# hpcde/spmv-acc

Measured on AMD Instinct MI355X. Metric: CSR SpMV GFLOP/s (fp64, int32 indices; achieved HBM GB/s in roofline), higher is better.
Workload: dtype f64

## Files before the change

include/spmv_acc.h:

```cpp
#ifndef SPMV_ACC_C_ABI_H
#define SPMV_ACC_C_ABI_H

#ifdef __cplusplus
extern "C" {
#endif

enum spmv_acc_strategy {
  SPMV_ACC_DEFAULT = 0,
  SPMV_ACC_ADAPTIVE = 1,
  SPMV_ACC_THREAD_ROW = 2,
  SPMV_ACC_WF_ROW = 3,
  SPMV_ACC_BLOCK_ROW_ORDINARY = 4,
  SPMV_ACC_LIGHT = 5,
  SPMV_ACC_VECTOR_ROW = 6,
  SPMV_ACC_LINE_ENHANCE = 7,
  SPMV_ACC_LINE = 8,
  SPMV_ACC_FLAT = 9,
  SPMV_ACC_ADAPTIVE_PLUS = 10
};
int spmv_acc_set_strategy(const char *name);
int spmv_acc_set_strategy_id(int strategy);
int spmv_acc_get_strategy(void);
const char *spmv_acc_strategy_name(int strategy);
int spmv_acc_parse_strategy(const char *name);

#ifndef SPMV_ACC_AMD_API_SPMV_H
void sparse_spmv(int htrans, const double halpha, const double hbeta, int hm, int hn, const int *rowptr,
                 const int *colindex, const double *value, const double *x, double *y);
#endif

void spmv_acc_csr_spmv(int trans, double alpha, double beta, int m, int n, int nnz, const int *h_rowptr,
                       const int *d_rowptr, const int *d_colindex, const double *d_value, const double *dx,
                       double *dy);

void spmv_acc_csr_spmv_strategy(int strategy, int trans, double alpha, double beta, int m, int n, int nnz,
                                const int *h_rowptr, const int *d_rowptr, const int *d_colindex,
                                const double *d_value, const double *dx, double *dy);

void spmv_acc_csr_spmv_oop(int strategy, int trans, double alpha, double beta, int m, int n, int nnz, const int *h_rowptr,
                           const int *d_rowptr, const int *d_colindex, const double *d_value, const double *dx,
                           const double *dy_in, double *dy_out);

enum spmv_acc_layout { SPMV_ACC_ROW_MAJOR = 0, SPMV_ACC_COL_MAJOR = 1 };
int spmv_acc_csr_spmm(int layout, int k, double alpha, double beta, int m, int n, int nnz, const int *h_rowptr,
                      const int *d_rowptr, const int *d_colindex, const double *d_value,
                      const double *dX, long long ldx, double *dY, long long ldy);

int spmv_acc_csr_spmv_chunks(int strategy, double alpha, double beta, int n, int nchunks, const int *row_cuts, const int *nnz_ends,
                             const int *d_rowptr, const int *d_colindex, const double *d_value, const double *dx,
                             const double *dy_in, double *dy_out, void *const *streams, void *const *events);

int spmv_acc_break_points(const int *d_rowptr, int m, int nnz, int stride, int *d_break_points, int bp_len);
int spmv_acc_break_points_len(int nnz, int stride);

int spmv_acc_adaptive_plus_analyze(int m, int min_nnz_per_block, int threads_per_block, int vec_size,
                                   const int *h_rowptr, int *h_break_points, int bp_cap,
                                   int *h_first_block_of_row);
int spmv_acc_adaptive_plus_analyze_device(int m, int min_nnz_per_block, int threads_per_block, int vec_size,
                                          const int *d_rowptr, int *d_break_points, int bp_cap,
                                          int *d_first_block_of_row);
int spmv_acc_adaptive_plus_vec(int m, int nnz);

int spmv_acc_adaptive_branch(int m, int rp_quarter, int rp_half, int rp_three_quarter, int rp_last);

int spmv_acc_partition_rows(int m, int parts, int mode, const int *h_rowptr, int *row_begin);

int spmv_acc_sharded_spmv(void *nccl_comm, int strategy, double alpha, double beta, int m_local, int m_pad, int n, int nnz_local,
                          const int *h_rowptr, const int *d_rowptr, const int *d_colindex, const double *d_value, const double *dx,
                          double *dy_local, double *dy_full);

typedef struct spmv_acc_shard *spmv_acc_shard_t;
int spmv_acc_shard_create(spmv_acc_shard_t *out, void *nccl_comm, int strategy, int m_local, int m_pad, int n, int nnz_local,
                          const int *d_rowptr, const int *d_colindex, const double *d_value, int pipeline);
int spmv_acc_shard_step(spmv_acc_shard_t shard, double alpha, double beta, const double *dx, const double *dy_in_local,
                        double *dy_full);
int spmv_acc_shard_prepare(spmv_acc_shard_t shard, double beta, const double *dx);
int spmv_acc_shard_pipeline(spmv_acc_shard_t shard);
int spmv_acc_shard_destroy(spmv_acc_shard_t shard);
int spmv_acc_rccl_comm_init_all(void **comms, int ndev, const int *devices);
int spmv_acc_rccl_comm_destroy(void *comm);

int spmv_acc_stage_csr(int m, int n, int nnz, const int *h_rowptr, const int *h_colindex, const double *h_value,
                       const double *h_x, const double *h_y, int **d_rowptr, int **d_colindex, double **d_value,
                       double **d_x, double **d_y);
int spmv_acc_free_device(void *p);

int spmv_acc_prepare(int strategy, int m, int n, int nnz, const int *h_rowptr, const int *d_rowptr, const int *d_colindex,
                     const double *d_value, const double *dx, float *ms_out);
int spmv_acc_prepare_beta(int strategy, double beta, int m, int n, int nnz, const int *h_rowptr, const int *d_rowptr,
                          const int *d_colindex, const double *d_value, const double *dx, float *ms_out);

void spmv_acc_set_tune_cache(const char *path);

int spmv_acc_refresh_values(const int *d_rowptr);

double spmv_acc_last_prepare_us(void);

void spmv_acc_release_plans(const int *d_rowptr);
int spmv_acc_cached_plans(void);
int spmv_acc_check_plans(void);
int spmv_acc_query_plan(const int *d_rowptr, int m, int *out);
int spmv_acc_query_plan_beta0(const int *d_rowptr, int m);
int spmv_acc_query_plan_slab_passes(const int *d_rowptr, int m);
int spmv_acc_query_plan_settled(const int *d_rowptr, int m);
int spmv_acc_query_plan_col16(const int *d_rowptr, int m);
enum spmv_acc_kernel {
  SPMV_ACC_KERNEL_ROWBLOCK = 0,
  SPMV_ACC_KERNEL_ROWBLOCK_PLUS = 1,
  SPMV_ACC_KERNEL_FLAT_TILE = 2,
  SPMV_ACC_KERNEL_SLAB_PASSES = 3,
  SPMV_ACC_KERNEL_VECTOR_TILE = 4, SPMV_ACC_KERNEL_VECTOR_ROW = 5, SPMV_ACC_KERNEL_WAVE_ROW = 6, SPMV_ACC_KERNEL_LIGHT = 7,
  SPMV_ACC_KERNEL_BLOCK_ROW = 8, SPMV_ACC_KERNEL_COL_SLABS = 9, SPMV_ACC_KERNEL_SCALE_ONLY = 10
};
int spmv_acc_query_plan_last_kernel(const int *d_rowptr, int m);

void spmv_acc_set_stream(void *hip_stream);
void *spmv_acc_get_stream(void);

int spmv_acc_last_error(void);
const char *spmv_acc_last_error_string(void);
void spmv_acc_clear_error(void);
enum spmv_acc_error {
  SPMV_ACC_OK = 0,
  SPMV_ACC_ERR_UNSUPPORTED_TRANS = 1,
  SPMV_ACC_ERR_BAD_ARGUMENT = 2,
  SPMV_ACC_ERR_HIP = 3,
  SPMV_ACC_ERR_TOO_LARGE = 4,
  SPMV_ACC_ERR_UNKNOWN_STRATEGY = 5,
  SPMV_ACC_ERR_NO_DEVICE = 6
};

int spmv_acc_time_spmv(int strategy, int iters, double alpha, double beta, int m, int n, int nnz,
                       const int *h_rowptr, const int *d_rowptr, const int *d_colindex, const double *d_value,
                       const double *dx, double *dy, const double *d_y0, float *ms_out);

int spmv_acc_time_spmv_events(int strategy, int iters, double alpha, double beta, int m, int n, int nnz,
                              const int *h_rowptr, const int *d_rowptr, const int *d_colindex, const double *d_value,
                              const double *dx, double *dy, const double *d_y0, float *ms_out, unsigned event_flags);

int spmv_acc_time_spmv_cold(int strategy, int iters, double alpha, double beta, int m, int n, int nnz,
                            const int *h_rowptr, const int *d_rowptr, const int *d_colindex, const double *d_value,
                            const double *dx, double *dy, const double *d_y0, void *d_flush, long long flush_bytes, float *ms_out);

int spmv_acc_time_spmv_total(int strategy, int iters, double alpha, double beta, int m, int n, int nnz,
                             const int *h_rowptr, const int *d_rowptr, const int *d_colindex, const double *d_value,
                             const double *dx, double *dy, float *total_ms_out);
int spmv_acc_time_spmv_kernels(int strategy, int iters, double alpha, double beta, int m, int n, int nnz,
                               const int *h_rowptr, const int *d_rowptr, const int *d_colindex, const double *d_value,
                               const double *dx, double *dy, const double *d_y0, float *event_ms_out, float *kernel_ms_out, int *launches_out);
int spmv_acc_time_spmv_region(int strategy, int iters, double alpha, double beta, int m, int n, int nnz,
                              const int *h_rowptr, const int *d_rowptr, const int *d_colindex, const double *d_value,
                              const double *dx, double *dy, float *total_ms_out);
double spmv_acc_copy_ceiling_gbs(void *d_dst, const void *d_src, long long bytes, int reps);

int spmv_acc_set_tunable(const char *name, int value);
int spmv_acc_get_tunable(const char *name);
void spmv_acc_reset_tunables(void);

const char *spmv_acc_version(void);

#ifdef __cplusplus
}
#endif

#endif
```

spmv_acc_amd/__init__.py:

```python
from __future__ import annotations

import ctypes
import os
from typing import Optional, Sequence

_HERE = os.path.dirname(os.path.abspath(__file__))
LIB_PATH = os.path.join(_HERE, "lib", "libspmv_acc.so")

STRATEGIES = (
    "default", "adaptive", "thread_row", "wf_row", "block_row_ordinary", "light",
    "vector_row", "line_enhance", "line", "flat", "adaptive_plus",
)
HOT_STRATEGIES = ("default", "adaptive", "flat", "line_enhance", "line", "vector_row", "adaptive_plus")

_c_int_p = ctypes.POINTER(ctypes.c_int)
_c_double_p = ctypes.POINTER(ctypes.c_double)

C_ABI_SYMBOLS = (
    "sparse_spmv", "spmv_acc_csr_spmv", "spmv_acc_csr_spmv_strategy", "spmv_acc_set_strategy",
    "spmv_acc_set_strategy_id", "spmv_acc_get_strategy", "spmv_acc_strategy_name", "spmv_acc_parse_strategy",
    "spmv_acc_break_points", "spmv_acc_break_points_len", "spmv_acc_adaptive_plus_analyze",
    "spmv_acc_adaptive_plus_vec", "spmv_acc_adaptive_branch", "spmv_acc_partition_rows", "spmv_acc_stage_csr",
    "spmv_acc_free_device", "spmv_acc_release_plans", "spmv_acc_cached_plans", "spmv_acc_query_plan",
    "spmv_acc_set_stream", "spmv_acc_get_stream", "spmv_acc_last_error", "spmv_acc_last_error_string",
    "spmv_acc_clear_error", "spmv_acc_time_spmv", "spmv_acc_version", "spmv_acc_set_tunable",
    "spmv_acc_get_tunable", "spmv_acc_reset_tunables", "spmv_acc_time_spmv_total", "spmv_acc_copy_ceiling_gbs", "spmv_acc_adaptive_plus_analyze_device", "spmv_acc_prepare",
    "spmv_acc_last_prepare_us", "spmv_acc_sharded_spmv", "spmv_acc_shard_prepare", "spmv_acc_csr_spmv_chunks", "spmv_acc_query_plan_settled", "spmv_acc_query_plan_col16", "spmv_acc_time_spmv_cold", "spmv_acc_csr_spmv_oop", "spmv_acc_check_plans",
    "spmv_acc_query_plan_beta0", "spmv_acc_query_plan_slab_passes", "spmv_acc_shard_create", "spmv_acc_shard_step", "spmv_acc_shard_pipeline",
    "spmv_acc_shard_destroy", "spmv_acc_rccl_comm_init_all", "spmv_acc_rccl_comm_destroy", "spmv_acc_set_tune_cache",
    "spmv_acc_prepare_beta", "spmv_acc_time_spmv_events", "spmv_acc_refresh_values", "spmv_acc_time_spmv_region", "spmv_acc_query_plan_last_kernel", "spmv_acc_time_spmv_kernels",
    "spmv_acc_csr_spmm",
)

_lib = None


class SpmvAccError(RuntimeError):
    pass


def load_library(path: Optional[str] = None) -> ctypes.CDLL:
    global _lib
    if _lib is not None and path is None:
        return _lib
    p = path or LIB_PATH
    if not os.path.exists(p):
        raise SpmvAccError(
            f"{p} not found: the HIP extension is not built. Run `python -c 'import __graft_entry__ as g; g.build()'` "
            "or `make -C spmv_acc_amd/csrc`. There is no CPU fallback."
        )
    try:
        import torch
    except ImportError:
        pass
    lib = ctypes.CDLL(p)
    vp, ci, cd = ctypes.c_void_p, ctypes.c_int, ctypes.c_double
    lib.sparse_spmv.argtypes = [ci, cd, cd, ci, ci, vp, vp, vp, vp, vp]
    lib.sparse_spmv.restype = None
    lib.spmv_acc_csr_spmv.argtypes = [ci, cd, cd, ci, ci, ci, vp, vp, vp, vp, vp, vp]
    lib.spmv_acc_csr_spmv.restype = None
    lib.spmv_acc_csr_spmv_strategy.argtypes = [ci, ci, cd, cd, ci, ci, ci, vp, vp, vp, vp, vp, vp]
    lib.spmv_acc_csr_spmv_strategy.restype = None
    lib.spmv_acc_set_strategy.argtypes = [ctypes.c_char_p]
    lib.spmv_acc_set_strategy_id.argtypes = [ci]
    lib.spmv_acc_strategy_name.argtypes = [ci]
    lib.spmv_acc_strategy_name.restype = ctypes.c_char_p
    lib.spmv_acc_parse_strategy.argtypes = [ctypes.c_char_p]
    lib.spmv_acc_break_points.argtypes = [vp, ci, ci, ci, vp, ci]
    lib.spmv_acc_break_points_len.argtypes = [ci, ci]
    lib.spmv_acc_adaptive_plus_analyze.argtypes = [ci, ci, ci, ci, vp, vp, ci, vp]
    lib.spmv_acc_adaptive_plus_vec.argtypes = [ci, ci]
    lib.spmv_acc_adaptive_plus_analyze_device.argtypes = [ci, ci, ci, ci, vp, vp, ci, vp]
    lib.spmv_acc_adaptive_branch.argtypes = [ci, ci, ci, ci, ci]
    lib.spmv_acc_partition_rows.argtypes = [ci, ci, ci, vp, vp]
    lib.spmv_acc_stage_csr.argtypes = [ci, ci, ci, vp, vp, vp, vp, vp] + [ctypes.POINTER(vp)] * 5
    lib.spmv_acc_free_device.argtypes = [vp]
    lib.spmv_acc_prepare.argtypes = [ci, ci, ci, ci, vp, vp, vp, vp, vp, ctypes.POINTER(ctypes.c_float)]
    lib.spmv_acc_release_plans.argtypes = [vp]
    lib.spmv_acc_release_plans.restype = None
    lib.spmv_acc_query_plan.argtypes = [vp, ci, vp]
    lib.spmv_acc_set_stream.argtypes = [vp]
    lib.spmv_acc_set_stream.restype = None
    lib.spmv_acc_get_stream.restype = vp
    lib.spmv_acc_last_error_string.restype = ctypes.c_char_p
    lib.spmv_acc_clear_error.restype = None
    lib.spmv_acc_time_spmv.argtypes = [ci, ci, cd, cd, ci, ci, ci, vp, vp, vp, vp, vp, vp, vp, vp]
    lib.spmv_acc_time_spmv_events.argtypes = [ci, ci, cd, cd, ci, ci, ci, vp, vp, vp, vp, vp, vp, vp, vp, ctypes.c_uint]
    lib.spmv_acc_time_spmv_cold.argtypes = [ci, ci, cd, cd, ci, ci, ci, vp, vp, vp, vp, vp, vp, vp, vp, ctypes.c_longlong, vp]
    lib.spmv_acc_version.restype = ctypes.c_char_p
    lib.spmv_acc_set_tunable.argtypes = [ctypes.c_char_p, ci]
    lib.spmv_acc_get_tunable.argtypes = [ctypes.c_char_p]
    lib.spmv_acc_reset_tunables.restype = None
    lib.spmv_acc_time_spmv_total.argtypes = [ci, ci, cd, cd, ci, ci, ci, vp, vp, vp, vp, vp, vp, vp]
    lib.spmv_acc_time_spmv_kernels.argtypes = [ci, ci, cd, cd, ci, ci, ci, vp, vp, vp, vp, vp, vp, vp, vp, vp, vp]
    lib.spmv_acc_time_spmv_region.argtypes = [ci, ci, cd, cd, ci, ci, ci, vp, vp, vp, vp, vp, vp, vp]
    lib.spmv_acc_copy_ceiling_gbs.argtypes = [vp, vp, ctypes.c_longlong, ci]
    lib.spmv_acc_copy_ceiling_gbs.restype = cd
    lib.spmv_acc_last_prepare_us.restype = cd
    lib.spmv_acc_sharded_spmv.argtypes = [vp, ci, cd, cd, ci, ci, ci, ci, vp, vp, vp, vp, vp, vp, vp]
    lib.spmv_acc_csr_spmv_oop.argtypes = [ci, ci, cd, cd, ci, ci, ci, vp, vp, vp, vp, vp, vp, vp]
    lib.spmv_acc_csr_spmv_oop.restype = None
    lib.spmv_acc_query_plan_beta0.argtypes = [vp, ci]
    lib.spmv_acc_query_plan_slab_passes.argtypes = [vp, ci]
    lib.spmv_acc_query_plan_settled.argtypes = [vp, ci]
    lib.spmv_acc_query_plan_col16.argtypes = [vp, ci]
    lib.spmv_acc_query_plan_last_kernel.argtypes = [vp, ci]
    lib.spmv_acc_shard_create.argtypes = [ctypes.POINTER(vp), vp, ci, ci, ci, ci, ci, vp, vp, vp, ci]
    lib.spmv_acc_shard_step.argtypes = [vp, cd, cd, vp, vp, vp]
    lib.spmv_acc_shard_pipeline.argtypes = [vp]
    lib.spmv_acc_shard_destroy.argtypes = [vp]
    lib.spmv_acc_rccl_comm_init_all.argtypes = [ctypes.POINTER(vp), ci, vp]
    lib.spmv_acc_rccl_comm_destroy.argtypes = [vp]
    lib.spmv_acc_set_tune_cache.argtypes = [ctypes.c_char_p]
    lib.spmv_acc_set_tune_cache.restype = None
    lib.spmv_acc_refresh_values.argtypes = [vp]
    lib.spmv_acc_prepare_beta.argtypes = [ci, cd, ci, ci, ci, vp, vp, vp, vp, vp, ctypes.POINTER(ctypes.c_float)]
    lib.spmv_acc_shard_prepare.argtypes = [vp, cd, vp]
    lib.spmv_acc_csr_spmv_chunks.argtypes = [ci, cd, cd, ci, ci, vp, vp, vp, vp, vp, vp, vp, vp, vp, vp]
    ll = ctypes.c_longlong
    lib.spmv_acc_csr_spmm.argtypes = [ci, ci, cd, cd, ci, ci, ci, vp, vp, vp, vp, vp, ll, vp, ll]
    lib.spmv_acc_csr_spmm.restype = ci
    if path is None:
        _lib = lib
    return lib


def strategy_id(name_or_id) -> int:
    if isinstance(name_or_id, int):
        return name_or_id
    s = load_library().spmv_acc_parse_strategy(str(name_or_id).encode())
    if s < 0:
        raise SpmvAccError(f"unknown KERNEL_STRATEGY {name_or_id!r}")
    return s


def _check(lib) -> None:
    code = lib.spmv_acc_last_error()
    if code not in (0, 1):
        msg = lib.spmv_acc_last_error_string().decode()
        lib.spmv_acc_clear_error()
        raise SpmvAccError(f"spmv_acc error {code}: {msg}")


def _ptr(t) -> int:
    if t is None:
        return 0
    if isinstance(t, int):
        return t
    if hasattr(t, "data_ptr"):
        return t.data_ptr()
    return t.ctypes.data


def _require_cuda(*tensors) -> None:
    for t in tensors:
        if t is not None and hasattr(t, "is_cuda") and not t.is_cuda:
            raise SpmvAccError("device pointers required: tensor is not on the GPU (no CPU fallback)")


def _require(lib, **named) -> None:
    device = None
    for name, (t, kind, count) in named.items():
        if t is None or not hasattr(t, "is_cuda"):
            continue
        if not t.is_cuda:
            raise SpmvAccError(f"{name}: device pointers required, tensor is not on the GPU (no CPU fallback)")
        want = "torch.int32" if kind == "i32" else "torch.float64"
        if str(t.dtype) != want:
            raise SpmvAccError(f"{name}: dtype {t.dtype}, the library reads {want} (int32 indices, fp64 values)")
        if not t.is_contiguous():
            raise SpmvAccError(f"{name}: tensor is not contiguous")
        if t.numel() < count:
            raise SpmvAccError(f"{name}: {t.numel()} elements, the shape needs at least {count}")
        if device is None:
            device = t.device
        elif t.device != device:
            raise SpmvAccError(f"{name}: on {t.device}, other arguments on {device}")
    if device is not None:
        import torch

        lib.spmv_acc_set_stream(torch.cuda.current_stream(device).cuda_stream)


def _csr_args(lib, m, n, nnz, rowptr, colindex, value, x, y=None, y0=None) -> None:
    k = max(nnz, 0)
    _require(lib, rowptr=(rowptr, "i32", m + 1), colindex=(colindex, "i32", k), value=(value, "f64", k),
             x=(x, "f64", n), y=(y, "f64", m), y0=(y0, "f64", m))


def sparse_spmv(trans: int, alpha: float, beta: float, m: int, n: int, rowptr, colindex, value, x, y) -> None:
    lib = load_library()
    _csr_args(lib, m, n, -1, rowptr, colindex, value, x, y)
    lib.sparse_spmv(trans, alpha, beta, m, n, _ptr(rowptr), _ptr(colindex), _ptr(value), _ptr(x), _ptr(y))
    _check(lib)


def csr_spmv(alpha: float, beta: float, m: int, n: int, nnz: int, rowptr, colindex, value, x, y,
             strategy=None, h_rowptr=None, trans: int = 0, y_in=None) -> None:
    lib = load_library()
    _csr_args(lib, m, n, nnz, rowptr, colindex, value, x, y, y_in)
    if y_in is not None:
        lib.spmv_acc_csr_spmv_oop(-1 if strategy is None else strategy_id(strategy), trans, alpha, beta, m, n, nnz,
                                  _ptr(h_rowptr), _ptr(rowptr), _ptr(colindex), _ptr(value), _ptr(x), _ptr(y_in), _ptr(y))
        _check(lib)
        return
    args = (trans, alpha, beta, m, n, nnz, _ptr(h_rowptr), _ptr(rowptr), _ptr(colindex), _ptr(value), _ptr(x), _ptr(y))
    if strategy is None:
        lib.spmv_acc_csr_spmv(*args)
    else:
        lib.spmv_acc_csr_spmv_strategy(strategy_id(strategy), *args)
    _check(lib)


SPMM_ROW_MAJOR, SPMM_COL_MAJOR = 0, 1


def _spmm_layouts(name, t, rows: int, k: int):
    s0, s1 = t.stride()
    out = {}
    if (s1 == 1 or k <= 1) and s0 >= max(k, 1):
        out[SPMM_ROW_MAJOR] = s0
    if (s0 == 1 or rows <= 1) and s1 >= max(rows, 1):
        out[SPMM_COL_MAJOR] = s1
    if not out and rows > 0 and k > 0:
        raise SpmvAccError(f"{name}: strides {tuple(t.stride())} of a ({rows}, {k}) view are neither row-major (unit stride on dim 1, "
                           f"leading dimension >= k) nor column-major (unit stride on dim 0, leading dimension >= {rows})")
    return out


def csr_spmm(alpha: float, beta: float, m: int, n: int, nnz: int, rowptr, colindex, value, X, Y, h_rowptr=None) -> None:
    lib = load_library()
    for name, t, rows in (("X", X, n), ("Y", Y, m)):
        if not hasattr(t, "is_cuda") or not hasattr(t, "stride"):
            raise SpmvAccError(f"{name}: a torch tensor on the GPU is required")
        if not t.is_cuda:
            raise SpmvAccError(f"{name}: device pointers required, tensor is not on the GPU (no CPU fallback)")
        if str(t.dtype) != "torch.float64":
            raise SpmvAccError(f"{name}: dtype {t.dtype}, the library reads torch.float64")
        if t.dim() != 2 or t.shape[0] != rows:
            raise SpmvAccError(f"{name}: shape {tuple(t.shape)}, expected ({rows}, k)")
    if X.shape[1] != Y.shape[1]:
        raise SpmvAccError(f"X has {X.shape[1]} columns, Y has {Y.shape[1]}")
    if X.device != Y.device:
        raise SpmvAccError(f"Y: on {Y.device}, X on {X.device}")
    k = int(X.shape[1])
    lx, ly = _spmm_layouts("X", X, n, k), _spmm_layouts("Y", Y, m, k)
    if not lx or not ly:
        layout, ldx, ldy = SPMM_ROW_MAJOR, k, k
    else:
        both = [lay for lay in (SPMM_ROW_MAJOR, SPMM_COL_MAJOR) if lay in lx and lay in ly]
        if not both:
            raise SpmvAccError("X and Y must share one layout (both row-major or both column-major)")
        layout = both[0]
        ldx, ldy = lx[layout], ly[layout]
    _require(lib, rowptr=(rowptr, "i32", m + 1), colindex=(colindex, "i32", max(nnz, 0)), value=(value, "f64", max(nnz, 0)))
    if hasattr(rowptr, "device") and rowptr.device != X.device:
        raise SpmvAccError(f"X: on {X.device}, rowptr on {rowptr.device}")
    lib.spmv_acc_set_stream(__import__("torch").cuda.current_stream(X.device).cuda_stream)
# ... 40 lines not shown
    if blocks < 0:
        raise SpmvAccError(f"adaptive_plus_analyze failed ({blocks})")
    return blocks, bp[: blocks + 1].copy(), fbr


def adaptive_plus_analyze_device(rowptr, m: int, nnz: int, min_nnz_per_block: int = 1024, threads_per_block: int = 256,
                                 vec_size: int = 1):
    import torch

    lib = load_library()
    _require(lib, rowptr=(rowptr, "i32", m + 1))
    cap = m + 2 + nnz // (2 * min_nnz_per_block)
    bp = torch.empty(cap, dtype=torch.int32, device=rowptr.device)
    fbr = torch.empty(m + 1, dtype=torch.int32, device=rowptr.device)
    blocks = lib.spmv_acc_adaptive_plus_analyze_device(m, min_nnz_per_block, threads_per_block, vec_size, _ptr(rowptr),
                                                       _ptr(bp), cap, _ptr(fbr))
    if blocks < 0:
        _check(lib)
        raise SpmvAccError(f"adaptive_plus_analyze_device failed ({blocks})")
    return blocks, bp[: blocks + 1], fbr


def adaptive_branch(m: int, h_rowptr) -> int:
    return load_library().spmv_acc_adaptive_branch(m, int(h_rowptr[m // 4]), int(h_rowptr[m // 2]),
                                                   int(h_rowptr[3 * m // 4]), int(h_rowptr[m]))


def partition_rows(m: int, parts: int, mode: int = 0, h_rowptr=None):
    import numpy as np

    lib = load_library()
    out = np.zeros(parts + 1, dtype=np.int32)
    if h_rowptr is not None:
        h_rowptr = np.ascontiguousarray(h_rowptr, dtype=np.int32)
    rc = lib.spmv_acc_partition_rows(m, parts, mode, _ptr(h_rowptr), _ptr(out))
    if rc != 0:
        _check(lib)
        raise SpmvAccError("partition_rows failed")
    return out


EVENT_DISABLE_SYSTEM_FENCE = 0x20000000


def time_spmv(strategy, iters: int, alpha: float, beta: float, m: int, n: int, nnz: int, rowptr, colindex, value,
              x, y, y0=None, h_rowptr=None, event_flags: int = 0) -> Sequence[float]:
    lib = load_library()
    _csr_args(lib, m, n, nnz, rowptr, colindex, value, x, y, y0)
    out = (ctypes.c_float * iters)()
    rc = lib.spmv_acc_time_spmv_events(strategy_id(strategy), iters, alpha, beta, m, n, nnz, _ptr(h_rowptr), _ptr(rowptr),
                                       _ptr(colindex), _ptr(value), _ptr(x), _ptr(y), _ptr(y0),
                                       ctypes.cast(out, ctypes.c_void_p), event_flags)
    if rc != 0:
        msg = lib.spmv_acc_last_error_string().decode()
        raise SpmvAccError(f"time_spmv failed ({rc}): {msg}")
    return list(out)


def time_spmv_cold(strategy, iters: int, alpha: float, beta: float, m: int, n: int, nnz: int, rowptr, colindex, value, x, y, y0, flush,
                   h_rowptr=None) -> Sequence[float]:
    lib = load_library()
    _csr_args(lib, m, n, nnz, rowptr, colindex, value, x, y, y0)
    out = (ctypes.c_float * iters)()
    rc = lib.spmv_acc_time_spmv_cold(strategy_id(strategy), iters, alpha, beta, m, n, nnz, _ptr(h_rowptr), _ptr(rowptr), _ptr(colindex),
                                     _ptr(value), _ptr(x), _ptr(y), _ptr(y0), _ptr(flush), int(flush.numel() * flush.element_size()),
                                     ctypes.cast(out, ctypes.c_void_p))
    if rc != 0:
        raise SpmvAccError(f"time_spmv_cold failed ({rc}): {lib.spmv_acc_last_error_string().decode()}")
    return list(out)


def time_spmv_total(strategy, iters: int, alpha: float, beta: float, m: int, n: int, nnz: int, rowptr, colindex, value,
                    x, y, h_rowptr=None) -> float:
    lib = load_library()
    _csr_args(lib, m, n, nnz, rowptr, colindex, value, x, y)
    out = ctypes.c_float(0.0)
    rc = lib.spmv_acc_time_spmv_total(strategy_id(strategy), iters, alpha, beta, m, n, nnz, _ptr(h_rowptr), _ptr(rowptr),
                                      _ptr(colindex), _ptr(value), _ptr(x), _ptr(y), ctypes.addressof(out))
    if rc != 0:
        raise SpmvAccError(f"time_spmv_total failed ({rc}): {lib.spmv_acc_last_error_string().decode()}")
    return float(out.value)


def time_spmv_kernels(strategy, iters: int, alpha: float, beta: float, m: int, n: int, nnz: int, rowptr, colindex, value, x, y, y0=None):
    lib = load_library()
    _csr_args(lib, m, n, nnz, rowptr, colindex, value, x, y, y0)
    ev = (ctypes.c_float * iters)()
    kn = (ctypes.c_float * iters)()
    ln = (ctypes.c_int * iters)()
    rc = lib.spmv_acc_time_spmv_kernels(strategy_id(strategy), iters, alpha, beta, m, n, nnz, None, _ptr(rowptr), _ptr(colindex), _ptr(value),
                                        _ptr(x), _ptr(y), _ptr(y0), ctypes.cast(ev, ctypes.c_void_p), ctypes.cast(kn, ctypes.c_void_p),
                                        ctypes.cast(ln, ctypes.c_void_p))
    if rc != 0:
        raise SpmvAccError(f"time_spmv_kernels failed ({rc}): {lib.spmv_acc_last_error_string().decode()}")
    return list(ev), list(kn), list(ln)


def time_spmv_region(strategy, iters: int, alpha: float, beta: float, m: int, n: int, nnz: int, rowptr, colindex, value, x, y):
    lib = load_library()
    _csr_args(lib, m, n, nnz, rowptr, colindex, value, x, y)
    out = ctypes.c_float(0.0)
    args = (strategy_id(strategy), iters, alpha, beta, m, n, nnz, None, _ptr(rowptr), _ptr(colindex), _ptr(value), _ptr(x), _ptr(y),
            ctypes.addressof(out))
    fn = lib.spmv_acc_time_spmv_region

    def run() -> float:
        rc = fn(*args)
        if rc != 0:
            raise SpmvAccError(f"time_spmv_region failed ({rc}): {lib.spmv_acc_last_error_string().decode()}")
        return float(out.value)

    return run


def copy_ceiling_gbs(dst, src, reps: int = 5) -> float:
    lib = load_library()
    _require_cuda(dst, src)
    nbytes = (src.numel() * src.element_size()) // 16 * 16
    return float(lib.spmv_acc_copy_ceiling_gbs(_ptr(dst), _ptr(src), nbytes, reps))


def release_plans(rowptr=None) -> None:
    load_library().spmv_acc_release_plans(_ptr(rowptr))


def set_tune_cache(path: Optional[str]) -> None:
    load_library().spmv_acc_set_tune_cache(path.encode() if path else None)


def refresh_values(rowptr) -> int:
    return int(load_library().spmv_acc_refresh_values(_ptr(rowptr)))


def check_plans() -> int:
    return int(load_library().spmv_acc_check_plans())


KERNEL_NAMES = {0: "rowblock", 1: "rowblock_plus", 2: "flat_tile", 3: "slab_passes", 4: "vector_tile", 5: "vector_row", 6: "wave_row", 7: "light",
                8: "block_row", 9: "col_slabs", 10: "scale_only"}


def query_plan(rowptr, m: int):
    import numpy as np

    out = np.zeros(9, dtype=np.int32)
    found = load_library().spmv_acc_query_plan(_ptr(rowptr), m, _ptr(out))
    if not found:
        return None
    keys = ("nnz", "adaptive_branch", "vec", "flat_tiles", "plus_blocks", "aligned16", "stream_policy", "flat_fixup", "adaptive_family")
    info = dict(zip(keys, (int(v) for v in out)))
    info["slab_passes"] = max(0, int(load_library().spmv_acc_query_plan_slab_passes(_ptr(rowptr), m)))
    info["settled"] = int(load_library().spmv_acc_query_plan_settled(_ptr(rowptr), m)) == 1
    info["col16"] = int(load_library().spmv_acc_query_plan_col16(_ptr(rowptr), m))
    info["last_kernel"] = KERNEL_NAMES.get(int(load_library().spmv_acc_query_plan_last_kernel(_ptr(rowptr), m)), "none")
    return info


def set_strategy(name: str) -> None:
    lib = load_library()
    if lib.spmv_acc_set_strategy(name.encode()) != 0:
        lib.spmv_acc_clear_error()
        raise SpmvAccError(f"unknown KERNEL_STRATEGY {name!r}")


def get_strategy() -> str:
    lib = load_library()
    return lib.spmv_acc_strategy_name(lib.spmv_acc_get_strategy()).decode()
```

spmv_acc_amd/csrc/c_api.cpp:

```cpp
#include <hip/hip_runtime.h>

#include <dlfcn.h>

#include <algorithm>
#include <cstdlib>
#include <cstring>
#include <mutex>
#include <vector>

#include "../../include/spmv_acc.h"
#include "engine.hpp"

#include <string>
#include <cstdint>

using namespace spmv_acc;

namespace {
struct PinTable {
  std::mutex mu;
  struct Range { uintptr_t lo, hi; int refs; };
  std::vector<Range> ranges;
  static constexpr uintptr_t kPage = 4096;
  bool pin(void *p, size_t bytes) {
// ... 202 lines not shown
  if (e != hipSuccess) {
    set_error(kErrHip, hipGetErrorString(e));
    return kErrHip;
  }
  return kOk;
}

int spmv_acc_adaptive_plus_analyze(int m, int min_nnz_per_block, int threads_per_block, int vec_size,
                                   const int *h_rowptr, int *h_break_points, int bp_cap,
                                   int *h_first_block_of_row) {
  if (m < 0 || !h_rowptr || !h_break_points || !h_first_block_of_row || min_nnz_per_block <= 0 || vec_size <= 0 ||
      threads_per_block < vec_size) {
    set_error(kErrBadArgument, "spmv_acc_adaptive_plus_analyze: bad argument");
    return -2;
  }
  std::vector<int> bp, fbr;
  const int blocks = plus_analyze_host(m, min_nnz_per_block, threads_per_block, vec_size, h_rowptr, bp, fbr);
  if (static_cast<int>(bp.size()) > bp_cap) return -1;
  std::copy(bp.begin(), bp.end(), h_break_points);
  std::copy(fbr.begin(), fbr.end(), h_first_block_of_row);
  return blocks;
}

int spmv_acc_adaptive_plus_analyze_device(int m, int min_nnz_per_block, int threads_per_block, int vec_size,
                                          const int *d_rowptr, int *d_break_points, int bp_cap,
                                          int *d_first_block_of_row) {
  if (m < 0 || !d_rowptr || !d_break_points || !d_first_block_of_row || min_nnz_per_block <= 0 || vec_size <= 0 ||
      threads_per_block < vec_size || bp_cap < 1) {
    set_error(kErrBadArgument, "spmv_acc_adaptive_plus_analyze_device: bad argument");
    return -2;
  }
  return plus_analyze_device(m, min_nnz_per_block, threads_per_block, vec_size, d_rowptr, d_break_points, bp_cap,
                             d_first_block_of_row);
}

int spmv_acc_adaptive_plus_vec(int m, int nnz) { return plus_pick_vec(m, nnz); }

int spmv_acc_adaptive_branch(int m, int rp_quarter, int rp_half, int rp_three_quarter, int rp_last) {
  if (m <= 0) return 0;
  RowptrSamples s;
  s.q1 = rp_quarter;
  s.half = rp_half;
  s.q3 = rp_three_quarter;
  s.last = rp_last;
  return adaptive_branch(m, s);
}

int spmv_acc_partition_rows(int m, int parts, int mode, const int *h_rowptr, int *row_begin) {
  if (m < 0 || parts <= 0 || !row_begin || (mode == 1 && !h_rowptr)) {
    set_error(kErrBadArgument, "spmv_acc_partition_rows: bad argument");
    return kErrBadArgument;
  }
  row_begin[0] = 0;
  row_begin[parts] = m;
  if (mode == 0) {
    const long long per = (static_cast<long long>(m) + parts - 1) / parts;
    for (int p = 1; p < parts; ++p) row_begin[p] = static_cast<int>(std::min<long long>(per * p, m));
  } else {
    const long long nnz = h_rowptr[m];
    for (int p = 1; p < parts; ++p) {
      const long long target = nnz * p / parts;
      const int *it = std::lower_bound(h_rowptr, h_rowptr + m + 1, static_cast<int>(target));
      int r = static_cast<int>(it - h_rowptr);
      r = std::max(r, row_begin[p - 1]);
      row_begin[p] = std::min(r, m);
    }
  }
  return kOk;
}

int spmv_acc_sharded_spmv(void *nccl_comm, int strategy, double alpha, double beta, int m_local, int m_pad, int n, int nnz_local,
                          const int *h_rowptr, const int *d_rowptr, const int *d_colindex, const double *d_value, const double *dx,
                          double *dy_local, double *dy_full) {
  if (!nccl_comm || m_local < 0 || m_pad < m_local || m_pad <= 0 || !dy_local || !dy_full) {
    set_error(kErrBadArgument, "spmv_acc_sharded_spmv: bad argument");
    return kErrBadArgument;
  }
  const nccl_all_gather_t all_gather = resolve_all_gather();
  if (!all_gather) {
    set_error(kErrNoDevice, "spmv_acc_sharded_spmv: no RCCL found in the process (librccl.so.1 / librccl.so / SPMV_ACC_RCCL_LIB)");
    return kErrNoDevice;
  }
  clear_error();
  if (m_local > 0) run_spmv(strategy, 0, alpha, beta, m_local, n, nnz_local, h_rowptr, d_rowptr, d_colindex, d_value, dx, dy_local);
  if (last_error() != kOk) return last_error();
  const int rc = all_gather(dy_local, dy_full, static_cast<size_t>(m_pad), kNcclFloat64, nccl_comm, get_stream());
  if (rc != 0) {
    set_error(kErrHip, "spmv_acc_sharded_spmv: ncclAllGather failed (ncclResult " + std::to_string(rc) + ")");
    return kErrHip;
  }
  return kOk;
}

int spmv_acc_stage_csr(int m, int n, int nnz, const int *h_rowptr, const int *h_colindex, const double *h_value,
                       const double *h_x, const double *h_y, int **d_rowptr, int **d_colindex, double **d_value,
                       double **d_x, double **d_y) {
  if (m < 0 || n < 0 || nnz < 0 || !d_rowptr || !d_colindex || !d_value || !d_x || !d_y) {
    set_error(kErrBadArgument, "spmv_acc_stage_csr: bad argument");
    return kErrBadArgument;
  }
  Stager st;
  bool ok = st.ok;
  ok = ok && stage_one(st, h_rowptr, static_cast<size_t>(m) + 1, d_rowptr);
  ok = ok && stage_one(st, h_colindex, static_cast<size_t>(nnz), d_colindex);
  ok = ok && stage_one(st, h_value, static_cast<size_t>(nnz), d_value);
  ok = ok && stage_one(st, h_x, static_cast<size_t>(n), d_x);
  ok = ok && stage_one(st, h_y, static_cast<size_t>(m), d_y);
  ok = ok && hipStreamSynchronize(st.copy) == hipSuccess;
  if (!ok) {
    const hipError_t e = hipGetLastError();
    set_error(kErrHip, std::string("spmv_acc_stage_csr: ") + hipGetErrorString(e));
    return kErrHip;
  }
  return kOk;
}

int spmv_acc_free_device(void *p) {
  if (!p) return kOk;
  return hipFree(p) == hipSuccess ? kOk : kErrHip;
}

void spmv_acc_release_plans(const int *d_rowptr) { release_plans(d_rowptr); }
int spmv_acc_cached_plans(void) { return cached_plan_count(); }
int spmv_acc_check_plans(void) { return check_plans(); }
int spmv_acc_query_plan(const int *d_rowptr, int m, int *out) {
  PlanInfo info;
  if (!out || !query_plan(d_rowptr, m, &info)) return 0;
  out[0] = info.nnz;
  out[1] = info.adaptive_branch;
  out[2] = info.vec;
  out[3] = info.flat_tiles;
  out[4] = info.plus_blocks;
  out[5] = info.aligned16;
  out[6] = info.stream_policy;
  out[7] = info.flat_fixup;
  out[8] = info.adaptive_family;
  return 1;
}
int spmv_acc_query_plan_beta0(const int *d_rowptr, int m) {
  PlanInfo info;
  return query_plan(d_rowptr, m, &info) ? info.adaptive_family_beta0 : -2;
}
int spmv_acc_query_plan_slab_passes(const int *d_rowptr, int m) {
  PlanInfo info;
  return query_plan(d_rowptr, m, &info) ? info.slab_passes : -2;
}
int spmv_acc_query_plan_last_kernel(const int *d_rowptr, int m) {
  PlanInfo info;
  return query_plan(d_rowptr, m, &info) ? info.last_kernel : -2;
}
int spmv_acc_query_plan_col16(const int *d_rowptr, int m) {
  PlanInfo info;
  return query_plan(d_rowptr, m, &info) ? info.col16 : -2;
}
int spmv_acc_query_plan_settled(const int *d_rowptr, int m) {
  PlanInfo info;
  return query_plan(d_rowptr, m, &info) ? info.settled : -2;
}

void spmv_acc_set_stream(void *hip_stream) { set_stream(static_cast<hipStream_t>(hip_stream)); }
void *spmv_acc_get_stream(void) { return static_cast<void *>(get_stream()); }

int spmv_acc_set_tunable(const char *name, int value) { return name ? set_tunable(name, value) : -1; }
int spmv_acc_get_tunable(const char *name) { return name ? get_tunable(name) : -1; }
void spmv_acc_reset_tunables(void) { reset_tunables(); }

double spmv_acc_last_prepare_us(void) { return last_prepare_us(); }

int spmv_acc_last_error(void) { return last_error(); }
const char *spmv_acc_last_error_string(void) { return last_error_string(); }
void spmv_acc_clear_error(void) { clear_error(); }

void spmv_acc_set_tune_cache(const char *path) { set_tune_cache(path); }
int spmv_acc_refresh_values(const int *d_rowptr) { return refresh_values(d_rowptr); }

int spmv_acc_prepare(int strategy, int m, int n, int nnz, const int *h_rowptr, const int *d_rowptr, const int *d_colindex,
                     const double *d_value, const double *dx, float *ms_out) {
  return spmv_acc_prepare_beta(strategy, 1.0, m, n, nnz, h_rowptr, d_rowptr, d_colindex, d_value, dx, ms_out);
}

int spmv_acc_prepare_beta(int strategy, double beta, int m, int n, int nnz, const int *h_rowptr, const int *d_rowptr,
                          const int *d_colindex, const double *d_value, const double *dx, float *ms_out) {
  if (m <= 0) return kOk;
  hipStream_t st = get_stream();
  double *scratch = nullptr;
  if (hipMalloc(reinterpret_cast<void **>(&scratch), sizeof(double) * static_cast<size_t>(m)) != hipSuccess) {
    set_error(kErrHip, "spmv_acc_prepare: hipMalloc failed");
    return kErrHip;
  }
  hipEvent_t e0 = nullptr, e1 = nullptr;
  const bool timed = ms_out && hipEventCreate(&e0) == hipSuccess && hipEventCreate(&e1) == hipSuccess;
  clear_error();
  if (timed) (void)hipEventRecord(e0, st);
  (void)hipMemsetAsync(scratch, 0, sizeof(double) * static_cast<size_t>(m), st);
  {
    UnboundedTuningScope unbounded;
    for (int round = 0; round < 6; ++round) {
      run_spmv(strategy, 0, 1.0, beta != 0.0 ? 1.0 : 0.0, m, n, nnz, h_rowptr, d_rowptr, d_colindex, d_value, dx, scratch);
      if (last_error() != kOk || last_prepare_us() <= 0.0) break;
    }
  }
  if (timed) (void)hipEventRecord(e1, st);
  int rc = hipStreamSynchronize(st) == hipSuccess ? kOk : kErrHip;
  if (timed && rc == kOk && hipEventElapsedTime(ms_out, e0, e1) != hipSuccess) rc = kErrHip;
  if (e0) (void)hipEventDestroy(e0);
  if (e1) (void)hipEventDestroy(e1);
  (void)hipFree(scratch);
  if (rc != kOk) set_error(kErrHip, "spmv_acc_prepare: HIP failure");
  if (rc == kOk && last_error() != kOk) rc = last_error();
  return rc;
}

int spmv_acc_time_spmv(int strategy, int iters, double alpha, double beta, int m, int n, int nnz,
                       const int *h_rowptr, const int *d_rowptr, const int *d_colindex, const double *d_value,
                       const double *dx, double *dy, const double *d_y0, float *ms_out) {
  return spmv_acc_time_spmv_events(strategy, iters, alpha, beta, m, n, nnz, h_rowptr, d_rowptr, d_colindex, d_value, dx, dy, d_y0,
                                   ms_out, 0u);
}

static int time_spmv_per_launch(int strategy, int iters, double alpha, double beta, int m, int n, int nnz,
                                const int *h_rowptr, const int *d_rowptr, const int *d_colindex, const double *d_value,
                                const double *dx, double *dy, const double *d_y0, float *ms_out, unsigned event_flags, void *d_flush,
                                long long flush_bytes);
int spmv_acc_time_spmv_events(int strategy, int iters, double alpha, double beta, int m, int n, int nnz,
                              const int *h_rowptr, const int *d_rowptr, const int *d_colindex, const double *d_value,
                              const double *dx, double *dy, const double *d_y0, float *ms_out, unsigned event_flags) {
  return time_spmv_per_launch(strategy, iters, alpha, beta, m, n, nnz, h_rowptr, d_rowptr, d_colindex, d_value, dx, dy, d_y0, ms_out, event_flags,
                              nullptr, 0);
}
int spmv_acc_time_spmv_cold(int strategy, int iters, double alpha, double beta, int m, int n, int nnz, const int *h_rowptr,
                            const int *d_rowptr, const int *d_colindex, const double *d_value, const double *dx, double *dy,
                            const double *d_y0, void *d_flush, long long flush_bytes, float *ms_out) {
  if (!d_flush || flush_bytes < 32 || reinterpret_cast<uintptr_t>(d_flush) % 16 != 0) {
    set_error(kErrBadArgument, "spmv_acc_time_spmv_cold: needs a 16-byte aligned scratch buffer");
    return kErrBadArgument;
  }
  return time_spmv_per_launch(strategy, iters, alpha, beta, m, n, nnz, h_rowptr, d_rowptr, d_colindex, d_value, dx, dy, d_y0, ms_out, 0u, d_flush,
                              flush_bytes);
}
static int time_spmv_per_launch(int strategy, int iters, double alpha, double beta, int m, int n, int nnz,
                                const int *h_rowptr, const int *d_rowptr, const int *d_colindex, const double *d_value,
                                const double *dx, double *dy, const double *d_y0, float *ms_out, unsigned event_flags, void *d_flush,
                                long long flush_bytes) {
  if (iters <= 0 || !ms_out) {
    set_error(kErrBadArgument, "spmv_acc_time_spmv: bad argument");
    return kErrBadArgument;
  }
  if (spmv_acc_prepare_beta(strategy, beta, m, n, nnz, h_rowptr, d_rowptr, d_colindex, d_value, dx, nullptr) != kOk) return last_error();
  hipStream_t st = get_stream();
  std::vector<hipEvent_t> ev(2 * static_cast<size_t>(iters));
  for (auto &e : ev) {
    if (hipEventCreateWithFlags(&e, event_flags) != hipSuccess) {
      set_error(kErrHip, "hipEventCreate failed");
      return kErrHip;
    }
  }
  clear_error();
  static const bool reset_memcpy = [] {
    const char *e = std::getenv("SPMV_ACC_RESET_MEMCPY");
    return e && *e && *e != '0';
  }();
  static const bool reset_nt = [] {
    const char *e = std::getenv("SPMV_ACC_RESET_NT");
    return !(e && *e == '0');
  }();
  const size_t ybytes = sizeof(double) * static_cast<size_t>(m);
  const bool kernel_copy = !reset_memcpy && reinterpret_cast<uintptr_t>(dy) % 16 == 0 && reinterpret_cast<uintptr_t>(d_y0) % 16 == 0;
  for (int i = 0; i < iters; ++i) {
    if (d_y0) {
      const size_t body = kernel_copy ? ybytes / 16 * 16 : 0;
      if (body) launch_stream_copy(st, dy, d_y0, static_cast<long long>(body), reset_nt);
      if (body < ybytes && kernel_copy)
        hipLaunchKernelGGL(copy_doubles_kernel, dim3(1), dim3(64), 0, st, dy + body / 8, d_y0 + body / 8, static_cast<int>((ybytes - body) / 8));
      else if (body < ybytes)
        (void)hipMemcpyAsync(dy, d_y0, ybytes, hipMemcpyDeviceToDevice, st);
    }
    if (d_flush) {
      const long long half = flush_bytes / 2 / 16 * 16;
      launch_stream_copy(st, static_cast<char *>(d_flush) + half, d_flush, half, false);
    }
    (void)hipEventRecord(ev[2 * i], st);
    run_spmv(strategy, 0, alpha, beta, m, n, nnz, h_rowptr, d_rowptr, d_colindex, d_value, dx, dy);
    (void)hipEventRecord(ev[2 * i + 1], st);
  }
  int rc = kOk;
  if (hipStreamSynchronize(st) != hipSuccess) rc = kErrHip;
  for (int i = 0; i < iters && rc == kOk; ++i) {
    if (hipEventElapsedTime(&ms_out[i], ev[2 * i], ev[2 * i + 1]) != hipSuccess) rc = kErrHip;
  }
  for (auto &e : ev) (void)hipEventDestroy(e);
  if (rc != kOk) set_error(kErrHip, "spmv_acc_time_spmv: HIP failure while timing");
  if (rc == kOk && last_error() != kOk) rc = last_error();
  return rc;
}

int spmv_acc_time_spmv_total(int strategy, int iters, double alpha, double beta, int m, int n, int nnz,
                             const int *h_rowptr, const int *d_rowptr, const int *d_colindex, const double *d_value,
                             const double *dx, double *dy, float *total_ms_out) {
  if (iters <= 0 || !total_ms_out) {
    set_error(kErrBadArgument, "spmv_acc_time_spmv_total: bad argument");
    return kErrBadArgument;
  }
  if (spmv_acc_prepare_beta(strategy, beta, m, n, nnz, h_rowptr, d_rowptr, d_colindex, d_value, dx, nullptr) != kOk) return last_error();
  hipStream_t st = get_stream();
  hipEvent_t e0, e1;
  if (hipEventCreate(&e0) != hipSuccess || hipEventCreate(&e1) != hipSuccess) {
// ... 156 lines not shown
```

spmv_acc_amd/csrc/dispatch.cpp:

```cpp
#include "engine_internal.hpp"

namespace spmv_acc {
using namespace detail;

namespace detail {

constexpr int kFlatMaxTileRows = 16384;

thread_local int t_strict_name = -1;

bool run_flat(hipStream_t st, Plan &p, double alpha, double beta, const double *x, double *y) {
  if (!ensure_flat(p, st)) return false;
  const bool strict = t_strict_name == kFlat;
  if (p.flat.max_tile_rows > kFlatMaxTileRows && tun(kT_rowblock_guard) && !strict) {
    return run_rowblock(st, p, nullptr, alpha, beta, x, y, false, 0);
  }
  p.A.cold = nullptr;
  p.flat.col16 = nullptr;
  if (!autotune_policy(p, kFamFlat, st, [&](int pol, double *ys) { launch_flat_with(st, p, pol, 1.0, trial_beta(), x, ys); })) return false;
  if (!autotune_flat_mode(p, st, x)) return false;
  if (!autotune_flat_geometry(p, st, x)) return false;
  if (!autotune_hint(p, kFamFlat, st, [&](double *ys) { launch_flat_with(st, p, policy_for(p, kFamFlat), 1.0, trial_beta(), x, ys); })) return false;
  const Col16 *c16 = nullptr;
  if (p.flat.stride == kThreads * kNnzPerThread && !flat_segment_sum() &&
      !autotune_col16(p, kFamFlat, st, [&](const Col16 *c, double *ys) {
        p.flat.col16 = c;
        launch_flat_with(st, p, policy_for(p, kFamFlat), 1.0, trial_beta(), x, ys);
      }, &c16))
    return false;
  p.flat.col16 = c16;
  const int rb_mode = tun(kT_flat_rowblock);
  const bool tile_pinned = tun(kT_flat_finish) >= 0 || tun(kT_flat_npt) >= 0 || tun(kT_flat_early) >= 0;
  if (rb_mode != 0 && (rb_mode > 0 || !tile_pinned) && !flat_segment_sum() && tun(kT_col16) <= 0 &&
      !t_coarse_tuning && !strict) {
    if (rb_mode > 0) {
      int vec = 1, rpb = kThreads;
      pick_rowblock_shape(p.A.m, p.A.count(), rowblock_target_for(p), &vec, &rpb);
      if (t_capturing ? (p.rowblock_ok == 1 && p.rowblock_rpb == rpb) : (probe_rowblock(p, rpb, st) && p.rowblock_ok == 1))
        return run_rowblock(st, p, nullptr, alpha, beta, x, y, false, 0);
    } else if (p.flat_rowblock_choice < 0 && !t_capturing && !by_rule()) {
      int vec = 1, rpb = kThreads;
      pick_rowblock_shape(p.A.m, p.A.count(), rowblock_target_for(p), &vec, &rpb);
      if (!probe_rowblock(p, rpb, st)) return false;
      p.flat_rowblock_choice = 0;
      if (p.rowblock_ok == 1) {
        TimingPhase ph(st, p.A.m);
        float ms2[2] = {0.f, 0.f};
        bool ok = ph.ok && run_rowblock(st, p, nullptr, 1.0, trial_beta(), x, ph.y, false);
        ok = ok && ph.in_turns(2, [&](int c) {
          if (c == 0) launch_flat_with(st, p, policy_for(p, kFamFlat), 1.0, trial_beta(), x, ph.y);
          else (void)run_rowblock(st, p, nullptr, 1.0, trial_beta(), x, ph.y, false);
        }, ranking_rounds(), ms2);
        if (!ok) return false;
        const float ms_flat = ms2[0], ms_rb = ms2[1];
        p.flat_rowblock_choice = ms_rb < 0.985f * ms_flat ? 1 : 0;
        tune_log("m %d nnz %d flat on balanced rows: tile kernel %.2f us, row blocks %.2f us -> %s", p.A.m, p.A.nnz, ms_flat * 1e3f, ms_rb * 1e3f,
                 p.flat_rowblock_choice ? "row blocks" : "tile kernel");
      }
    }
    if (rb_mode < 0 && p.flat_rowblock_choice == 1) return run_rowblock(st, p, nullptr, alpha, beta, x, y, false, 0);
  }
  launch_flat_with(st, p, policy_for(p, kFamFlat), alpha, beta, x, y);
  p.last_kernel = kKernelFlatTile;
  p.last_c16 = c16 && p.flat.stride == kThreads * kNnzPerThread && p.A.cold == nullptr ? c16->rec_ints : 0;
  return true;
}

bool validate_plan(Plan &p, hipStream_t st) {
  if (p.invalid < 0) {
    if (!plan_work_allowed("validating the matrix")) return false;
    ++t_plan_work;
    int *d_flags = nullptr;
    int h = -1;
    if (!hip_ok(hipMalloc(reinterpret_cast<void **>(&d_flags), sizeof(int)), "hipMalloc validate")) return false;
    if (hip_ok(hipMemsetAsync(d_flags, 0, sizeof(int), st), "memset validate")) {
      launch_validate_csr(st, p.A, d_flags);
      if (!hip_ok(hipMemcpyAsync(&h, d_flags, sizeof(int), hipMemcpyDeviceToHost, st), "read validate") ||
          !hip_ok(hipStreamSynchronize(st), "sync validate"))
        h = -1;
    }
    (void)hipFree(d_flags);
    if (h < 0) return false;
    p.invalid = h;
  }
  if (p.invalid != 0) {
    std::string what = "matrix failed validation:";
    if (p.invalid & 1) what += " rowptr decreases or is negative;";
    if (p.invalid & 2) what += " rowptr[m] != nnz;";
    if (p.invalid & 4) what += " column index outside [0, n);";
    set_error(kErrBadArgument, what);
    return false;
  }
  return true;
}

bool launch_full_guard(Plan &p, hipStream_t st) {
  if (!p.A.guard || !p.A.stale) return true;
  if (!p.have_rp_digest) {
    if (!plan_work_allowed("the full row-pointer digest (guard_full)")) return false;
    ++t_plan_work;
    const size_t words = static_cast<size_t>(Plan::kDigestSlots) * kDigestMaxParts + 1;
    if (!p.d_digest_acc && !hip_ok(hipMalloc(reinterpret_cast<void **>(&p.d_digest_acc), sizeof(unsigned long long) * words), "hipMalloc digest"))
      return false;
    unsigned long long *out = p.d_digest_acc + words - 1;
    launch_rowptr_digest(st, p.A.rp, p.A.m, p.d_digest_acc);
    launch_rowptr_verdict(st, p.d_digest_acc, p.A.m, 0, nullptr, out);
    unsigned long long h = 0;
    if (!hip_ok(hipMemcpyAsync(&h, out, sizeof(h), hipMemcpyDeviceToHost, st), "read digest") || !hip_ok(hipStreamSynchronize(st), "sync digest"))
      return false;
    p.rp_digest = h;
    p.have_rp_digest = true;
  }
  unsigned long long *part = p.d_digest_acc + static_cast<size_t>(p.digest_turn++ % Plan::kDigestSlots) * kDigestMaxParts;
  launch_rowptr_digest(st, p.A.rp, p.A.m, part);
  launch_rowptr_verdict(st, part, p.A.m, p.rp_digest, p.A.stale, nullptr);
  return true;
}

bool probe_rowblock(Plan &p, int rpb, hipStream_t st) {
  if (p.rowblock_ok >= 0 && p.rowblock_rpb == rpb) return true;
  if (!plan_work_allowed("the row-block balance probe")) return false;
  ++t_plan_work;
  p.rowblock_rpb = rpb;
  int *d_max = nullptr;
  if (!hip_ok(hipMalloc(reinterpret_cast<void **>(&d_max), 2 * sizeof(int)), "hipMalloc probe")) return false;
  bool ok = hip_ok(hipMemsetAsync(d_max, 0, 2 * sizeof(int), st), "memset probe");
  if (ok) {
    const long long nblocks = (static_cast<long long>(p.A.m) + rpb - 1) / rpb;
    const long long avg_block = nblocks > 0 ? p.A.count() / nblocks : 0;
    launch_max_block_nnz(st, p.A.rp, p.A.m, rpb, static_cast<int>(avg_block), d_max);
    int h[2] = {0, 0};
    ok = hip_ok(hipMemcpyAsync(h, d_max, 2 * sizeof(int), hipMemcpyDeviceToHost, st), "read probe") &&
         hip_ok(hipStreamSynchronize(st), "sync probe");
    if (ok) {
      p.max_block_nnz = h[0];
      const bool few_rounds = h[0] <= kRowblockMaxRounds * kTile;
      const bool near_avg = h[0] <= kTile || h[0] <= 4 * avg_block;
      p.rowblock_ok = (few_rounds && near_avg) ? 1 : 0;
      p.rowblock_uneven = nblocks >= 16 && 5LL * h[1] >= nblocks;
    }
  }
  (void)hipFree(d_max);
  return ok;
}

bool ensure_digest(Plan &p, int rpb, hipStream_t st) {
  if (p.digest.lens && p.digest.rpb == rpb) return true;
  if (!plan_work_allowed("the row digest")) return false;
  ++t_plan_work;
  p.free_digest();
  const size_t nblocks = (static_cast<size_t>(p.A.m) + rpb - 1) / rpb;
  if (!hip_ok(hipMalloc(reinterpret_cast<void **>(&p.digest.lens), static_cast<size_t>(p.A.m)), "hipMalloc row lengths") ||
      !hip_ok(hipMalloc(reinterpret_cast<void **>(&p.digest.base), sizeof(int) * (nblocks + 1)), "hipMalloc row-block bases")) {
    p.free_digest();
    return false;
  }
  launch_row_digest(st, p.A.rp, p.A.m, rpb, p.digest.lens, p.digest.base);
  if (!hip_ok(hipStreamSynchronize(st), "build the row digest")) {
    p.free_digest();
    return false;
  }
  p.digest.rpb = rpb;
  return true;
}

bool run_plus(hipStream_t st, Plan &p, const int *h_rowptr, double alpha, double beta, const double *x, double *y);

bool run_rowblock(hipStream_t st, Plan &p, const int *h_rowptr, double alpha, double beta, const double *x, double *y,
                  bool allow_uneven_switch, int lanes_per_row) {
  int vec = 1, rpb = kThreads;
  const int forced = tun(kT_rowblock_vec);
  auto shape_for = [&](int target, int *v_out, int *r_out) {
    pick_rowblock_shape(p.A.m, p.A.count(), target, v_out, r_out);
    if (lanes_per_row > 0) *v_out = lanes_per_row;
    if (forced > 0) {
      *v_out = forced;
      *r_out = kThreads / forced;
    }
  };
  shape_for(rowblock_target_for(p), &vec, &rpb);
  if (tun(kT_rowblock_guard)) {
    if (!probe_rowblock(p, rpb, st)) return false;
    if (p.rowblock_ok == 0)
      return run_plus(st, p, h_rowptr, alpha, beta, x, y);
    if (p.rowblock_uneven && allow_uneven_switch) return run_plus(st, p, h_rowptr, alpha, beta, x, y);
  }
  const RowDigest *dg = nullptr;
  int cache_ends = 0;
  const int want_lens = tun(kT_rowlen);
  auto setup = [&]() {
    dg = nullptr;
    if (want_lens > 0 || (want_lens < 0 && static_cast<long long>(p.A.count()) <= 8LL * p.A.m)) {
      const bool have = p.digest.lens && p.digest.rpb == rpb;
      if (have || !t_capturing) {
        if (!ensure_digest(p, rpb, st)) return false;
        dg = &p.digest;
      }
    }
    cache_ends = 0;
    if (tun(kT_cache_ends_mb) > 0 && tun(kT_zigzag) && p.A.count() > 0) {
      const long long nblocks = (static_cast<long long>(p.A.m) + rpb - 1) / rpb;
      const double bytes_per_block = 12.0 * p.A.count() / static_cast<double>(nblocks);
      cache_ends = static_cast<int>(tun(kT_cache_ends_mb) * 1048576.0 / bytes_per_block);
    }
    return true;
  };
  if (!setup()) return false;
  const int chunk = tun(kT_xcd_chunk);
  const int base_flags = chunk > 0 ? (4 | (chunk << 8)) : 0;
  p.A.cold = nullptr;
  if (!autotune_policy(p, kFamRowblock, st, [&](int pol, double *ys) {
        const int zz = next_reverse(p) ? 64 : 0;
        launch_rowblock_stream(st, p.A, vec, rpb, base_flags | (pol << 4) | zz, 1.0, trial_beta(), x, ys, dg, cache_ends);
      }))
    return false;
  if (tun(kT_rowblock_target) <= 0 && p.rb_target == 0 && p.stream_policy[kFamRowblock][t_beta_class] >= 0 && !t_capturing && !t_coarse_tuning &&
      !t_no_policy_timing && !by_rule()) {
    int v2[2], r2[2];
    const int cand[2] = {kRowblockTargetRule, kRowblockTargetAlt};
    for (int c = 0; c < 2; ++c) shape_for(cand[c], &v2[c], &r2[c]);
    if (v2[0] == v2[1] && r2[0] == r2[1]) {
      p.rb_target = cand[0];
    } else {
      TimingPhase ph(st, p.A.m);
      bool ok = ph.ok;
      bool skip[2] = {false, false};
      float ms[2] = {1e30f, 1e30f};
      const int pol = policy_for(p, kFamRowblock);
      for (int c = 0; ok && c < 2; ++c) {
        vec = v2[c];
        rpb = r2[c];
        if (tun(kT_rowblock_guard)) {
          ok = probe_rowblock(p, rpb, st);
          skip[c] = ok && p.rowblock_ok == 0;
        }
      }
      for (int round = 0; ok && round < ranking_rounds(); ++round) {
        for (int c = 0; ok && c < 2; ++c) {
          if (skip[c]) continue;
          vec = v2[c];
          rpb = r2[c];
          ok = setup();
          float t = 0.f;
          ok = ok && ph.time([&] {
            const int zz = next_reverse(p) ? 64 : 0;
            launch_rowblock_stream(st, p.A, vec, rpb, base_flags | (pol << 4) | zz, 1.0, trial_beta(), x, ph.y, dg, cache_ends);
          }, &t);
          if (ok && t < ms[c]) ms[c] = t;
        }
      }
      if (!ok) return false;
      p.rb_target = (!skip[1] && (skip[0] || ms[1] < 0.985f * ms[0])) ? cand[1] : cand[0];
      tune_log("m %d nnz %d row blocks: %d products per block %.2f us, %d products %.2f us -> %d", p.A.m, p.A.nnz, cand[0], ms[0] * 1e3f, cand[1], ms[1] * 1e3f,
               p.rb_target);
    }
    shape_for(rowblock_target_for(p), &vec, &rpb);
    if (tun(kT_rowblock_guard) && !probe_rowblock(p, rpb, st)) return false;
    if (!setup()) return false;
  }
  if (!autotune_hint(p, kFamRowblock, st, [&](double *ys) {
        const int zz = next_reverse(p) ? 64 : 0;
        launch_rowblock_stream(st, p.A, vec, rpb, base_flags | (policy_for(p, kFamRowblock) << 4) | zz, 1.0, trial_beta(), x, ys, dg, cache_ends);
      }))
    return false;
  const Col16 *c16 = nullptr;
  if (!autotune_col16(p, kFamRowblock, st, [&](const Col16 *c, double *ys) {
        const int zz = next_reverse(p) ? 64 : 0;
        launch_rowblock_stream(st, p.A, vec, rpb, base_flags | (policy_for(p, kFamRowblock) << 4) | zz, 1.0, trial_beta(), x, ys, dg, cache_ends, c);
      }, &c16))
    return false;
  const int zz = next_reverse(p) ? 64 : 0;
  launch_rowblock_stream(st, p.A, vec, rpb, base_flags | (policy_for(p, kFamRowblock) << 4) | zz, alpha, beta, x, y, dg, cache_ends, c16);
  p.last_kernel = kKernelRowblock;
  p.last_c16 = c16 && p.A.cold == nullptr ? c16->rec_ints : 0;
  return true;
}

bool run_plus_prepare(Plan &p, const int *h_rowptr, hipStream_t st, const double *x) {
  auto launch = [&](int pol, double *ys) {
    launch_plus(st, p.A, p.d_pbp, p.d_pfbr, p.d_pblk, p.plus_blocks, p.plus_has_long, tun(kT_xcd_chunk), pol,
                p.d_ppartial, 1.0, trial_beta(), x, ys, next_reverse(p));
  };
  const int forced = tun(kT_plus_min_nnz);
  if (forced > 0) {
    return ensure_plus(p, h_rowptr, st, forced > 0 ? forced : kPlusMinNnz) && autotune_policy(p, kFamPlus, st, launch);
  }
  if (tun(kT_deterministic)) {
    int vec = 1, rpb = kThreads;
    pick_rowblock_shape(p.A.m, p.A.count(), rowblock_target_for(p), &vec, &rpb);
    return probe_rowblock(p, rpb, st) && ensure_plus(p, h_rowptr, st, p.rowblock_ok == 0 ? kPlusMinNnz : 1536);
  }
  if (p.plus_tuned_min > 0) return ensure_plus(p, h_rowptr, st, p.plus_tuned_min) && autotune_policy(p, kFamPlus, st, launch);
  if (t_capturing) return (p.plus_blocks >= 0 || ensure_plus(p, h_rowptr, st, 1536)) && autotune_policy(p, kFamPlus, st, launch);
  if (t_coarse_tuning || defer_tuning())
    return ensure_plus(p, h_rowptr, st, p.rowblock_ok == 0 ? kPlusMinNnz : 1536) && autotune_policy(p, kFamPlus, st, launch);
  if (!ensure_plus(p, h_rowptr, st, 1536) || !autotune_policy(p, kFamPlus, st, launch)) return false;
  TimingPhase ph(st, p.A.m);
  bool ok = ph.ok;
  const int candidates[3] = {1536, 1920, kPlusMinNnz};
  float best = 1e30f;
  int best_min = kPlusMinNnz;
  for (int c = 0; ok && c < 3; ++c) {
    ok = ensure_plus(p, h_rowptr, st, candidates[c]);
    if (!ok) break;
    float ms = 0.f;
    ok = ph.time([&] { launch(policy_for(p, kFamPlus), ph.y); }, &ms);
    if (ok) tune_log("m %d nnz %d beta class %d row-block-plus: MIN_NNZ_PER_BLOCK %d -> %.2f us (kept for both classes)", p.A.m, p.A.nnz, t_beta_class, candidates[c], ms * 1e3f);
    if (ok && ms < best) {
      best = ms;
      best_min = candidates[c];
    }
  }
  if (!ok) return false;
  p.plus_tuned_min = best_min;
  return ensure_plus(p, h_rowptr, st, best_min);
}

thread_local bool t_in_slab = false;
bool ensure_segments(Plan &p, int S, hipStream_t st);
thread_local bool t_in_segment_timing = false;
static bool decide_whole_pass_hint(hipStream_t st, Plan &p, const double *x) {
  const int s = p.seg_slabs - 1;
  if (p.seg_rest_below <= 0 || p.seg_entries[s] == 0 || tun(kT_gather_hint) == 0 || static_cast<long long>(p.A.n) * 8 >= (1LL << 32)) return true;
  if (p.hint_state < 0 && !t_capturing && !ensure_hint(p, st)) return false;
  if (p.hint_state != 1 || !p.d_cold) return true;
  if (p.seg_whole_hint >= 0 || t_capturing || by_rule()) return true;
  TimingPhase ph(st, p.A.m, false);
  float ms[2] = {0.f, 0.f};
  bool ok = ph.ok;
  for (int h = 0; ok && h < 2; ++h)
    ok = ph.time([&] {
      launch_segment_tiles(st, p.seg_blocks[s], 1.0, p.seg_blk[s], p.seg_row[s], p.seg_begin[s], p.seg_vptr[s], p.A.ci, p.A.v, x, p.d_seg_ys, ph.y,
                           h ? p.d_cold : nullptr);
    }, &ms[h]);
  if (!ok) return false;
  p.seg_whole_hint = ms[1] < 0.985f * ms[0] ? 1 : 0;
  tune_log("m %d nnz %d: slab passes, whole-row pass: plain gathers %.1f us, hinted %.1f us -> %s", p.A.m, p.A.nnz, ms[0] * 1e3f, ms[1] * 1e3f,
           p.seg_whole_hint ? "hinted" : "plain");
  return true;
}

void run_segments(hipStream_t st, Plan &p, double alpha, double beta, const double *x, double *y) {
  p.last_kernel = kKernelSlabPasses;
  const int whole = p.seg_rest_below > 0 ? p.seg_slabs - 1 : -1;
  if (!t_in_segment_timing && !decide_whole_pass_hint(st, p, x)) return;
  const bool whole_hinted = whole >= 0 && p.hint_state == 1 && p.d_cold && p.seg_whole_hint != 0 && tun(kT_gather_hint) != 0 &&
                            static_cast<long long>(p.A.n) * 8 < (1LL << 32);
  const unsigned char *whole_cold = whole_hinted ? p.d_cold : nullptr;
  launch_guard_check(st, p.A);
  if (beta != 1.0 || p.A.yin) launch_scale_y(st, p.A.m, beta, y, p.A.yin);
  for (int s = 0; s < p.seg_slabs; ++s) {
    if (p.seg_entries[s] == 0) continue;
    launch_segment_tiles(st, p.seg_blocks[s], alpha, p.seg_blk[s], p.seg_row[s], p.seg_begin[s], p.seg_vptr[s], p.A.ci, p.A.v, x, p.d_seg_ys, y,
                         s == whole ? whole_cold : nullptr);
    if (p.seg_pieces[s]) launch_segment_merge(st, p.seg_pieces[s], p.seg_cut[s], p.seg_entries[s], p.seg_row[s], p.d_seg_ys, y);
  }
}
int seg_auto_slabs(int n) {
  const long long per = static_cast<long long>(tun(kT_slab_kb) > 0 ? tun(kT_slab_kb) : 32768) << 10;
  const long long s = (static_cast<long long>(n) * 8 + per / 2) / per;
  return s < 2 ? 2 : (s > 16 ? 16 : static_cast<int>(s));
}

bool run_plus(hipStream_t st, Plan &p, const int *h_rowptr, double alpha, double beta, const double *x, double *y) {
  p.A.cold = nullptr;
  auto launch_here = [&](double a, double b, double *yy) {
    launch_plus(st, p.A, p.d_pbp, p.d_pfbr, p.d_pblk, p.plus_blocks, p.plus_has_long, tun(kT_xcd_chunk), policy_for(p, kFamPlus),
                p.d_ppartial, a, b, x, yy, next_reverse(p));
  };
  auto time_against_segments = [&](float ms[2], bool *timed) {
    *timed = false;
    const int S_auto = seg_auto_slabs(p.A.n);
    if (p.seg_state < 0) {
      size_t free_b = 0, total_b = 0;
      const size_t build_bytes = (2 * static_cast<size_t>(S_auto) + 4) * (static_cast<size_t>(p.A.m) + 1) * sizeof(int) + (static_cast<size_t>(p.A.count()) / 4) * 12;
      const bool room = hipMemGetInfo(&free_b, &total_b) == hipSuccess && free_b > 2 * build_bytes;
      (void)hipGetLastError();
      if (room && last_error_code_only() == kOk && !ensure_segments(p, S_auto, st)) {
        (void)hipGetLastError();
        tune_log("m %d nnz %d: slab_segments: the run lists could not be built (%s), row-block-plus stays", p.A.m, p.A.nnz, last_error_string());
        clear_error();
        p.free_segments();
      }
    }
    if (p.seg_state != 1) return true;
    TimingPhase ph(st, p.A.m);
    ScopedSet<const double *> no_yin(p.A.yin, nullptr);
    bool ok = ph.ok && decide_whole_pass_hint(st, p, x);
    ScopedSet in_timing(t_in_segment_timing, true);
    ok = ok && ph.time([&] { launch_here(1.0, trial_beta(), ph.y); }, &ms[0]) && ph.time([&] { run_segments(st, p, 1.0, trial_beta(), x, ph.y); }, &ms[1]);
    if (ok && ms[0] < 1.33f * ms[1] && ms[1] < 1.33f * ms[0]) {
      float again[2] = {0.f, 0.f};
      ok = ph.time([&] { launch_here(1.0, trial_beta(), ph.y); }, &again[0]) && ph.time([&] { run_segments(st, p, 1.0, trial_beta(), x, ph.y); }, &again[1]);
      if (ok) ms[0] = std::min(ms[0], again[0]), ms[1] = std::min(ms[1], again[1]);
    }
    *timed = ok;
    return ok;
  };
  const bool slabs_auto = tun(kT_slab_segments) < 0 && !t_in_slab && t_strict_name != kLineEnhance && t_strict_name != kLine;
  if (slabs_auto && p.seg_choice < 0 && !p.seg_early_tried && !t_capturing && !by_rule() && tun(kT_gather_hint) != 0) {
    if (!ensure_hint(p, st)) return false;
    p.seg_early_tried = true;
    if (p.hint_state == 1) {
      {
        ScopedSet coarse(t_coarse_tuning, true), no_policy(t_no_policy_timing, true);
        if (!run_plus_prepare(p, h_rowptr, st, x)) return false;
      }
      float ms[2] = {0.f, 0.f};
      bool timed = false;
      if (!time_against_segments(ms, &timed)) return false;
      if (timed && ms[1] < 0.85f * ms[0]) p.seg_choice = 1;
      if (timed)
        tune_log("m %d nnz %d beta class %d: row-block-plus (coarse) %.2f us, %d column-slab passes over run lists %.2f us -> %s", p.A.m, p.A.nnz, t_beta_class,
                 ms[0] * 1e3f, seg_auto_slabs(p.A.n), ms[1] * 1e3f, p.seg_choice == 1 ? "slab passes" : "not decided: the kernel is tuned first");
      if (!timed) p.seg_choice = 0;
    }
  }
  if (slabs_auto && p.seg_choice == 1) {
    if (p.seg_state != 1 && !t_capturing && last_error_code_only() == kOk && !ensure_segments(p, seg_auto_slabs(p.A.n), st)) {
      (void)hipGetLastError();
      clear_error();
      p.free_segments();
      p.seg_choice = 0;
    }
    if (p.seg_state == 1) {
      run_segments(st, p, alpha, beta, x, y);
      return true;
// ... 92 lines not shown
    p.adaptive_family[cls] = best_family;
    p.adaptive_provisional[cls] = !looked_twice;
    if (!looked_twice) t_tuning_deferred = true;
  }
  return run_family(p.adaptive_family[cls], alpha, beta, y);
}

}


int refresh_values(const int *d_rowptr) {
  std::vector<std::shared_ptr<Plan>> todo;
  {
    std::lock_guard<std::mutex> lk(g_mu);
    for (auto &kv : g_plans)
      if (std::get<1>(kv.first) == d_rowptr && kv.second->d_slab_rp) todo.push_back(kv.second);
  }
  hipStream_t st = t_stream;
  for (auto &p : todo) {
    std::lock_guard<std::mutex> plan_lock(p->mu);
    if (!p->d_slab_rp) continue;
    launch_slab_scatter(st, p->A, p->slab_width, p->slab_count, p->d_slab_rp, p->d_slab_off, p->d_slab_ci, p->d_slab_v, true);
  }
  return static_cast<int>(todo.size());
}

UnboundedTuningScope::UnboundedTuningScope() { ++t_unbounded_tuning; }
UnboundedTuningScope::~UnboundedTuningScope() { --t_unbounded_tuning; }
FlatSegmentSumScope::FlatSegmentSumScope() : prev(t_flat_segment_sum) { t_flat_segment_sum = true; }
FlatSegmentSumScope::~FlatSegmentSumScope() { t_flat_segment_sum = prev; }

static bool run_col_slabs(Plan &p, int S, int strategy, hipStream_t st, double alpha, double beta, int m, int n, const double *dx, double *dy) {
  if (!ensure_slabs(p, S, st)) return false;
  launch_guard_check(st, p.A);
  if (beta != 1.0 || p.A.yin) launch_scale_y(st, m, beta, dy, p.A.yin);
  ScopedSet in_slab(t_in_slab, true);
  for (int s = 0; s < S && last_error_code_only() == kOk; ++s) {
    const long long o = p.slab_off[s];
    const int ms = p.slab_rows[s];
    if (ms == 0) continue;
    run_spmv(strategy, 0, alpha, 0.0, ms, n, static_cast<int>(p.slab_off[s + 1] - o), nullptr, p.slab_crp[s], p.d_slab_ci + o, p.d_slab_v + o, dx,
             p.d_slab_ys, nullptr);
    if (last_error_code_only() == kOk) launch_slab_merge(st, ms, p.slab_rowid[s], p.d_slab_ys, dy);
  }
  p.last_kernel = kKernelColSlabs;
  return last_error_code_only() == kOk;
}

static int slab_copy_auto(Plan &p, int strategy, hipStream_t st, int n, const double *dx) {
  const bool hook = tun(kT_col_slabs) == -2;
  if (p.slab_copy_choice == 0 || p.seg_state != 1 || !(hook || (p.seg_choice == 1 && tun(kT_slab_segments) < 0)) || tun(kT_deterministic) || t_strict_name >= 0 ||
      t_capturing || !dx)
    return 0;
  const int S = p.seg_slabs - (p.seg_rest_below > 0 ? 1 : 0);
  if (S < 2 || S > 16) return 0;
  const bool adopted = p.slab_copy_choice == 1 && !p.d_slab_rp;
  if (p.slab_copy_choice < 0 || adopted) {
    if (!(t_unbounded_tuning > 0 || (p.calls > static_cast<unsigned long long>(kSlabCopyAfterCalls) && !defer_tuning()))) return 0;
    size_t free_b = 0, total_b = 0;
    if (hipMemGetInfo(&free_b, &total_b) != hipSuccess || free_b < 36ull * static_cast<size_t>(p.A.count())) {
      (void)hipGetLastError();
      p.slab_copy_choice = 0;
      tune_log("m %d nnz %d: slab-major copy not built: %.1f GB free, 3 x 12 B per non-zero = %.1f GB wanted", p.A.m, p.A.nnz, free_b / 1e9, 36e-9 * p.A.count());
      return 0;
    }
    const int count = p.A.count() < kValueSamples ? p.A.count() : kValueSamples;
    TimingPhase ph(st, p.A.m);
    bool ok = ph.ok && ensure_slabs(p, S, st) &&
              hip_ok(hipMalloc(reinterpret_cast<void **>(&p.d_value_samples), 12 * static_cast<size_t>(count) + 8), "hipMalloc value samples") &&
              hip_ok(hipHostMalloc(reinterpret_cast<void **>(&p.h_values_changed), sizeof(int)), "hipHostMalloc value flag");
    if (ok) {
      *p.h_values_changed = 0;
      p.value_samples = count;
      launch_value_samples(st, p.A.v, p.A.ci, p.A.nnz0, p.A.count() - 1, count, p.d_value_samples, nullptr);
      UnboundedTuningScope unbounded;
      ScopedSet no_budget(t_budget_spmvs, 0.0);
      for (int round = 0; ok && round < 4 && !adopted; ++round) {
        const unsigned w0 = t_plan_work;
        ok = run_col_slabs(p, S, strategy, st, 1.0, trial_beta(), p.A.m, n, dx, ph.y) && hip_ok(hipStreamSynchronize(st), "settle the slabs' plans");
        if (t_plan_work == w0) break;
      }
      float ms[2] = {0.f, 0.f};
      ScopedSet in_timing(t_in_segment_timing, true);
      ok = ok && (adopted || ph.in_turns(2, [&](int c) {
        if (c == 0) run_segments(st, p, 1.0, trial_beta(), dx, ph.y);
        else (void)run_col_slabs(p, S, strategy, st, 1.0, trial_beta(), p.A.m, n, dx, ph.y);
      }, 2, ms));
      if (ok && !adopted) {
        p.slab_copy_choice = (ms[1] < 0.97f * ms[0] || tun(kT_col_slabs) == -2) ? 1 : 0;
        tune_log("m %d nnz %d: slab passes over run lists %.1f us, slab-major copy (%d slabs, %.2f GB held) %.1f us -> %s", p.A.m, p.A.nnz, ms[0] * 1e3f, S,
                 12e-9 * p.A.count(), ms[1] * 1e3f, p.slab_copy_choice ? "the copy (values guarded by samples)" : "the passes");
      }
    }
    if (!ok || p.slab_copy_choice != 1) {
      if (!ok) {
        (void)hipGetLastError();
        clear_error();
      }
      p.free_slabs();
      p.slab_copy_choice = 0;
      return 0;
    }
  }
  *p.h_values_changed = 0;
  launch_value_samples(st, p.A.v, p.A.ci, p.A.nnz0, p.A.count() - 1, p.value_samples, p.d_value_samples, p.h_values_changed);
  if (!hip_ok(hipStreamSynchronize(st), "compare the value samples")) return 0;
  if (*p.h_values_changed & 2) {
    tune_log("m %d nnz %d: the caller's column indices changed under the slab-major copy: the copy is dropped, the run-list passes serve", p.A.m, p.A.nnz);
    p.free_slabs();
    p.slab_copy_choice = 0;
    return 0;
  }
  if (*p.h_values_changed) {
    launch_slab_scatter(st, p.A, p.slab_width, p.slab_count, p.d_slab_rp, p.d_slab_off, p.d_slab_ci, p.d_slab_v, true);
    launch_value_samples(st, p.A.v, p.A.ci, p.A.nnz0, p.A.count() - 1, p.value_samples, p.d_value_samples, nullptr);
    ++p.values_refreshed;
    tune_log("m %d nnz %d: the caller's values changed under the slab-major copy: refreshed (%u so far)", p.A.m, p.A.nnz, p.values_refreshed);
  }
  return S;
}

namespace {
thread_local bool t_early_clock = false;
thread_local std::chrono::steady_clock::time_point t_early_began;

void run_spmv_call(int strategy, int trans, double alpha, double beta, int m, int n, int nnz, const int *h_rowptr,
                   const int *d_rowptr, const int *d_colindex, const double *d_value, const double *dx, double *dy,
                   const double *dy_in);
}

void run_spmv(int strategy, int trans, double alpha, double beta, int m, int n, int nnz, const int *h_rowptr,
              const int *d_rowptr, const int *d_colindex, const double *d_value, const double *dx, double *dy,
              const double *dy_in) {
  apply_env_tunables();
  bool early = rule_until_settled() && !t_in_slab && !t_rule_twin && t_unbounded_tuning == 0 && m > 0 && d_rowptr && dy && strategy >= 0 &&
               strategy < kStrategyCount && strategy < 32 && tun(kT_col_slabs) < 2;
  const bool capturing = early && stream_capturing(t_stream);
  if (early) early = !plan_settled_for(d_rowptr, d_colindex, d_value, m, n, strategy, beta != 0.0 ? 1 : 0);
  if (!early) {
    run_spmv_call(strategy, trans, alpha, beta, m, n, nnz, h_rowptr, d_rowptr, d_colindex, d_value, dx, dy, dy_in);
    return;
  }
  if (capturing && !rule_twin_exists(d_rowptr, d_colindex, d_value, m, n)) {
    run_spmv_call(strategy, trans, alpha, beta, m, n, nnz, h_rowptr, d_rowptr, d_colindex, d_value, dx, dy, dy_in);
    return;
  }
  if (capturing) {
    ScopedSet twin(t_rule_twin, true);
    run_spmv_call(strategy, trans, alpha, beta, m, n, nnz, h_rowptr, d_rowptr, d_colindex, d_value, dx, dy, dy_in);
    return;
  }
  const auto began = std::chrono::steady_clock::now();
  const int err_before = last_error_code_only();
  int served_kernel = -1, served_c16 = 0;
  {
    ScopedSet twin(t_rule_twin, true);
    run_spmv_call(strategy, trans, alpha, beta, m, n, nnz, h_rowptr, d_rowptr, d_colindex, d_value, dx, dy, dy_in);
    if (const std::shared_ptr<Plan> tp = t_last_plan.lock()) {
      served_kernel = tp->last_kernel;
      served_c16 = tp->last_c16;
    }
  }
  if (last_error_code_only() != err_before && last_error_code_only() != kOk && last_error_code_only() != kErrUnsupportedTrans) return;
  const double twin_prepare_us = t_last_prepare_us;
  double *scratch = tune_scratch(static_cast<size_t>(m));
  if (!scratch) {
    clear_error();
    return;
  }
  (void)hipMemsetAsync(scratch, 0, sizeof(double) * static_cast<size_t>(m), t_stream);
  t_early_began = began;
  {
    ScopedSet early_clock(t_early_clock, true);
    run_spmv_call(strategy, 0, alpha, beta, m, n, nnz, h_rowptr, d_rowptr, d_colindex, d_value, dx, scratch, nullptr);
  }
  t_last_prepare_us += twin_prepare_us;
  if (const std::shared_ptr<Plan> p = t_last_plan.lock()) {
    std::lock_guard<std::mutex> plan_lock(p->mu);
    const int cls = beta != 0.0 ? 1 : 0;
    if (!((p->settled_for[cls] >> strategy) & 1u)) {
      p->last_kernel = served_kernel;
      p->last_c16 = served_c16;
    }
  }
  if (plan_settled_for(d_rowptr, d_colindex, d_value, m, n, strategy, beta != 0.0 ? 1 : 0)) drop_rule_twin(d_rowptr, d_colindex, d_value, m, n);
}

namespace {
void run_spmv_call(int strategy, int trans, double alpha, double beta, int m, int n, int nnz, const int *h_rowptr,
                   const int *d_rowptr, const int *d_colindex, const double *d_value, const double *dx, double *dy,
                   const double *dy_in) {
  const int strategy_named = strategy;
  if (trans != 0) {
    set_error(kErrUnsupportedTrans, "only operation_none is supported; computed y = alpha*A*x + beta*y");
  }
  apply_env_tunables();
  if (m <= 0) return;
  if (m > INT_MAX - (1 << 16)) {
    set_error(kErrTooLarge, "row count does not leave room for block arithmetic in int32; shard the matrix");
    return;
  }
  if (!d_rowptr || !dy || (n > 0 && !dx)) {
    set_error(kErrBadArgument, "null rowptr / x / y");
    return;
  }
  if (dy_in == dy) dy_in = nullptr;
  if (dy_in && beta != 0.0) {
    const uintptr_t a = reinterpret_cast<uintptr_t>(dy_in), b = reinterpret_cast<uintptr_t>(dy), bytes = sizeof(double) * static_cast<uintptr_t>(m);
    if (a < b + bytes && b < a + bytes) {
      set_error(kErrBadArgument, "y_in and y_out overlap without being the same vector");
      return;
    }
  }
  hipStream_t st = t_stream;
  note_stream_use();
  t_capturing = stream_capturing(st);
  if (strategy < 0 || strategy >= kStrategyCount) {
    set_error(kErrUnknownStrategy, "unknown strategy id");
    return;
  }
  const std::shared_ptr<Plan> p = get_plan(m, n, nnz, h_rowptr, d_rowptr, d_colindex, d_value);
  if (!p) return;
  t_last_plan = p;
  struct ScratchScope {
    bool outer;
    ~ScratchScope() {
      if (outer) release_tune_scratch();
    }
  } scratch_scope{!t_in_slab};
  std::lock_guard<std::mutex> plan_lock(p->mu);
  t_beta_class = beta != 0.0 ? 1 : 0;
  struct BudgetScope {
    Plan &p;
    bool outer;
    int strategy, cls;
    ~BudgetScope() {
      if (!outer) return;
      if (t_first_trial_ms > 0.f) p.trial_ms = t_first_trial_ms;
      p.tuning_open = t_tuning_deferred;
      if (!t_tuning_deferred && strategy >= 0 && strategy < 32) p.settled_for[cls] |= 1u << strategy;
      t_budget_spmvs = 0.0;
      t_budget_ms = -1.0;
    }
  } budget_scope{*p, !t_in_slab, strategy_named, beta != 0.0 ? 1 : 0};
  if (!t_in_slab) {
    t_call_began = (t_early_clock && p->calls == 0) ? t_early_began : std::chrono::steady_clock::now();
    t_tuning_deferred = false;
    t_first_trial_ms = 0.f;
    const int allowance = p->calls == 0 ? tun(kT_first_call_budget) : tun(kT_later_call_budget);
    t_budget_spmvs = (t_unbounded_tuning > 0 || t_capturing || allowance <= 0) ? 0.0 : static_cast<double>(allowance);
    t_budget_ms = (t_budget_spmvs > 0.0 && p->trial_ms > 0.0) ? t_budget_spmvs * p->trial_ms : -1.0;
  }
  struct PrepareClock {
    unsigned work0;
    std::chrono::steady_clock::time_point t0;
    ~PrepareClock() {
      t_last_prepare_us =
          t_plan_work != work0 ? std::chrono::duration<double, std::micro>(std::chrono::steady_clock::now() - t0).count() : 0.0;
    }
  } prepare_clock{t_plan_work, std::chrono::steady_clock::now()};
  if (p->calls++ == 0) ++t_plan_work;
  (void)hipGetLastError();
  if (p->launched && p->last_stream != st && !t_capturing && !t_in_slab) {
    if (!p->order_event && hipEventCreateWithFlags(&p->order_event, hipEventDisableTiming) != hipSuccess) p->order_event = nullptr;
    if (p->order_event && hipEventRecord(p->order_event, p->last_stream) == hipSuccess) (void)hipStreamWaitEvent(st, p->order_event, 0);
    (void)hipGetLastError();
  }
  p->last_stream = st;
  p->launched = true;
  if (t_capturing) p->captured = true;
  struct YinScope {
    CsrDev &A;
    ~YinScope() { A.yin = nullptr; }
  } yin_scope{p->A};
  p->A.yin = beta != 0.0 ? dy_in : nullptr;
  p->last_c16 = 0;

  if (p->A.count() == 0) {
    launch_scale_y(st, m, beta, dy, p->A.yin);
    p->last_kernel = kKernelScaleOnly;
    return;
  }
  ScopedSet strict_scope(t_strict_name, t_in_slab ? t_strict_name : (tun(kT_strict_strategy) ? strategy : -1));
  if (!d_colindex || !d_value) {
    set_error(kErrBadArgument, "null colindex / value with nnz > 0");
    return;
  }
  if (tun(kT_validate) && !validate_plan(*p, st)) return;
  if (tun(kT_guard_full) && !t_in_slab && !launch_full_guard(*p, st)) return;

  int copy_slabs = (tun(kT_col_slabs) >= 2 && !t_in_slab) ? (tun(kT_col_slabs) > 64 ? 64 : tun(kT_col_slabs)) : 0;
  if (!copy_slabs && tun(kT_col_slabs) < 0 && !t_in_slab) copy_slabs = slab_copy_auto(*p, strategy, st, n, dx);
  if (copy_slabs) {
    if (!run_col_slabs(*p, copy_slabs, strategy, st, alpha, beta, m, n, dx, dy)) return;
    t_last_plan = p;
    t_beta_class = beta != 0.0 ? 1 : 0;
    if (t_plan_work != prepare_clock.work0 && p->tune_key) tune_store(*p);
    return;
  }

  if (tun(kT_slab_segments) >= 1 && !t_in_slab && !(t_strict_name == kLineEnhance || t_strict_name == kLine || t_strict_name == kFlat)) {
    const int S = tun(kT_slab_segments) == 1 ? seg_auto_slabs(n) : tun(kT_slab_segments) > 16 ? 16 : tun(kT_slab_segments);
    if (last_error_code_only() == kOk && !t_capturing && !ensure_segments(*p, S, st)) {
      (void)hipGetLastError();
      tune_log("m %d nnz %d: slab_segments: the run lists could not be built (%s), ordinary path", m, p->A.nnz, last_error_string());
      clear_error();
      p->free_segments();
      p->seg_state = 0;
    }
    if (p->seg_state == 1) {
      run_segments(st, *p, alpha, beta, dx, dy);
      if (t_plan_work != prepare_clock.work0 && p->tune_key) tune_store(*p);
      return;
    }
  }


  const long long avg = static_cast<long long>(p->A.count()) / m;
  auto resident_blocks = [&]() {
    int cus = 0;
    if (hipDeviceGetAttribute(&cus, hipDeviceAttributeMultiprocessorCount, p->device) != hipSuccess || cus <= 0) cus = 256;
    (void)hipGetLastError();
    return cus * 8;
  };
  if (strategy == kLight) {
    if (!p->d_light_counter) {
      if (!plan_work_allowed("LIGHT's row counter")) return;
      ++t_plan_work;
      if (!hip_ok(hipMalloc(reinterpret_cast<void **>(&p->d_light_counter), 2 * sizeof(unsigned)), "hipMalloc light counter") ||
          !hip_ok(hipMemsetAsync(p->d_light_counter, 0, 2 * sizeof(unsigned), st), "memset light counter") ||
          !hip_ok(hipStreamSynchronize(st), "sync light counter"))
        return;
    }
    launch_light(st, p->A, classic_vec(avg), resident_blocks(), p->d_light_counter, alpha, beta, dx, dy);
    p->last_kernel = kKernelLight;
    strategy = -1;
  } else if (strategy == kBlockRowOrdinary) {
    launch_block_row(st, p->A, resident_blocks(), alpha, beta, dx, dy);
    p->last_kernel = kKernelBlockRow;
    strategy = -1;
  }
  switch (strategy) {
  case -1:
    break;
  case kVectorRow:
  {
    const int forced_w = tun(kT_vector_width);
    const bool tile_form = tun(kT_vector_tile) != 0;
    const int w = (forced_w >= 1 && forced_w <= 64 && (forced_w & (forced_w - 1)) == 0) ? forced_w
                  : tile_form ? tile_vec(avg) : classic_vec(avg);
    if (tun(kT_rowblock_guard) && !probe_rowblock(*p, kThreads / w, st)) return;
    if (tile_form && p->rowblock_ok == 0) {
      run_plus(st, *p, h_rowptr, alpha, beta, dx, dy);
    } else if (tile_form && p->rowblock_ok != 0) {
      const double a = static_cast<double>(p->A.count()) / m;
      auto launch = [&](int pol, double al, double be, double *yy) {
        launch_vector_tile(st, p->A, m, w, w, a, a, kVectorTarget, tun(kT_xcd_chunk), pol, al, be, dx, yy,
                           next_reverse(*p));
      };
      if (!autotune_policy(*p, kFamVector, st, [&](int pol, double *ys) { launch(pol, 1.0, trial_beta(), ys); })) return;
      launch(policy_for(*p, kFamVector), alpha, beta, dy);
      p->last_kernel = kKernelVectorTile;
    } else {
      launch_vector_row(st, p->A, m, w, 1, alpha, beta, dx, dy, p->rowblock_ok == 0);
      p->last_kernel = kKernelVectorRow;
    }
    break;
  }
  case kWfRow:
    launch_wave_row(st, p->A, alpha, beta, dx, dy);
    p->last_kernel = kKernelWaveRow;
    break;
  case kDefault:
    run_rowblock(st, *p, h_rowptr, alpha, beta, dx, dy, true);
    break;
  case kThreadRow:
    run_rowblock(st, *p, h_rowptr, alpha, beta, dx, dy, false, 1);
    break;
  case kLineEnhance:
  case kLine:
    run_rowblock(st, *p, h_rowptr, alpha, beta, dx, dy);
    break;
  case kFlat:
    run_flat(st, *p, alpha, beta, dx, dy);
    break;
  case kAdaptive: {
    if (!fetch_samples(*p, h_rowptr)) return;
    if (tun(kT_adaptive_timed) && !tun(kT_adaptive_split) && !tun(kT_deterministic)) {
      run_adaptive_timed(st, *p, h_rowptr, alpha, beta, dx, dy);
      break;
    }
    switch (adaptive_branch(m, p->samples)) {
    case 1:
      if (tun(kT_adaptive_split)) {
        const int half_rows = m / 2;
        const long long a0 = half_rows > 0 ? p->samples.half / half_rows : 0;
        const long long a1 = (static_cast<long long>(p->samples.last) - p->samples.half) / (m - half_rows);
        if (tun(kT_vector_tile)) {
          const double f0 = half_rows > 0 ? static_cast<double>(p->samples.half) / half_rows : 0.0;
          const double f1 = (static_cast<double>(p->samples.last) - p->samples.half) / (m - half_rows);
          launch_vector_tile(st, p->A, half_rows, tile_vec(a0), tile_vec(a1), f0, f1, kVectorTarget,
                             tun(kT_xcd_chunk), policy_for(*p, kFamVector), alpha, beta, dx, dy);
        } else {
          launch_vector_row(st, p->A, half_rows, classic_vec(a0), classic_vec(a1), alpha, beta, dx, dy);
        }
      } else {
        run_plus(st, *p, h_rowptr, alpha, beta, dx, dy);
      }
      break;
    default:
      if (quarters_uneven(p->samples) && !tun(kT_adaptive_split)) run_plus(st, *p, h_rowptr, alpha, beta, dx, dy);
      else run_rowblock(st, *p, h_rowptr, alpha, beta, dx, dy, true);
      break;
    }
    break;
  }
  case kAdaptivePlus:
    run_plus(st, *p, h_rowptr, alpha, beta, dx, dy);
    break;
  default:
    set_error(kErrUnknownStrategy, "unknown strategy id");
    break;
  }
  if (t_plan_work != prepare_clock.work0 && p->tune_key) tune_store(*p);
  const hipError_t launch_err = hipGetLastError();
  if (launch_err != hipSuccess && last_error_code_only() == kOk)
    set_error(kErrHip, std::string("kernel launch failed: ") + hipGetErrorString(launch_err));
}
}
// ... 3 lines not shown
```

spmv_acc_amd/csrc/engine.hpp:

```cpp
#pragma once

#include <hip/hip_runtime_api.h>

#include <string>
#include <vector>

#include "kernels.hpp"

namespace spmv_acc {

enum Strategy {
  kDefault = 0,
  kAdaptive = 1,
  kThreadRow = 2,
  kWfRow = 3,
  kBlockRowOrdinary = 4,
  kLight = 5,
  kVectorRow = 6,
  kLineEnhance = 7,
  kLine = 8,
  kFlat = 9,
  kAdaptivePlus = 10,
  kStrategyCount = 11
};

enum Error {
  kOk = 0,
  kErrUnsupportedTrans = 1,
  kErrBadArgument = 2,
  kErrHip = 3,
  kErrTooLarge = 4,
  kErrUnknownStrategy = 5,
  kErrNoDevice = 6
};

const char *strategy_name(int s);
int parse_strategy(const char *name);

void set_error(int code, const std::string &what);
int last_error();
const char *last_error_string();
void clear_error();

int set_tunable(const char *name, int value);
int get_tunable(const char *name);
void reset_tunables();

struct UnboundedTuningScope {
  UnboundedTuningScope();
  ~UnboundedTuningScope();
};

double last_prepare_us();

void set_stream(hipStream_t s);
hipStream_t get_stream();

int active_strategy();
int set_active_strategy(int s);

struct FlatSegmentSumScope {
  FlatSegmentSumScope();
  ~FlatSegmentSumScope();
  bool prev;
};

struct RowptrSamples {
  int q1 = 0;
  int half = 0;
  int q3 = 0;
  int last = 0;
};

int adaptive_branch(int m, const RowptrSamples &s);

int plus_analyze_host(int m, int min_nnz_per_block, int threads_per_block, int vec_size, const int *host_row_ptr,
                      std::vector<int> &break_points, std::vector<int> &first_block_of_row);
int plus_analyze_device(int m, int min_nnz_per_block, int threads_per_block, int vec_size, const int *d_rowptr,
                        int *d_break_points, int bp_cap, int *d_first_block_of_row);
int plus_pick_vec(int m, int nnz);
int plus_pick_vec_tuned(int m, int nnz, int min_nnz);

void run_spmv(int strategy, int trans, double alpha, double beta, int m, int n, int nnz, const int *h_rowptr,
              const int *d_rowptr, const int *d_colindex, const double *d_value, const double *dx, double *dy,
              const double *dy_in = nullptr);

int run_spmm(int layout, int k, double alpha, double beta, int m, int n, int nnz, const int *h_rowptr, const int *d_rowptr, const int *d_colindex,
             const double *d_value, const double *dX, long long ldx, double *dY, long long ldy);
void release_plans(const int *d_rowptr, int m_only = -1);
void kernel_clock_begin();
void kernel_clock_set(bool on);
void kernel_clock_release();
size_t kernel_clock_used();
bool kernel_clock_failed();
hipEvent_t kernel_clock_event(size_t i);

struct PlanInfo {
  int nnz = 0;
  int adaptive_branch = 0;
  int vec = 0;
  int flat_tiles = 0;
  int plus_blocks = 0;
  int aligned16 = 0;
  int stream_policy = -1;
  int flat_fixup = -1;
  int adaptive_family = -1;
  int adaptive_family_beta0 = -1;
  int slab_passes = 0;
  int last_kernel = -1;
  int col16 = -1;
  int settled = 0;
};
bool query_plan(const int *d_rowptr, int m, PlanInfo *out);
unsigned plan_work_count();
int cached_plan_count();
void set_tune_cache(const char *path);
int refresh_values(const int *d_rowptr);
int check_plans();

}
```

spmv_acc_amd/csrc/engine_internal.hpp:

```cpp
#pragma once

#include "engine.hpp"

#include <hip/hip_runtime.h>

#include <algorithm>
#include <atomic>
#include <chrono>
#include <climits>
#include <cstdarg>
#include <cstdio>
#include <cstdint>
#include <cstdlib>
#include <cstring>
#include <deque>
#include <map>
#include <memory>
#include <mutex>
#include <string>
#include <tuple>

#include <vector>

#include "kernels.hpp"

namespace spmv_acc {
namespace detail {

extern thread_local hipStream_t t_stream;
void note_stream_use();
extern std::mutex g_mu;
bool hip_ok(hipError_t e, const char *what);
int last_error_code_only();
extern thread_local double t_last_prepare_us;
extern thread_local unsigned t_plan_work;
extern const char *const kStaleText;
inline bool stream_capturing(hipStream_t st) {
  hipStreamCaptureStatus cap = hipStreamCaptureStatusNone;
  const bool capturing = hipStreamIsCapturing(st, &cap) == hipSuccess && cap != hipStreamCaptureStatusNone;
  (void)hipGetLastError();
  return capturing;
}
template <typename T> struct ScopedSet {
  T &ref;
  const T old;
  ScopedSet(T &r, T value) : ref(r), old(r) { ref = value; }
  ~ScopedSet() { ref = old; }
  ScopedSet(const ScopedSet &) = delete;
  ScopedSet &operator=(const ScopedSet &) = delete;
};
struct Tunable {
  const char *name;
  int def;
  int val;
};
enum TunableId {
  kT_xcd_chunk, kT_rowblock_vec, kT_rowblock_target, kT_stream_plain, 
  kT_rowblock_guard, kT_adaptive_timed, kT_adaptive_split, 
  kT_plus_min_nnz, kT_plus_host_analysis, kT_flat_finish, kT_flat_npt, kT_validate, kT_rowlen, kT_flat_early, kT_vector_tile, kT_col16, kT_vector_width, kT_zigzag, kT_cache_ends_mb, kT_flat_reduce, kT_gather_hint, kT_hint_budget_kb, kT_deterministic, kT_col_slabs, kT_flat_rowblock, kT_guard_full, kT_slab_segments, kT_first_call_budget, kT_later_call_budget, kT_slab_whole_below, kT_strict_strategy, kT_slab_kb, kT_hint_min_x_mb, kT_max_grid_blocks, kT_flat_small_nnz_k, kTunableCount
};
extern Tunable g_tunables[];
void apply_env_tunables();
extern thread_local bool t_rule_twin;
inline int tun(TunableId id) {
  if (id == kT_deterministic) return (t_rule_twin || g_tunables[id].val > 0) ? 1 : 0;
  return g_tunables[id].val;
}
inline bool rule_until_settled() { return g_tunables[kT_deterministic].val == 0; }
bool quarters_uneven(const RowptrSamples &s);
int classic_vec(long long avg);
int tile_vec(long long avg);

int guard_acquire(int device, const int **d_guard, int **h_flag);
void guard_release(int device, int slot, bool launched, hipStream_t last_stream);
enum Family { kFamRowblock = 0, kFamPlus = 1, kFamFlat = 2, kFamVector = 3, kFamilyCount = 4 };
enum LastKernel { kKernelRowblock = 0, kKernelPlus = 1, kKernelFlatTile = 2, kKernelSlabPasses = 3, kKernelVectorTile = 4, kKernelVectorRow = 5,
                  kKernelWaveRow = 6, kKernelLight = 7, kKernelBlockRow = 8, kKernelColSlabs = 9, kKernelScaleOnly = 10 };
extern thread_local int t_strict_name;

typedef std::tuple<int, const void *, const void *, const void *, int, int, int> PlanKey;

struct Plan {
  int device = 0;
  PlanKey key;
  hipStream_t last_stream = nullptr;
  hipEvent_t order_event = nullptr;
  bool launched = false;
  unsigned long long last_use = 0;
  std::mutex mu;
  unsigned long long calls = 0;
  unsigned launches = 0;
  double trial_ms = 0.0;
  int last_c16 = -1;
  int last_kernel = -1;
  bool tuning_open = true;
  bool captured = false;
  unsigned settled_for[2] = {0, 0};
  CsrDev A;
  int guard_slot = -1;
  bool have_samples = false;
  RowptrSamples samples;
  int stream_policy[kFamilyCount][2] = {{-1, -1}, {-1, -1}, {-1, -1}, {-1, -1}};
  int invalid = -1;
  int rowblock_ok = -1;
  int rowblock_rpb = 0;
  int rb_target = 0;
  int max_block_nnz = 0;
  bool rowblock_uneven = false;
  int adaptive_family[2] = {-1, -1};
  float adaptive_ms[2][3] = {{1e30f, 1e30f, 1e30f}, {1e30f, 1e30f, 1e30f}};
  bool adaptive_provisional[2] = {false, false};
  bool adaptive_skipped[2][3] = {{false, false, false}, {false, false, false}};
  RowDigest digest;
  int flat_tiles = -1;
  FlatPlan flat;
  Col16 col16;
  int c16_use[kFamilyCount] = {-1, -1, -1, -1};
  int flat_npt_choice = 0;
  bool flat_geometry_tuned = false;
  int flat_rowblock_choice = -1;
  bool flat_early_choice = false;
  int flat_mode_choice[2] = {-1, -1};
  unsigned long long tune_key = 0;
  unsigned *d_light_counter = nullptr;
  static constexpr int kDigestSlots = 8;
  bool have_rp_digest = false;
  unsigned long long rp_digest = 0;
  unsigned long long *d_digest_acc = nullptr;
  unsigned digest_turn = 0;
  int slab_count = 0;
  int slab_width = 0;
  int slab_copy_choice = -1;
  unsigned long long *d_value_samples = nullptr;
  int *h_values_changed = nullptr;
  int value_samples = 0;
  unsigned values_refreshed = 0;
  long long *d_slab_off = nullptr;
  std::vector<int *> slab_rowid, slab_crp;
  std::vector<int> slab_rows;
  double *d_slab_ys = nullptr;
  int *d_slab_rp = nullptr;
  int *d_slab_ci = nullptr;
  double *d_slab_v = nullptr;
  std::vector<long long> slab_off;
  int plus_blocks = -1;
  int plus_vec = 0;
  int plus_min = 0;
  int plus_tuned_min = 0;
  bool plus_has_long = false;
  int hint_state = -1;
  unsigned char *d_cold = nullptr;
  double hint_hot_share = 0.0;
  int hint_use[kFamilyCount] = {-1, -1, -1, -1};
  int *d_pbp = nullptr;
  int *d_pfbr = nullptr;
  double *d_ppartial = nullptr;
  void *d_pblk = nullptr;
  int spmm_state = -1;
  SpmmLong spmm;
  void free_spmm() {
    for (void *q : {static_cast<void *>(spmm.rows), static_cast<void *>(spmm.first), static_cast<void *>(spmm.piece), static_cast<void *>(spmm.partial)})
      if (q) (void)hipFree(q);
    spmm = SpmmLong();
    spmm_state = -1;
  }

  ~Plan() {
    free_device();
    guard_release(device, guard_slot, launched, last_stream);
  }
  bool is_stale() const { return A.stale && __atomic_load_n(A.stale, __ATOMIC_RELAXED) != 0; }
  void free_col16() {
    if (col16.d16) (void)hipFree(col16.d16);
    if (col16.rec) (void)hipFree(col16.rec);
    if (col16.ovf) (void)hipFree(col16.ovf);
    if (col16.ci_guard) (void)hipFree(col16.ci_guard);
    col16 = Col16();
  }
  void free_digest() {
    if (digest.lens) (void)hipFree(digest.lens);
    if (digest.base) (void)hipFree(digest.base);
    digest = RowDigest();
  }
  void free_slabs();
  int seg_state = -1, seg_slabs = 0;
  int seg_choice = -1;
  bool seg_early_tried = false;
  std::vector<int *> seg_row, seg_begin, seg_vptr, seg_blk, seg_cut;
  std::vector<int> seg_entries, seg_blocks, seg_pieces;
  double *d_seg_ys = nullptr;
  int seg_rest_below = 0;
  int seg_whole_hint = -1;
  void free_segments() {
    seg_rest_below = 0;
    seg_whole_hint = -1;
    for (auto *list : {&seg_row, &seg_begin, &seg_vptr, &seg_blk, &seg_cut}) {
      for (int *q : *list)
        if (q) (void)hipFree(q);
      list->clear();
    }
    seg_entries.clear();
    seg_blocks.clear();
    seg_pieces.clear();
    if (d_seg_ys) (void)hipFree(d_seg_ys);
    d_seg_ys = nullptr;
    seg_state = -1;
    seg_slabs = 0;
  }
  void free_device() {
    if (order_event) (void)hipEventDestroy(order_event);
    order_event = nullptr;
    free_slabs();
    free_segments();
    if (d_light_counter) (void)hipFree(d_light_counter);
    d_light_counter = nullptr;
    if (d_digest_acc) (void)hipFree(d_digest_acc);
    d_digest_acc = nullptr;
    if (d_cold) (void)hipFree(d_cold);
    d_cold = nullptr;
    hint_state = -1;
    free_flat();
    free_digest();
    free_col16();
    free_spmm();
    if (d_pbp) (void)hipFree(d_pbp);
    if (d_pfbr) (void)hipFree(d_pfbr);
    if (d_ppartial) (void)hipFree(d_ppartial);
    if (d_pblk) (void)hipFree(d_pblk);
    d_pblk = nullptr;
    d_ppartial = nullptr;
    d_pbp = d_pfbr = nullptr;
  }
  static void free_flat_plan(FlatPlan &F) {
    if (F.bp) (void)hipFree(F.bp);
    if (F.head) (void)hipFree(F.head);
    if (F.tail) (void)hipFree(F.tail);
    if (F.tail_row) (void)hipFree(F.tail_row);
    if (F.tail_end) (void)hipFree(F.tail_end);
    if (F.digest) (void)hipFree(F.digest);
    F = FlatPlan();
  }
  void free_flat() {
    free_flat_plan(flat);
    flat_tiles = -1;
  }
};

struct TuneRecord {
  int v[26];
  bool operator==(const TuneRecord &o) const { return std::memcmp(v, o.v, sizeof(v)) == 0; }
};
constexpr int kTuneFields = 26;
bool tune_cache_enabled();
void tune_adopt(Plan &p);
void tune_store(const Plan &p);
extern std::map<PlanKey, std::shared_ptr<Plan>> g_plans;
extern thread_local std::weak_ptr<Plan> t_last_plan;
extern thread_local bool t_capturing;
bool plan_work_allowed(const char *what);
bool plan_settled_for(const int *rp, const int *ci, const double *v, int m, int n, int strategy, int cls);
void drop_rule_twin(const int *rp, const int *ci, const double *v, int m, int n);
bool rule_twin_exists(const int *rp, const int *ci, const double *v, int m, int n);
const int *host_view(const int *h);
bool fetch_samples(Plan &p, const int *h_rowptr);
std::shared_ptr<Plan> get_plan(int m, int n, int nnz, const int *h_rowptr, const int *rp, const int *ci, const double *v);
bool report_stale_last_plan();
void drain_deferred_locked();

extern thread_local bool t_flat_segment_sum;
inline bool flat_segment_sum() { return (t_flat_segment_sum || tun(kT_flat_reduce) == 1) && tun(kT_col16) <= 0; }
extern thread_local int t_beta_class;
inline double trial_beta() { return t_beta_class ? 1.0 : 0.0; }
extern thread_local bool t_coarse_tuning;
extern thread_local bool t_no_policy_timing;
extern thread_local bool t_in_slab;
inline bool next_reverse(Plan &p) { return tun(kT_zigzag) && (p.launches++ & 1u); }
constexpr int kRowblockTargetRule = 1800, kRowblockTargetAlt = 1500;
inline int rowblock_target_for(const Plan &p) { return tun(kT_rowblock_target) > 0 ? tun(kT_rowblock_target) : (p.rb_target > 0 ? p.rb_target : kRowblockTargetRule); }
constexpr int kFlatSmallNnz = 24 << 20;
inline long long flat_small_nnz() { return static_cast<long long>(tun(kT_flat_small_nnz_k)) << 10; }
int policy_for(const Plan &p, int fam);
bool tune_log_enabled();
void tune_log(const char *fmt, ...);
double *tune_scratch(size_t len);
void release_tune_scratch();
bool build_flat_plan(const CsrDev &A, int stride, hipStream_t stream, FlatPlan &F);
int flat_stride_for(const Plan &p);
bool ensure_flat(Plan &p, hipStream_t stream);
int analyze_on_device(hipStream_t st, const int *d_rowptr, int m, int min_nnz, int threads, int vec, int **d_bp, int **d_fbr);
bool ensure_plus(Plan &p, const int *h_rowptr, hipStream_t stream, int min_nnz);
bool ensure_col16(Plan &p, hipStream_t st);
bool ensure_hint(Plan &p, hipStream_t st);
bool ensure_slabs(Plan &p, int S, hipStream_t st);
bool ensure_segments(Plan &p, int S_cols, hipStream_t st);
void launch_flat_plan(hipStream_t st, const CsrDev &A, FlatPlan &F, int policy, double alpha, double beta, const double *x, double *y, bool reverse);
void launch_flat_with(hipStream_t st, Plan &p, int policy, double alpha, double beta, const double *x, double *y);
bool autotune_flat_mode(Plan &p, hipStream_t st, const double *x);
bool autotune_flat_geometry(Plan &p, hipStream_t st, const double *x);

extern thread_local std::chrono::steady_clock::time_point t_call_began;
extern thread_local double t_budget_spmvs;
extern thread_local double t_budget_ms;
extern thread_local bool t_tuning_deferred;
extern thread_local float t_first_trial_ms;
extern thread_local int t_unbounded_tuning;
inline bool defer_tuning() {
  if (t_budget_spmvs <= 0.0 || t_budget_ms < 0.0) return false;
  const double spent = std::chrono::duration<double, std::milli>(std::chrono::steady_clock::now() - t_call_began).count();
  if (spent < 0.5 * t_budget_ms) return false;
  t_tuning_deferred = true;
  return true;
}
inline bool by_rule() { return tun(kT_deterministic) != 0 || defer_tuning(); }
inline double budget_spent_fraction() {
  if (t_budget_spmvs <= 0.0 || t_budget_ms <= 0.0) return 0.0;
  return std::chrono::duration<double, std::milli>(std::chrono::steady_clock::now() - t_call_began).count() / t_budget_ms;
}

struct TuneTimer {
  static constexpr int kMaxTimed = 5;
  hipEvent_t e0 = nullptr, e1 = nullptr;
  hipEvent_t per[2 * kMaxTimed] = {};
  void *reset_ptr = nullptr;
  size_t reset_bytes = 0;
  bool ok = false;
  TuneTimer() {
// ... 195 lines not shown
```

spmv_acc_amd/csrc/k_col16.hip:

```cpp
#include <climits>

#include <rocprim/device/device_scan.hpp>

#include "device_utils.hpp"
#include "kernels.hpp"

namespace spmv_acc {
namespace {

using namespace dev;

constexpr int kChunk = kCol16Chunk;

__global__ __launch_bounds__(kThreads) void col16_base_kernel(const int *__restrict__ ci, int nnz, int chunk0, int nchunks,
                                                              int *__restrict__ base, int *__restrict__ esc_count,
                                                              unsigned long long *__restrict__ stats) {
  const int lane = threadIdx.x & (kWave - 1);
  const long long c_ll = static_cast<long long>(blockIdx.x) * (kThreads / kWave) + threadIdx.x / kWave;
  if (c_ll >= nchunks) return;
  const int c = static_cast<int>(c_ll);
  const long long j0 = (static_cast<long long>(chunk0) + c) * kChunk + 4 * lane;
  int col[4];
#pragma unroll
  for (int e = 0; e < 4; ++e) col[e] = (j0 + e < nnz) ? ci[j0 + e] : INT_MAX;
  int lo0 = col[0] < col[1] ? col[0] : col[1], hi0 = col[0] < col[1] ? col[1] : col[0];
  int lo1 = col[2] < col[3] ? col[2] : col[3], hi1 = col[2] < col[3] ? col[3] : col[2];
  const int smallest = lo0 < lo1 ? lo0 : lo1;
  int second = lo0 < lo1 ? (hi0 < lo1 ? hi0 : lo1) : (hi1 < lo0 ? hi1 : lo0);
  const int mine = second != INT_MAX ? second : smallest;
  int rank = 0;
  for (int l = 0; l < kWave; ++l) {
    const int other = __shfl(mine, l, kWave);
    rank += (other < mine || (other == mine && l < lane)) ? 1 : 0;
  }
  const int valid = __popcll(__ballot(mine != INT_MAX));
  const int want = valid > 0 ? (valid - 1) / 2 : 0;
  const unsigned long long holder = __ballot(rank == want);
  const int src = holder ? __ffsll(static_cast<long long>(holder)) - 1 : 0;
  const int median = __shfl(mine, src, kWave);
  long long b = static_cast<long long>(median) - 32767;
  if (valid == 0 || b < 0) b = 0;
  const int bs = static_cast<int>(b);
  int esc = 0;
#pragma unroll
  for (int e = 0; e < 4; ++e) {
    if (col[e] != INT_MAX) {
      const long long d = static_cast<long long>(col[e]) - bs;
      esc += (d < 0 || d > 65534) ? 1 : 0;
    }
  }
#pragma unroll
  for (int o = 32; o > 0; o >>= 1) esc += __shfl_xor(esc, o, kWave);
  if (lane == 0) {
    base[c] = bs;
    esc_count[c] = esc;
    if (esc > 0) atomicAdd(stats, static_cast<unsigned long long>(esc));
    if (esc > 12) atomicAdd(stats + 1, 1ull);
    if (esc > 28) atomicAdd(stats + 2, 1ull);
    if (esc > 60) atomicAdd(stats + 3, 1ull);
  }
}

__global__ __launch_bounds__(kThreads) void col16_overflow_kernel(int *__restrict__ cnt, int nchunks, int E) {
  const long long c = static_cast<long long>(blockIdx.x) * kThreads + threadIdx.x;
  if (c < nchunks) {
    const int over = cnt[c] - E;
    cnt[c] = over > 0 ? over : 0;
  }
}

__global__ __launch_bounds__(kThreads) void col16_encode_kernel(const int *__restrict__ ci, int nnz, int chunk0, int nchunks,
                                                                const int *__restrict__ base, const int *__restrict__ ovf_start,
                                                                int R, unsigned short *__restrict__ d16, int *__restrict__ rec,
                                                                int *__restrict__ ovf) {
  const int lane = threadIdx.x & (kWave - 1);
  const long long c_ll = static_cast<long long>(blockIdx.x) * (kThreads / kWave) + threadIdx.x / kWave;
  if (c_ll >= nchunks) return;
  const int c = static_cast<int>(c_ll);
  const long long j0 = (static_cast<long long>(chunk0) + c) * kChunk + 4 * lane;
  const int bs = base[c];
  const int E = R - 4;
  int col[4];
  bool is_esc[4];
  int mine = 0;
#pragma unroll
  for (int e = 0; e < 4; ++e) {
    col[e] = (j0 + e < nnz) ? ci[j0 + e] : bs;
    const long long d = static_cast<long long>(col[e]) - bs;
    is_esc[e] = d < 0 || d > 65534;
    mine += is_esc[e] ? 1 : 0;
  }
  int incl = mine;
#pragma unroll
  for (int o = 1; o < kWave; o <<= 1) {
    const int up = __shfl_up(incl, o, kWave);
    if (lane >= o) incl += up;
  }
  const int total = __shfl(incl, kWave - 1, kWave);
  int pos = incl - mine;
  int *r = rec + static_cast<size_t>(c) * R;
  const int o0 = ovf_start[c];
  unsigned short out[4];
#pragma unroll
  for (int e = 0; e < 4; ++e) {
    out[e] = 0xFFFF;
    if (is_esc[e]) {
      if (pos < E) r[4 + pos] = col[e];
      else ovf[o0 + pos - E] = col[e];
      ++pos;
    } else {
      out[e] = static_cast<unsigned short>(col[e] - bs);
    }
  }
  unsigned short *dst = d16 + static_cast<size_t>(c) * kChunk + 4 * lane;
#pragma unroll
  for (int e = 0; e < 4; ++e) dst[e] = out[e];
  if (lane == 0) {
    r[0] = bs;
    r[1] = total;
    r[2] = o0;
  }
}

__global__ __launch_bounds__(kWave) void col16_guard_kernel(const int *__restrict__ ci, int lo, int span, int *__restrict__ out) {
  out[threadIdx.x] = ci[lo + static_cast<int>(static_cast<long long>(threadIdx.x) * span / (kWave - 1))];
}

}

size_t col16_scan_bytes(int nchunks) {
  size_t bytes = 0;
  (void)rocprim::exclusive_scan(nullptr, bytes, static_cast<int *>(nullptr), static_cast<int *>(nullptr), 0,
                                static_cast<size_t>(nchunks) + 1, rocprim::plus<int>());
  return bytes;
}

void launch_col16_base(hipStream_t stream, const int *ci, int nnz, int chunk0, int nchunks, int *base, int *esc_count,
                       unsigned long long *stats) {
  if (nchunks <= 0) return;
  const int waves_per_block = kThreads / kWave;
  SPMV_ACC_LAUNCH(col16_base_kernel, dim3((nchunks + waves_per_block - 1) / waves_per_block), dim3(kThreads), 0, stream, ci, nnz,
                     chunk0, nchunks, base, esc_count, stats);
}

void launch_col16_overflow(hipStream_t stream, int *cnt, int nchunks, int E) {
  if (nchunks <= 0) return;
  SPMV_ACC_LAUNCH(col16_overflow_kernel, dim3((nchunks + kThreads - 1) / kThreads), dim3(kThreads), 0, stream, cnt, nchunks, E);
}

bool launch_col16_scan(hipStream_t stream, int nchunks, const int *esc_count, int *esc_start, void *tmp, size_t tmp_bytes) {
  return rocprim::exclusive_scan(tmp, tmp_bytes, esc_count, esc_start, 0, static_cast<size_t>(nchunks) + 1, rocprim::plus<int>(),
                                 stream) == hipSuccess;
}

void launch_col16_encode(hipStream_t stream, const int *ci, int nnz, int chunk0, int nchunks, const int *base, const int *ovf_start,
                         int R, unsigned short *d16, int *rec, int *ovf) {
  if (nchunks <= 0) return;
  const int waves_per_block = kThreads / kWave;
  SPMV_ACC_LAUNCH(col16_encode_kernel, dim3((nchunks + waves_per_block - 1) / waves_per_block), dim3(kThreads), 0, stream, ci, nnz,
                     chunk0, nchunks, base, ovf_start, R, d16, rec, ovf);
}

void launch_col16_guard(hipStream_t stream, const int *ci, int lo, int span, int *out) {
  SPMV_ACC_LAUNCH(col16_guard_kernel, dim3(1), dim3(kWave), 0, stream, ci, lo, span, out);
}

}
```

spmv_acc_amd/csrc/kernels.hpp:

```cpp
#pragma once

#include <hip/hip_runtime_api.h>
#include <hip/hip_ext.h>

namespace spmv_acc {

bool kernel_clock_next(hipEvent_t *start, hipEvent_t *stop);
#define SPMV_ACC_LAUNCH(kernel, grid, block, shmem, stream, ...)                                                                  \
  do {                                                                                                                           \
    hipEvent_t kc_e0_ = nullptr, kc_e1_ = nullptr;                                                                               \
    if (::spmv_acc::kernel_clock_next(&kc_e0_, &kc_e1_))                                                                         \
      hipExtLaunchKernelGGL(kernel, grid, block, shmem, stream, kc_e0_, kc_e1_, 0, __VA_ARGS__);                                 \
    else                                                                                                                         \
      hipLaunchKernelGGL(kernel, grid, block, shmem, stream, __VA_ARGS__);                                                       \
  } while (0)

struct CsrDev {
  int m = 0;
  int n = 0;
  int nnz = 0;
  int nnz0 = 0;
  int count() const { return nnz - nnz0; }
  const int *rp = nullptr;
  const int *ci = nullptr;
  const double *v = nullptr;
  bool aligned16 = false;
  const int *guard = nullptr;
  int *stale = nullptr;
  const unsigned char *cold = nullptr;
  const double *yin = nullptr;
};
inline bool x32_ok(const CsrDev &A) { return A.n > 0 && A.n <= (1 << 29); }
constexpr int kGuardSamples = 64;
void launch_guard_fill(hipStream_t stream, const int *rp, int m, int *d_guard);
void launch_guard_check(hipStream_t stream, const CsrDev &A);
struct SlabBounds {
  int first[15];
};
constexpr int kSegMaxPlanes = 16;
bool launch_segment_count(hipStream_t stream, const CsrDev &A, const SlabBounds &B, int S, int *cnt, int *beg, int *not_monotone, int rest_below = 0);
void launch_segment_pieces(hipStream_t stream, const int *cnt_s, int m, int piece_max, int *pieces);
void launch_segment_compact(hipStream_t stream, const int *cnt_s, const int *beg_s, const int *pos, int m, int piece_max, int *seg_row,
                            int *seg_begin, int *seg_len, int *has_pieces);
void launch_segment_cut_list(hipStream_t stream, const int *cnt_s, const int *pos, int m, int piece_max, int *counter, int *cut);
constexpr int kSegPiece = 512;
void launch_segment_cost(hipStream_t stream, int entries, int *seg_len, int *cost);
int segment_block_count(long long total_cost);
void launch_segment_blocks(hipStream_t stream, int entries, int nblocks, const int *cptr, int *blk_first);
void launch_segment_tiles(hipStream_t stream, int nblocks, double alpha, const int *blk_first, const int *seg_row, const int *seg_begin,
                          const int *vptr, const int *ci, const double *v, const double *x, double *ys, double *y, const unsigned char *cold = nullptr);
void launch_segment_merge(hipStream_t stream, int ncut, const int *cut, int entries, const int *seg_row, const double *ys, double *y);
constexpr int kDigestMaxParts = 1024;
int rowptr_digest_parts(int m);
void launch_rowptr_digest(hipStream_t stream, const int *rp, int m, unsigned long long *part);
void launch_rowptr_verdict(hipStream_t stream, const unsigned long long *part, int m, unsigned long long expected, int *stale,
                           unsigned long long *digest_out);

constexpr int kStreamPolicyNt = 0;
constexpr int kStreamPolicyDefault = 1;
constexpr int kStreamPolicyIndexDefault = 2;
constexpr int kStreamPolicyValueDefault = 3;

constexpr int kThreads = 256;
constexpr int kMaxGridBlocks = 8388593;
int max_grid_blocks();
constexpr int kNnzPerThread = 8;
constexpr int kTile = kThreads * kNnzPerThread;
constexpr int kVectorTarget = 1900;
constexpr int kPlusThreads = 256;
constexpr int kPlusR = 2;
constexpr int kPlusMinNnz = 2 * kPlusR * kPlusThreads;
constexpr int kPlusLongChunk = 2 * kPlusMinNnz;

void launch_vector_row(hipStream_t stream, const CsrDev &A, int row_split, int w0, int w1, double alpha, double beta,
                       const double *x, double *y, bool single_row_groups = false);

void launch_vector_tile(hipStream_t stream, const CsrDev &A, int row_split, int w0, int w1, double avg0, double avg1,
                        int target_products, int xcd_chunk, int stream_policy, double alpha, double beta, const double *x,
                        double *y, bool reverse = false);

void launch_light(hipStream_t stream, const CsrDev &A, int w, int grid_blocks, unsigned *counter, double alpha, double beta, const double *x,
                  double *y);
void launch_block_row(hipStream_t stream, const CsrDev &A, int grid_blocks, double alpha, double beta, const double *x, double *y);

void launch_wave_row(hipStream_t stream, const CsrDev &A, double alpha, double beta, const double *x, double *y);

struct RowDigest {
  int rpb = 0;
  unsigned char *lens = nullptr;
  int *base = nullptr;
};
struct Col16;
void launch_rowblock_stream(hipStream_t stream, const CsrDev &A, int vec, int rows_per_block, int flags,
                            double alpha, double beta, const double *x, double *y, const RowDigest *digest = nullptr,
                            int cache_ends = 0, const Col16 *col16 = nullptr);
void launch_row_digest(hipStream_t stream, const int *rp, int m, int rows_per_block, unsigned char *lens, int *base);
void pick_rowblock_shape(int m, int nnz, int target_products, int *vec, int *rows_per_block);

void launch_max_block_nnz(hipStream_t stream, const int *rp, int m, int rows_per_block, int avg_block, int *d_out);
constexpr int kRowblockMaxRounds = 8;

void launch_break_points(hipStream_t stream, const int *rp, int m, int nnz, int stride, int *bp, int bp_len);

constexpr int kCol16Chunk = 256;
struct Col16 {
  int state = -1;
  int chunk0 = 0;
  int nchunks = 0;
  int rec_ints = 0;
  unsigned short *d16 = nullptr;
  int *rec = nullptr;
  int *ovf = nullptr;
  int *ci_guard = nullptr;
  long long escapes = 0;
  long long overflow = 0;
  size_t bytes = 0;
};
struct Col16Dev {
  const unsigned short *d16;
  const int *rec;
  const int *ovf;
  const int *ci_guard;
  int rec_ints;
  int guard_lo, guard_span;
};
inline Col16Dev col16_dev(const Col16 &C, const CsrDev &A) {
  Col16Dev d;
  d.d16 = C.d16 - static_cast<long long>(C.chunk0) * kCol16Chunk;
  d.rec = C.rec - static_cast<long long>(C.chunk0) * C.rec_ints;
  d.ovf = C.ovf;
  d.ci_guard = C.ci_guard;
  d.rec_ints = C.rec_ints;
  d.guard_lo = A.nnz0;
  d.guard_span = A.count() > 0 ? A.count() - 1 : 0;
  return d;
}
constexpr int kHintLineShift = 4;
constexpr int kHintBins = 4096;
constexpr int kHintSamples = 8 << 20;
void launch_hint_census(hipStream_t stream, const int *ci, int nnz, int ncols, int stride, int samples, unsigned *counts);
void launch_hint_hist(hipStream_t stream, const unsigned *counts, int nlines, unsigned *hist_lines, unsigned long long *hist_hits);
void launch_hint_bits(hipStream_t stream, const int *ci, int nnz, int ncols, const unsigned *counts, unsigned threshold, unsigned char *bits);

size_t col16_scan_bytes(int nchunks);
void launch_col16_base(hipStream_t stream, const int *ci, int nnz, int chunk0, int nchunks, int *base, int *esc_count, unsigned long long *stats);
void launch_col16_overflow(hipStream_t stream, int *cnt, int nchunks, int E);
bool launch_col16_scan(hipStream_t stream, int nchunks, const int *esc_count, int *esc_start, void *tmp, size_t tmp_bytes);
void launch_col16_encode(hipStream_t stream, const int *ci, int nnz, int chunk0, int nchunks, const int *base, const int *ovf_start, int R,
                         unsigned short *d16, int *rec, int *ovf);
void launch_col16_guard(hipStream_t stream, const int *ci, int lo, int span, int *out);

struct FlatPlan {
  int stride = 0;
  int ntiles = 0;
  int tile0 = 0;
  int *bp = nullptr;
  double *head = nullptr;
  double *tail = nullptr;
  int *tail_row = nullptr;
  int *tail_end = nullptr;
  void *digest = nullptr;
  int xcd_chunk = 0;
  int stream_policy = 0;
  bool can_finish = false;
  bool needs_fixup = true;
  int max_tile_rows = 0;
  bool early_stream = false;
  bool reverse = false;
  int cache_ends = 0;
  bool segment_sum = false;
  const Col16 *col16 = nullptr;
  bool mode_tuned[2] = {false, false};
  bool tuned_fixup[2] = {true, true};
};
constexpr int kFlatFinish = 128;
void launch_break_points_from(hipStream_t stream, const int *rp, int m, int nnz, int stride, int tile0, int *bp, int bp_len);
void launch_flat_digest(hipStream_t stream, const CsrDev &A, const FlatPlan &P);
void launch_flat_needs_fixup(hipStream_t stream, const CsrDev &A, const FlatPlan &P, int *d_flag);
void launch_flat(hipStream_t stream, const CsrDev &A, const FlatPlan &P, double alpha, double beta, const double *x,
                 double *y);

void launch_plus_digest(hipStream_t stream, const CsrDev &A, const int *bp, const int *fbr, int nblocks, int long_chunk, void *blk,
                        int *d_has_long);
void launch_plus(hipStream_t stream, const CsrDev &A, const int *bp, const int *fbr, const void *blk, int nblocks,
                 bool has_long_rows, int xcd_chunk, int stream_policy, double *partial, double alpha, double beta,
                 const double *x, double *y, bool reverse = false);

size_t plus_analyze_device_workspace_bytes(int m);
bool plus_analyze_device_count(hipStream_t stream, const int *rp, int m, int min_nnz, int threads_per_block,
                               int vec_size, void *workspace, int *d_total);
void plus_analyze_device_emit(hipStream_t stream, const int *rp, int m, int min_nnz, const void *workspace, int *d_bp,
                              int *d_fbr);

void launch_slab_count(hipStream_t stream, const CsrDev &A, int width, int S, int *cnt);
void launch_slab_scatter(hipStream_t stream, const CsrDev &A, int width, int S, const int *rps, const long long *off, int *ci_out,
                         double *v_out, bool values_only = false);
void launch_slab_flags(hipStream_t stream, const int *rps, int m, int *flags);
void launch_slab_compact(hipStream_t stream, const int *rps, const int *pos, int m, int *rowid, int *crp);
void launch_slab_merge(hipStream_t stream, int ms, const int *rowid, const double *ys, double *y);
void launch_value_samples(hipStream_t stream, const double *v, const int *ci, long long lo, long long span, int count, unsigned long long *saved, int *changed);
constexpr int kValueSamples = 65536;
constexpr int kSlabCopyAfterCalls = 32;

void launch_stream_copy(hipStream_t stream, void *dst, const void *src, long long bytes, bool non_temporal);

struct SpmmLong {
  int nlong = 0;
  int npieces = 0;
  int *rows = nullptr;
  int *first = nullptr;
  int *piece = nullptr;
  double *partial = nullptr;
};
int spmm_team_lanes(int kp);
void launch_spmm_rows(hipStream_t stream, const CsrDev &A, bool row_major, int kp, long long ldx, long long ldy, double alpha, double beta,
                      const double *x, double *y);
void launch_spmm_long(hipStream_t stream, const CsrDev &A, const SpmmLong &L, bool row_major, int kp, long long ldx, long long ldy, double alpha,
                      double beta, const double *x, double *y);
void launch_spmm_scale(hipStream_t stream, int m, int k, bool row_major, long long ldy, double beta, double *y);

void launch_scale_y(hipStream_t stream, int m, double beta, double *y, const double *yin = nullptr);
void launch_validate_csr(hipStream_t stream, const CsrDev &A, int *d_flags);

}
```

spmv_acc_amd/csrc/plan.cpp:

```cpp
#include "engine_internal.hpp"

namespace spmv_acc {
using namespace detail;

namespace detail {

constexpr int kGuardSlots = 4096;
struct GuardPool {
  int *d_guard = nullptr;
  int *h_flags = nullptr;
  std::deque<std::pair<int, hipEvent_t>> free_slots;
  bool failed = false;
};
std::mutex g_guard_mu;
std::map<int, GuardPool> g_guard_pools;

int guard_acquire(int device, const int **d_guard, int **h_flag) {
  std::lock_guard<std::mutex> lk(g_guard_mu);
  GuardPool &P = g_guard_pools[device];
  if (P.failed) return -1;
  if (!P.d_guard) {
    if (hipMalloc(reinterpret_cast<void **>(&P.d_guard), sizeof(int) * kGuardSlots * kGuardSamples) != hipSuccess ||
        hipHostMalloc(reinterpret_cast<void **>(&P.h_flags), sizeof(int) * kGuardSlots,
                      hipHostMallocCoherent | hipHostMallocMapped | hipHostMallocPortable) != hipSuccess) {
// ... 327 lines not shown
              "spmv_acc_release_plans: the results of the EARLIER calls made on it since the change are invalid; the plan has "
              "been rebuilt, so the call that reports this ran on the matrix as it is now and its y is valid");
    erase_with_sibling_locked(key);
    it = g_plans.end();
  }
  if (it != g_plans.end()) {
    if (nnz < 0 || nnz == it->second->A.nnz) {
      it->second->last_use = ++g_use_clock;
      return it->second;
    }
    if (!plan_work_allowed("rebuilding the plan of a matrix whose nnz changed")) return nullptr;
    erase_with_sibling_locked(key);
  }
  if (!plan_work_allowed("building the plan of a matrix seen for the first time")) return nullptr;
  if (!t_rule_twin && g_plans.size() >= kMaxPlans) {
    size_t primaries = 0;
    auto oldest = g_plans.end();
    for (auto jt = g_plans.begin(); jt != g_plans.end(); ++jt) {
      if (std::get<6>(jt->first) != 0) continue;
      ++primaries;
      if (oldest == g_plans.end() || jt->second->last_use < oldest->second->last_use) oldest = jt;
    }
    if (primaries >= kMaxPlans && oldest != g_plans.end()) {
      const PlanKey gone = oldest->first;
      erase_with_sibling_locked(gone);
    }
  }
  if (nnz < 0) {
    if ((h_rowptr = host_view(h_rowptr)) != nullptr) {
      nnz = h_rowptr[m];
    } else if (!hip_ok(hipMemcpyAsync(&nnz, rp + m, sizeof(int), hipMemcpyDeviceToHost, t_stream), "read rowptr[m]") ||
               !hip_ok(hipStreamSynchronize(t_stream), "read rowptr[m]")) {
      return nullptr;
    }
  }
  if (nnz < 0 || nnz > INT_MAX - (1 << 16)) {
    set_error(kErrTooLarge, "nnz does not leave room for tile arithmetic in int32; shard the matrix");
    return nullptr;
  }
  std::shared_ptr<Plan> p = std::make_shared<Plan>();
  p->device = dev;
  p->key = key;
  p->A.m = m;
  p->A.n = n;
  p->A.nnz = nnz;
  {
    const int *hv = host_view(h_rowptr);
    int first = 0;
    if (hv) first = hv[0];
    else if (!hip_ok(hipMemcpyAsync(&first, rp, sizeof(int), hipMemcpyDeviceToHost, t_stream), "read rowptr[0]") ||
             !hip_ok(hipStreamSynchronize(t_stream), "read rowptr[0]"))
      return nullptr;
    p->A.nnz0 = (first > 0 && first <= nnz) ? first : 0;
  }
  p->A.rp = rp;
  p->A.ci = ci;
  p->A.v = v;
  p->A.aligned16 = (reinterpret_cast<uintptr_t>(ci) % 16 == 0) && (reinterpret_cast<uintptr_t>(v) % 16 == 0) &&
                   nnz >= 8;
  p->last_use = ++g_use_clock;
  p->guard_slot = guard_acquire(dev, &p->A.guard, &p->A.stale);
  if (p->guard_slot >= 0) {
    launch_guard_fill(t_stream, rp, m, const_cast<int *>(p->A.guard));
    if (!hip_ok(hipStreamSynchronize(t_stream), "record the plan guard")) return nullptr;
    if (tune_cache_enabled() && !tun(kT_deterministic)) {
      int samples[kGuardSamples], col_samples[kGuardSamples] = {};
      bool ok = hipMemcpy(samples, p->A.guard, sizeof(samples), hipMemcpyDeviceToHost) == hipSuccess;
      const long long first = samples[0], extent = static_cast<long long>(samples[kGuardSamples - 1]) - first;
      for (int k = 0; ok && ci && extent > 0 && k < kGuardSamples; ++k)
        ok = hipMemcpy(&col_samples[k], ci + first + k * (extent - 1) / (kGuardSamples - 1), sizeof(int), hipMemcpyDeviceToHost) == hipSuccess;
      if (ok) {
        p->tune_key = tune_key_of(dev, m, n, nnz, samples, col_samples);
        tune_adopt(*p);
      }
      (void)hipGetLastError();
    }
  }
  g_plans[key] = p;
  return p;
}

const char *const kStaleText =
    "the matrix behind a cached plan changed (same pointers and shape, different rowptr) without spmv_acc_release_plans: the "
    "results of the calls made on it since the change -- including the calling thread's most recent SpMV on these pointers -- "
    "are invalid; the plan has been dropped and the next call on the matrix rebuilds it";

bool report_stale_last_plan() {
  const std::shared_ptr<Plan> p = t_last_plan.lock();
  if (!p || !p->is_stale()) return false;
  set_error(kErrBadArgument, kStaleText);
  t_last_plan.reset();
  std::lock_guard<std::mutex> lk(g_mu);
  auto it = g_plans.find(p->key);
  if (it != g_plans.end() && it->second == p) erase_with_sibling_locked(p->key);
  return true;
}
}

int check_plans() {
  std::lock_guard<std::mutex> lk(g_mu);
  int dropped = 0;
  std::vector<PlanKey> gone;
  for (auto &kv : g_plans) {
    if (!kv.second->is_stale()) continue;
    PlanKey k = kv.first;
    std::get<6>(k) = 0;
    if (std::find(gone.begin(), gone.end(), k) == gone.end()) gone.push_back(k);
  }
  for (const PlanKey &k : gone) {
    erase_with_sibling_locked(k);
    ++dropped;
  }
  if (dropped) set_error(kErrBadArgument, kStaleText);
  return dropped;
}


void release_plans(const int *d_rowptr, int m_only) {
  std::lock_guard<std::mutex> lk(g_mu);
  for (auto it = g_plans.begin(); it != g_plans.end();) {
    if (!d_rowptr || (std::get<1>(it->first) == d_rowptr && (m_only < 0 || std::get<4>(it->first) == m_only))) {
      it = g_plans.erase(it);
    } else {
      ++it;
    }
  }
  drain_deferred_locked();
}

bool query_plan(const int *d_rowptr, int m, PlanInfo *out) {
  std::lock_guard<std::mutex> lk(g_mu);
  for (auto &kv : g_plans) {
    if (std::get<1>(kv.first) == d_rowptr && std::get<4>(kv.first) == m && std::get<6>(kv.first) == 0) {
      const Plan &p = *kv.second;
      out->nnz = p.A.nnz;
      out->adaptive_branch = p.have_samples ? adaptive_branch(m, p.samples) : 0;
      int rb_vec = 1, rb_rows = kThreads;
      pick_rowblock_shape(m, p.A.count(), rowblock_target_for(p), &rb_vec, &rb_rows);
      out->vec = rb_vec;
      out->flat_tiles = p.flat_tiles;
      out->plus_blocks = p.plus_blocks;
      out->aligned16 = p.A.aligned16 ? 1 : 0;
      const int afam = p.adaptive_family[1] >= 0 ? p.adaptive_family[1] : p.adaptive_family[0];
      int fam = afam;
      for (int f = 0; fam < 0 && f < kFamilyCount; ++f)
        if (p.stream_policy[f][1] >= 0 || p.stream_policy[f][0] >= 0) fam = f;
      out->stream_policy = fam < 0 ? -1 : (p.stream_policy[fam][1] >= 0 ? p.stream_policy[fam][1] : p.stream_policy[fam][0]);
      out->flat_fixup = p.flat_tiles > 0 ? (p.flat.needs_fixup ? 1 : 0) : -1;
      out->adaptive_family = afam;
      out->adaptive_family_beta0 = p.adaptive_family[0];
      out->settled = p.calls > 0 && !p.tuning_open ? 1 : 0;
      out->last_kernel = p.last_kernel;
      out->col16 = p.last_c16;
      out->slab_passes = p.seg_state == 1 && (tun(kT_slab_segments) >= 1 || (tun(kT_slab_segments) < 0 && p.seg_choice == 1)) ? p.seg_slabs - (p.seg_rest_below > 0 ? 1 : 0) : 0;
      return true;
    }
  }
  return false;
}

int cached_plan_count() {
  std::lock_guard<std::mutex> lk(g_mu);
  int n = 0;
  for (auto &kv : g_plans) n += std::get<6>(kv.first) == 0 ? 1 : 0;
  return n;
}

namespace detail {
bool plan_settled_for(const int *rp, const int *ci, const double *v, int m, int n, int strategy, int cls) {
  int dev = 0;
  if (hipGetDevice(&dev) != hipSuccess) return true;
  std::lock_guard<std::mutex> lk(g_mu);
  auto it = g_plans.find(PlanKey(dev, rp, ci, v, m, n, 0));
  if (it == g_plans.end()) return false;
  const Plan &p = *it->second;
  return strategy >= 0 && strategy < 32 && ((p.settled_for[cls & 1] >> strategy) & 1u);
}

bool rule_twin_exists(const int *rp, const int *ci, const double *v, int m, int n) {
  int dev = 0;
  if (hipGetDevice(&dev) != hipSuccess) return false;
  std::lock_guard<std::mutex> lk(g_mu);
  return g_plans.find(PlanKey(dev, rp, ci, v, m, n, 1)) != g_plans.end();
}

void drop_rule_twin(const int *rp, const int *ci, const double *v, int m, int n) {
  int dev = 0;
  if (hipGetDevice(&dev) != hipSuccess) return;
  std::lock_guard<std::mutex> lk(g_mu);
  auto it = g_plans.find(PlanKey(dev, rp, ci, v, m, n, 1));
  if (it != g_plans.end() && !it->second->captured) g_plans.erase(it);
}
}

}
```

spmv_acc_amd/csrc/tile_stage.hpp:

```cpp
#pragma once

#include "device_utils.hpp"
#include "kernels.hpp"

namespace spmv_acc {
namespace dev {

template <int THREADS, int NPT, bool NTC, bool NTV, bool HINT>
__device__ __forceinline__ void stage_products_all(double *__restrict__ lds, int a0, int hi, const int *__restrict__ ci,
                                                   const double *__restrict__ v, const double *__restrict__ x,
                                                   const unsigned char *__restrict__ cold) {
  constexpr int K = NPT / 4;
  int4v c[K];
  double2v va[K], vb[K];
  unsigned nib[K];
#pragma unroll
  for (int k = 0; k < K; ++k) {
    const int j = a0 + 4 * (threadIdx.x + k * THREADS);
    const int jc = (j < hi) ? j : a0;
    c[k] = load_stream_i4<NTC>(ci + jc);
    va[k] = load_stream_d2<NTV>(v + jc);
    vb[k] = load_stream_d2<NTV>(v + jc + 2);
    if (HINT) nib[k] = static_cast<unsigned>(cold[jc >> 3]) >> (jc & 4);
  }
// ... 9 lines not shown
    } else {
      xg[k][0] = gather_u32(x, c[k].x);
      xg[k][1] = gather_u32(x, c[k].y);
      xg[k][2] = gather_u32(x, c[k].z);
      xg[k][3] = gather_u32(x, c[k].w);
    }
  }
#pragma unroll
  for (int k = 0; k < K; ++k) {
    const int g = threadIdx.x + k * THREADS;
    double2v p0, p1;
    p0.x = va[k].x * xg[k][0];
    p0.y = va[k].y * xg[k][1];
    p1.x = vb[k].x * xg[k][2];
    p1.y = vb[k].y * xg[k][3];
    double2v *dst = reinterpret_cast<double2v *>(lds + 4 * g);
    dst[0] = p0;
    dst[1] = p1;
  }
}

template <int THREADS, int NPT, bool NTC, bool NTV, bool HINT>
__device__ __forceinline__ void stage_products_tail(double *__restrict__ lds, int a0, int hi, const int *__restrict__ ci,
                                                    const double *__restrict__ v, const double *__restrict__ x,
                                                    const unsigned char *__restrict__ cold) {
  const XGather xr = make_xgather(x, HINT);
#pragma nounroll
  for (int k = 0; k < NPT / 4 - 1; ++k) {
    const int wave_j = __builtin_amdgcn_readfirstlane(a0 + 4 * ((threadIdx.x & ~(kWave - 1)) + k * THREADS));
    if (wave_j >= hi) break;
    const int g = threadIdx.x + k * THREADS;
    const int j = a0 + 4 * g;
    const int jc = (j < hi) ? j : a0;
    const int4v c = load_stream_i4<NTC>(ci + jc);
    const double2v va = load_stream_d2<NTV>(v + jc), vb = load_stream_d2<NTV>(v + jc + 2);
    double xg[4];
    if (HINT) {
      const unsigned nib = static_cast<unsigned>(cold[jc >> 3]) >> (jc & 4);
      xg[0] = gather_hinted(xr, c.x, nib & 1u);
      xg[1] = gather_hinted(xr, c.y, nib & 2u);
      xg[2] = gather_hinted(xr, c.z, nib & 4u);
      xg[3] = gather_hinted(xr, c.w, nib & 8u);
    } else {
      xg[0] = gather_u32(x, c.x);
      xg[1] = gather_u32(x, c.y);
      xg[2] = gather_u32(x, c.z);
      xg[3] = gather_u32(x, c.w);
    }
    double2v p0, p1;
    p0.x = va.x * xg[0];
    p0.y = va.y * xg[1];
    p1.x = vb.x * xg[2];
    p1.y = vb.y * xg[3];
    double2v *dst = reinterpret_cast<double2v *>(lds + 4 * g);
    dst[0] = p0;
    dst[1] = p1;
  }
}

template <int THREADS, int NPT, bool NTC = true, bool NTV = true, bool HINT = false>
__device__ __forceinline__ void stage_products(double *__restrict__ lds, int a0, int hi, int nnz,
                                               const int *__restrict__ ci, const double *__restrict__ v,
                                               const double *__restrict__ x, bool allow_fast = true,
                                               const unsigned char *__restrict__ cold = nullptr, bool x32 = false) {
  static_assert(NPT % 4 == 0, "NPT must be a multiple of 4");
  constexpr int K = NPT / 4;
  if (allow_fast && x32 && ((hi + 3) & ~3) <= nnz) {
    const int last_j = __builtin_amdgcn_readfirstlane(a0 + 4 * ((threadIdx.x & ~(kWave - 1)) + (K - 1) * THREADS));
    if (last_j < hi) stage_products_all<THREADS, NPT, NTC, NTV, HINT>(lds, a0, hi, ci, v, x, cold);
    else stage_products_tail<THREADS, NPT, NTC, NTV, HINT>(lds, a0, hi, ci, v, x, cold);
    return;
  }
#pragma nounroll
  for (int k = 0; k < K; ++k) {
    const int g = threadIdx.x + k * THREADS;
    const int j = a0 + 4 * g;
    if (j < hi && j + 4 <= nnz) {
      const int4v c = load_stream_i4<NTC>(ci + j);
      const double2v va = load_stream_d2<NTV>(v + j), vb = load_stream_d2<NTV>(v + j + 2);
      double2v p0, p1;
      p0.x = va.x * x[c.x];
      p0.y = va.y * x[c.y];
      p1.x = vb.x * x[c.z];
      p1.y = vb.y * x[c.w];
      double2v *dst = reinterpret_cast<double2v *>(lds + 4 * g);
      dst[0] = p0;
      dst[1] = p1;
    } else if (j < hi) {
#pragma unroll
      for (int e = 0; e < 4; ++e) {
        if (j + e < nnz) lds[4 * g + e] = v[j + e] * x[ci[j + e]];
      }
    }
  }
}

__device__ __forceinline__ bool stage_fast_ok(int hi, int nnz) { return ((hi + 3) & ~3) <= nnz; }

template <int NPT> struct StreamRegs {
  int4v c[NPT / 4];
  double2v va[NPT / 4], vb[NPT / 4];
  bool has[NPT / 4];
};

template <int THREADS, int NPT, bool NTC, bool NTV>
__device__ __forceinline__ void stage_issue(StreamRegs<NPT> &R, int a0, int hi, const int *__restrict__ ci,
                                            const double *__restrict__ v) {
#pragma unroll
  for (int k = 0; k < NPT / 4; ++k) {
    const int wave_j = __builtin_amdgcn_readfirstlane(a0 + 4 * ((threadIdx.x & ~(kWave - 1)) + k * THREADS));
    R.has[k] = wave_j < hi;
    if (R.has[k]) {
      const int j = a0 + 4 * (threadIdx.x + k * THREADS);
      const int jc = (j < hi) ? j : a0;
      R.c[k] = load_stream_i4<NTC>(ci + jc);
      R.va[k] = load_stream_d2<NTV>(v + jc);
      R.vb[k] = load_stream_d2<NTV>(v + jc + 2);
    }
  }
}

template <int THREADS, int NPT>
__device__ __forceinline__ void stage_finish(double *__restrict__ lds, const StreamRegs<NPT> &R, const double *__restrict__ x) {
  constexpr int K = NPT / 4;
  double xg[K][4];
#pragma unroll
  for (int k = 0; k < K; ++k) {
    if (R.has[k]) {
      xg[k][0] = x[R.c[k].x];
      xg[k][1] = x[R.c[k].y];
      xg[k][2] = x[R.c[k].z];
      xg[k][3] = x[R.c[k].w];
    }
  }
#pragma unroll
  for (int k = 0; k < K; ++k) {
    if (R.has[k]) {
      const int g = threadIdx.x + k * THREADS;
      double2v p0, p1;
      p0.x = R.va[k].x * xg[k][0];
      p0.y = R.va[k].y * xg[k][1];
      p1.x = R.vb[k].x * xg[k][2];
      p1.y = R.vb[k].y * xg[k][3];
      double2v *dst = reinterpret_cast<double2v *>(lds + 4 * g);
      dst[0] = p0;
      dst[1] = p1;
    }
  }
}

typedef unsigned int uint2v __attribute__((ext_vector_type(2)));
typedef uint2v uint2v_a2 __attribute__((aligned(2)));

__device__ __forceinline__ void c16_decode(int (&c)[4], const uint2v d, int rv, int R, int lane, const int *__restrict__ ovf) {
  const int bs = __builtin_amdgcn_readlane(rv, 0);
  const int nesc = __builtin_amdgcn_readlane(rv, 1);
  const int dq[4] = {static_cast<int>(d.x & 0xFFFFu), static_cast<int>(d.x >> 16), static_cast<int>(d.y & 0xFFFFu), static_cast<int>(d.y >> 16)};
#pragma unroll
  for (int q = 0; q < 4; ++q) c[q] = bs + dq[q];
  if (nesc > 0) {
    const int E = R - 4;
    const unsigned long long lt = (1ull << lane) - 1ull;
    const bool e[4] = {dq[0] == 0xFFFF, dq[1] == 0xFFFF, dq[2] == 0xFFFF, dq[3] == 0xFFFF};
    const unsigned long long slot[4] = {__ballot(e[0]), __ballot(e[1]), __ballot(e[2]), __ballot(e[3])};
    int r = __popcll(slot[0] & lt) + __popcll(slot[1] & lt) + __popcll(slot[2] & lt) + __popcll(slot[3] & lt);
#pragma unroll
    for (int q = 0; q < 4; ++q) {
      if (slot[q]) {
        const int got = __shfl(rv, (4 + r) & (kWave - 1), kWave);
        if (e[q]) c[q] = r < E ? got : ovf[__builtin_amdgcn_readlane(rv, 2) + r - E];
      }
      r += e[q] ? 1 : 0;
    }
  }
}

template <int THREADS, int NPT, bool NTC, bool NTV>
__device__ __forceinline__ void stage_products_c16_all(double *__restrict__ lds, int a0, int lo4, int hi, const Col16Dev &C,
                                                       const double *__restrict__ v, const double *__restrict__ x) {
  constexpr int K = NPT / 4;
  uint2v d[K];
  double2v va[K], vb[K];
  int rv[K];
  const int lane = threadIdx.x & (kWave - 1);
  const int R = C.rec_ints;
  const int rl = lane < R ? lane : 0;
#pragma unroll
  for (int k = 0; k < K; ++k) {
    const int wave_j = __builtin_amdgcn_readfirstlane(a0 + 4 * ((threadIdx.x & ~(kWave - 1)) + k * THREADS));
    rv[k] = C.rec[static_cast<long long>(wave_j >> 8) * R + rl];
  }
#pragma unroll
  for (int k = 0; k < K; ++k) {
    const int j = a0 + 4 * (threadIdx.x + k * THREADS);
    const uint2v_a2 *p = reinterpret_cast<const uint2v_a2 *>(C.d16 + j);
    d[k] = NTC ? __builtin_nontemporal_load(p) : *p;
  }
#pragma unroll
  for (int k = 0; k < K; ++k) {
    const int j = a0 + 4 * (threadIdx.x + k * THREADS);
    const int jv = (j >= lo4 && j < hi) ? j : lo4;
    va[k] = load_stream_d2<NTV>(v + jv);
    vb[k] = load_stream_d2<NTV>(v + jv + 2);
  }
  double xg[K][4];
#pragma unroll
  for (int k = 0; k < K; ++k) {
    const int j = a0 + 4 * (threadIdx.x + k * THREADS);
    int c[4];
    c16_decode(c, d[k], rv[k], R, lane, C.ovf);
    const bool mine = j >= lo4 && j < hi;
    const int bs = __builtin_amdgcn_readlane(rv[k], 0);
#pragma unroll
    for (int q = 0; q < 4; ++q) xg[k][q] = gather_u32(x, mine ? c[q] : bs);
  }
#pragma unroll
  for (int k = 0; k < K; ++k) {
    const int g = threadIdx.x + k * THREADS;
    double2v p0, p1;
    p0.x = va[k].x * xg[k][0];
    p0.y = va[k].y * xg[k][1];
    p1.x = vb[k].x * xg[k][2];
    p1.y = vb[k].y * xg[k][3];
    double2v *dst = reinterpret_cast<double2v *>(lds + 4 * g);
    dst[0] = p0;
    dst[1] = p1;
  }
}

template <int THREADS, int NPT, bool NTC, bool NTV>
__device__ __forceinline__ void stage_products_c16_tail(double *__restrict__ lds, int a0, int lo4, int hi, const Col16Dev &C,
                                                        const double *__restrict__ v, const double *__restrict__ x) {
  const int lane = threadIdx.x & (kWave - 1);
  const int R = C.rec_ints;
  const int rl = lane < R ? lane : 0;
#pragma nounroll
  for (int k = 0; k < NPT / 4 - 1; ++k) {
    const int wave_j = __builtin_amdgcn_readfirstlane(a0 + 4 * ((threadIdx.x & ~(kWave - 1)) + k * THREADS));
    if (wave_j >= hi) break;
    const int g = threadIdx.x + k * THREADS;
    const int j = a0 + 4 * g;
    const int rv = C.rec[static_cast<long long>(wave_j >> 8) * R + rl];
    const uint2v_a2 *p = reinterpret_cast<const uint2v_a2 *>(C.d16 + j);
    const uint2v d = NTC ? __builtin_nontemporal_load(p) : *p;
    const int jv = (j >= lo4 && j < hi) ? j : lo4;
    const double2v va = load_stream_d2<NTV>(v + jv), vb = load_stream_d2<NTV>(v + jv + 2);
    int c[4];
    c16_decode(c, d, rv, R, lane, C.ovf);
    const bool mine = j >= lo4 && j < hi;
    const int bs = __builtin_amdgcn_readlane(rv, 0);
    double xg[4];
#pragma unroll
    for (int q = 0; q < 4; ++q) xg[q] = gather_u32(x, mine ? c[q] : bs);
    double2v p0, p1;
    p0.x = va.x * xg[0];
    p0.y = va.y * xg[1];
    p1.x = vb.x * xg[2];
    p1.y = vb.y * xg[3];
    double2v *dst = reinterpret_cast<double2v *>(lds + 4 * g);
    dst[0] = p0;
    dst[1] = p1;
  }
}

template <int THREADS, int NPT, bool NTC, bool NTV>
__device__ __forceinline__ void stage_products_c16(double *__restrict__ lds, int a0, int lo4, int hi, const Col16Dev &C,
                                                   const double *__restrict__ v, const double *__restrict__ x) {
  const int last_j = __builtin_amdgcn_readfirstlane(a0 + 4 * ((threadIdx.x & ~(kWave - 1)) + (NPT / 4 - 1) * THREADS));
  if (last_j < hi) stage_products_c16_all<THREADS, NPT, NTC, NTV>(lds, a0, lo4, hi, C, v, x);
  else stage_products_c16_tail<THREADS, NPT, NTC, NTV>(lds, a0, lo4, hi, C, v, x);
}

__device__ __forceinline__ void check_ci_guard(const int *__restrict__ ci, const Col16Dev &C, int *__restrict__ stale) {
  if (C.ci_guard != nullptr && stale != nullptr && blockIdx.x == 0 && threadIdx.x < kWave) {
    const int idx = C.guard_lo + static_cast<int>(static_cast<long long>(threadIdx.x) * C.guard_span / (kWave - 1));
    if (ci[idx] != C.ci_guard[threadIdx.x]) __hip_atomic_store(stale, 1, __ATOMIC_RELAXED, __HIP_MEMORY_SCOPE_SYSTEM);
  }
}

constexpr int kTileSpans = 64;
template <int N> struct TileSpansN {
  int n;
  int lo[N], hi[N];
  double sum[N];
};
typedef TileSpansN<kTileSpans> TileSpans;
typedef TileSpansN<32> TileSpans2K;

template <int THREADS, class Spans>
__device__ __forceinline__ double tile_row_sum(const double *__restrict__ lds, Spans &sh, int lo, int hi, int lane, int w) {
  const int span = hi - lo;
  const bool posted = w < kWave && span >= 64 && span > 16 * w;
  int slot = -1;
  double s = 0.0;
  if (posted) {
    if (lane == 0) {
      slot = atomicAdd(&sh.n, 1);
      sh.lo[slot] = lo;
      sh.hi[slot] = hi;
    }
  } else {
    int j = lo + lane;
    for (; j + 3 * w < hi; j += 4 * w) {
      const double a = lds[j], b = lds[j + w], c = lds[j + 2 * w], d = lds[j + 3 * w];
      s += a;
      s += b;
      s += c;
      s += d;
    }
    for (; j < hi; j += w) s += lds[j];
  }
  const int n = __syncthreads_count(posted && lane == 0);
  if (n > 0) {
    const int wave = threadIdx.x / kWave, l = threadIdx.x & (kWave - 1);
    for (int e = wave; e < n; e += THREADS / kWave) {
      double t = 0.0;
      const int b = sh.hi[e];
      for (int j = sh.lo[e] + l; j < b; j += kWave) t += lds[j];
      t = group_sum<64>(t);
      if (l == 0) sh.sum[e] = t;
    }
    __syncthreads();
    if (slot >= 0) s = sh.sum[slot];
    __syncthreads();
    if (threadIdx.x == 0) sh.n = 0;
    __syncthreads();
  }
  return s;
}

template <int THREADS, int R, class Spans>
__device__ __forceinline__ void tile_rows_sum(const double *__restrict__ lds, Spans &sh, const int (&lo)[R], const int (&hi)[R],
                                              int lane, int w, double (&acc)[R]) {
  int slot[R];
  bool posted_any = false;
#pragma unroll
  for (int k = 0; k < R; ++k) {
    const int span = hi[k] - lo[k];
    const bool posted = w < kWave && span >= 64 && span > 16 * w;
    slot[k] = -1;
    if (posted) {
      if (lane == 0) {
        slot[k] = atomicAdd(&sh.n, 1);
        sh.lo[slot[k]] = lo[k];
        sh.hi[slot[k]] = hi[k];
        posted_any = true;
      }
    } else {
      for (int j = lo[k] + lane; j < hi[k]; j += w) acc[k] += lds[j];
    }
  }
  if (__syncthreads_count(posted_any) > 0) {
    const int n = sh.n;
    const int wave = threadIdx.x / kWave, l = threadIdx.x & (kWave - 1);
    for (int e = wave; e < n; e += THREADS / kWave) {
      double t = 0.0;
      const int b = sh.hi[e];
      for (int j = sh.lo[e] + l; j < b; j += kWave) t += lds[j];
      t = group_sum<64>(t);
      if (l == 0) sh.sum[e] = t;
    }
    __syncthreads();
#pragma unroll
    for (int k = 0; k < R; ++k)
      if (slot[k] >= 0) acc[k] += sh.sum[slot[k]];
    __syncthreads();
    if (threadIdx.x == 0) sh.n = 0;
    __syncthreads();
  }
}

}
}
```

spmv_acc_amd/csrc/tuner.cpp:

```cpp
#include "engine_internal.hpp"

namespace spmv_acc {
using namespace detail;

namespace detail {

bool build_flat_plan(const CsrDev &A, int stride, hipStream_t stream, FlatPlan &F) {
  if (!plan_work_allowed("flat: break points and tile digests")) return false;
  ++t_plan_work;
  Plan::free_flat_plan(F);
  const int nnz = A.nnz;
  const int tile0 = A.nnz0 / stride;
  const int tiles = nnz / stride + (nnz % stride ? 1 : 0) - tile0;
  const size_t n1 = static_cast<size_t>(tiles) + 1;
  if (!hip_ok(hipMalloc(reinterpret_cast<void **>(&F.bp), sizeof(int) * n1), "hipMalloc break points") ||
      !hip_ok(hipMalloc(reinterpret_cast<void **>(&F.head), sizeof(double) * n1), "hipMalloc head carries") ||
      !hip_ok(hipMalloc(reinterpret_cast<void **>(&F.tail), sizeof(double) * n1), "hipMalloc tail carries") ||
      !hip_ok(hipMalloc(reinterpret_cast<void **>(&F.tail_row), sizeof(int) * n1), "hipMalloc tail rows") ||
      !hip_ok(hipMalloc(reinterpret_cast<void **>(&F.tail_end), sizeof(int) * n1), "hipMalloc tail ends") ||
      !hip_ok(hipMalloc(&F.digest, 16 * n1), "hipMalloc tile digest")) {
    Plan::free_flat_plan(F);
    return false;
  }
  F.stride = stride;
// ... 105 lines not shown
  (void)hipFree(tbp);
  (void)hipFree(tfbr);
  return rc;
}

namespace detail {

bool ensure_plus(Plan &p, const int *h_rowptr, hipStream_t stream, int min_nnz) {
  if (min_nnz < 256 || min_nnz > kTile) min_nnz = kPlusMinNnz;
  const int want_vec =
      plus_pick_vec_tuned(p.A.m, p.A.count(), min_nnz);
  if (p.plus_blocks >= 0 && p.plus_vec == want_vec && p.plus_min == min_nnz) return true;
  if (!plan_work_allowed("row-block analysis")) return false;
  ++t_plan_work;
  auto drop_tables = [&p] {
    if (p.d_pbp) (void)hipFree(p.d_pbp);
    if (p.d_pfbr) (void)hipFree(p.d_pfbr);
    if (p.d_ppartial) (void)hipFree(p.d_ppartial);
    if (p.d_pblk) (void)hipFree(p.d_pblk);
    p.d_pblk = nullptr;
    p.d_pbp = p.d_pfbr = nullptr;
    p.d_ppartial = nullptr;
    p.plus_blocks = -1;
    return false;
  };
  if (p.plus_blocks >= 0) (void)drop_tables();
  const int m = p.A.m;
  const int vec = want_vec;
  int blocks = -1;
  if (tun(kT_plus_host_analysis)) {
    std::vector<int> staged;
    const int *hrp = host_view(h_rowptr);
    if (!hrp) {
      staged.resize(static_cast<size_t>(m) + 1);
      if (!hip_ok(hipMemcpy(staged.data(), p.A.rp, sizeof(int) * (static_cast<size_t>(m) + 1), hipMemcpyDeviceToHost),
                  "stage rowptr for analysis"))
        return false;
      hrp = staged.data();
    }
    std::vector<int> bp, fbr;
    blocks = plus_analyze_host(m, min_nnz, kPlusThreads, vec, hrp, bp, fbr);
    if (!hip_ok(hipMalloc(reinterpret_cast<void **>(&p.d_pbp), sizeof(int) * bp.size()), "hipMalloc plus bp") ||
        !hip_ok(hipMalloc(reinterpret_cast<void **>(&p.d_pfbr), sizeof(int) * fbr.size()), "hipMalloc plus fbr") ||
        !hip_ok(hipMemcpy(p.d_pbp, bp.data(), sizeof(int) * bp.size(), hipMemcpyHostToDevice), "copy plus bp") ||
        !hip_ok(hipMemcpy(p.d_pfbr, fbr.data(), sizeof(int) * fbr.size(), hipMemcpyHostToDevice), "copy plus fbr"))
      return drop_tables();
  } else {
    blocks = analyze_on_device(stream, p.A.rp, m, min_nnz, kPlusThreads, vec, &p.d_pbp, &p.d_pfbr);
    if (blocks < 0) return false;
  }
  int *d_flag = nullptr;
  if (!hip_ok(hipMalloc(reinterpret_cast<void **>(&p.d_ppartial), sizeof(double) * (static_cast<size_t>(blocks) + 1)),
              "hipMalloc plus partial") ||
      !hip_ok(hipMalloc(&p.d_pblk, 16 * (static_cast<size_t>(blocks) + 1)), "hipMalloc plus digest") ||
      !hip_ok(hipMalloc(reinterpret_cast<void **>(&d_flag), sizeof(int)), "hipMalloc plus flag"))
    return drop_tables();
  int has_long = 0;
  bool ok = hip_ok(hipMemsetAsync(d_flag, 0, sizeof(int), stream), "memset plus flag");
  if (ok) {
    launch_plus_digest(stream, p.A, p.d_pbp, p.d_pfbr, blocks, 2 * min_nnz, p.d_pblk, d_flag);
    ok = hip_ok(hipMemcpyAsync(&has_long, d_flag, sizeof(int), hipMemcpyDeviceToHost, stream), "read plus flag") &&
         hip_ok(hipStreamSynchronize(stream), "sync plus digest");
  }
  (void)hipFree(d_flag);
  if (!ok) return drop_tables();
  p.plus_vec = vec;
  p.plus_min = min_nnz;
  p.plus_blocks = blocks;
  p.plus_has_long = has_long != 0;
  return true;
}

thread_local int t_beta_class = 1;

int policy_for(const Plan &p, int fam) {
  const int forced = tun(kT_stream_plain);
  if (forced >= 0) return forced & 3;
  if (tun(kT_deterministic)) return static_cast<long long>(p.A.count()) <= 8LL * p.A.m ? kStreamPolicyNt : kStreamPolicyDefault;
  const int c = t_beta_class;
  if (p.stream_policy[fam][c] >= 0) return p.stream_policy[fam][c];
  for (int f = 0; f < kFamilyCount; ++f)
    if (p.stream_policy[f][c] >= 0) return p.stream_policy[f][c];
  if (p.stream_policy[fam][c ^ 1] >= 0) return p.stream_policy[fam][c ^ 1];
  return static_cast<long long>(p.A.count()) <= 8LL * p.A.m ? kStreamPolicyNt : kStreamPolicyDefault;
}

thread_local std::chrono::steady_clock::time_point t_call_began;
thread_local double t_budget_spmvs = 0.0;
thread_local double t_budget_ms = -1.0;
thread_local bool t_tuning_deferred = false;
thread_local bool t_rule_twin = false;
thread_local float t_first_trial_ms = 0.f;
thread_local int t_unbounded_tuning = 0;
thread_local bool t_coarse_tuning = false;
thread_local bool t_no_policy_timing = false;


bool tune_log_enabled() {
  static const bool on = [] {
    const char *e = std::getenv("SPMV_ACC_TUNE_LOG");
    return e && *e && *e != '0';
  }();
  return on;
}
void tune_log(const char *fmt, ...) {
  if (!tune_log_enabled()) return;
  va_list ap;
  va_start(ap, fmt);
  std::fputs("[spmv_acc tune] ", stderr);
  std::vfprintf(stderr, fmt, ap);
  std::fputc('\n', stderr);
  va_end(ap);
}

thread_local double *t_scratch = nullptr;
thread_local size_t t_scratch_len = 0;
double *tune_scratch(size_t len) {
  if (t_scratch && t_scratch_len >= len) return t_scratch;
  if (t_scratch) (void)hipFree(t_scratch);
  t_scratch = nullptr;
  t_scratch_len = 0;
  if (!hip_ok(hipMalloc(reinterpret_cast<void **>(&t_scratch), sizeof(double) * (len ? len : 1)), "hipMalloc tune y")) {
    t_scratch = nullptr;
    return nullptr;
  }
  t_scratch_len = len;
  return t_scratch;
}
void release_tune_scratch() {
  if (t_scratch) (void)hipFree(t_scratch);
  t_scratch = nullptr;
  t_scratch_len = 0;
}



bool ensure_col16(Plan &p, hipStream_t st) {
  Col16 &C = p.col16;
  if (C.state >= 0) return true;
  if (!plan_work_allowed("the 16-bit column encoding")) return false;
  const CsrDev &A = p.A;
  const int chunk0 = A.nnz0 / (kThreads * kNnzPerThread) * (kThreads * kNnzPerThread / kCol16Chunk);
  const int nchunks = (A.nnz + kCol16Chunk - 1) / kCol16Chunk - chunk0;
  if (!x32_ok(A) || nchunks < 64) {
    C.state = 0;
    return true;
  }
  ++t_plan_work;
  int *base = nullptr, *cnt = nullptr, *ovf_start = nullptr;
  unsigned long long *stats = nullptr;
  void *tmp = nullptr;
  const size_t tmp_bytes = col16_scan_bytes(nchunks);
  const size_t n1 = static_cast<size_t>(nchunks) + 1;
  bool ok = hip_ok(hipMalloc(reinterpret_cast<void **>(&base), sizeof(int) * n1), "hipMalloc col16 bases") &&
            hip_ok(hipMalloc(reinterpret_cast<void **>(&cnt), sizeof(int) * n1), "hipMalloc col16 escape counts") &&
            hip_ok(hipMalloc(reinterpret_cast<void **>(&ovf_start), sizeof(int) * n1), "hipMalloc col16 overflow offsets") &&
            hip_ok(hipMalloc(reinterpret_cast<void **>(&stats), sizeof(unsigned long long) * 4), "hipMalloc col16 statistics") &&
            hip_ok(hipMalloc(&tmp, tmp_bytes > 0 ? tmp_bytes : 16), "hipMalloc col16 scan workspace") &&
            hip_ok(hipMemsetAsync(cnt + nchunks, 0, sizeof(int), st), "memset col16") &&
            hip_ok(hipMemsetAsync(stats, 0, sizeof(unsigned long long) * 4, st), "memset col16 statistics");
  unsigned long long h_stats[4] = {0, 0, 0, 0};
  int R = 0, total = 0;
  if (ok) {
    launch_col16_base(st, A.ci, A.nnz, chunk0, nchunks, base, cnt, stats);
    ok = hip_ok(hipMemcpyAsync(h_stats, stats, sizeof(h_stats), hipMemcpyDeviceToHost, st), "read col16 statistics") &&
         hip_ok(hipStreamSynchronize(st), "sync col16 statistics");
  }
  if (ok) {
    const unsigned long long limit = static_cast<unsigned long long>(nchunks) / 100;
    R = h_stats[1] <= limit ? 16 : (h_stats[2] <= limit ? 32 : (h_stats[3] <= limit ? 64 : 0));
    const int forced = tun(kT_col16) > 1 ? tun(kT_col16) : 0;
    if (forced == 16 || forced == 32 || forced == 64) R = forced;
    tune_log("m %d nnz %d 16-bit columns: %llu escapes in %d chunks, %llu / %llu / %llu chunks above 12 / 28 / 60 -> %s", A.m, A.nnz, h_stats[0], nchunks,
             h_stats[1], h_stats[2], h_stats[3], R ? (R == 16 ? "16-int records" : (R == 32 ? "32-int records" : "64-int records")) : "not encoded");
  }
  if (ok && R > 0) {
    launch_col16_overflow(st, cnt, nchunks, R - 4);
    ok = launch_col16_scan(st, nchunks, cnt, ovf_start, tmp, tmp_bytes) &&
         hip_ok(hipMemcpyAsync(&total, ovf_start + nchunks, sizeof(int), hipMemcpyDeviceToHost, st), "read col16 overflow total") &&
         hip_ok(hipStreamSynchronize(st), "sync col16");
    const size_t d16_bytes = sizeof(unsigned short) * static_cast<size_t>(nchunks) * kCol16Chunk;
    const size_t rec_bytes = sizeof(int) * static_cast<size_t>(nchunks) * R;
    const size_t ovf_bytes = sizeof(int) * (static_cast<size_t>(total) + 64);
    ok = ok && hip_ok(hipMalloc(reinterpret_cast<void **>(&C.d16), d16_bytes), "hipMalloc col16 offsets") &&
         hip_ok(hipMalloc(reinterpret_cast<void **>(&C.rec), rec_bytes), "hipMalloc col16 records") &&
         hip_ok(hipMalloc(reinterpret_cast<void **>(&C.ovf), ovf_bytes), "hipMalloc col16 overflow list") &&
         hip_ok(hipMalloc(reinterpret_cast<void **>(&C.ci_guard), sizeof(int) * kGuardSamples), "hipMalloc col16 guard") &&
         hip_ok(hipMemsetAsync(C.rec, 0, rec_bytes, st), "memset col16 records") && hip_ok(hipMemsetAsync(C.ovf, 0, ovf_bytes, st), "memset col16 overflow");
    if (ok) {
      launch_col16_encode(st, A.ci, A.nnz, chunk0, nchunks, base, ovf_start, R, C.d16, C.rec, C.ovf);
      launch_col16_guard(st, A.ci, A.nnz0, A.count() > 0 ? A.count() - 1 : 0, C.ci_guard);
      ok = hip_ok(hipStreamSynchronize(st), "sync col16 encode");
    }
    C.bytes = d16_bytes + rec_bytes + ovf_bytes;
  }
  for (void *q : {static_cast<void *>(base), static_cast<void *>(cnt), static_cast<void *>(ovf_start), static_cast<void *>(stats), tmp})
    if (q) (void)hipFree(q);
  if (!ok) {
    p.free_col16();
    return false;
  }
  if (R == 0) {
    p.free_col16();
    C.state = 0;
    return true;
  }
  C.state = 1;
  C.chunk0 = chunk0;
  C.nchunks = nchunks;
  C.rec_ints = R;
  C.escapes = static_cast<long long>(h_stats[0]);
  C.overflow = total;
  return true;
}


void launch_flat_plan(hipStream_t st, const CsrDev &A, FlatPlan &F, int policy, double alpha, double beta, const double *x,
                      double *y, bool reverse) {
  F.xcd_chunk = tun(kT_xcd_chunk);
  F.stream_policy = policy;
  const int early = tun(kT_flat_early);
  if (early >= 0) F.early_stream = early != 0;
  F.reverse = reverse;
  F.cache_ends = tun(kT_cache_ends_mb) > 0 && tun(kT_zigzag) ? static_cast<int>(tun(kT_cache_ends_mb) * 1048576.0 / (12.0 * F.stride)) : 0;
  launch_flat(st, A, F, alpha, beta, x, y);
}
void launch_flat_with(hipStream_t st, Plan &p, int policy, double alpha, double beta, const double *x, double *y) {
  p.flat.segment_sum = flat_segment_sum();
  launch_flat_plan(st, p.A, p.flat, policy, alpha, beta, x, y, next_reverse(p));
}

bool autotune_flat_mode(Plan &p, hipStream_t st, const double *x) {
  FlatPlan &F = p.flat;
  const int forced = tun(kT_flat_finish);
  if (!F.can_finish || F.ntiles <= 1) {
    F.needs_fixup = !F.can_finish;
    return true;
  }
  if (forced >= 0) {
    F.needs_fixup = forced == 0;
    return true;
  }
  if (tun(kT_deterministic)) {
    F.needs_fixup = false;
    return true;
  }
  const int cls = t_beta_class;
  if (F.mode_tuned[cls]) {
    F.needs_fixup = F.tuned_fixup[cls];
    return true;
  }
  if (!t_capturing && defer_tuning()) {
    F.needs_fixup = false;
    return true;
  }
  if (t_capturing) {
    F.needs_fixup = F.mode_tuned[cls ^ 1] ? F.tuned_fixup[cls ^ 1] : false;
    return true;
  }
  if (t_coarse_tuning && p.A.count() >= flat_small_nnz()) {
    F.needs_fixup = true;
    return true;
  }
  TimingPhase ph(st, p.A.m);
  bool ok = ph.ok;
  float ms[2] = {0.f, 0.f};
  for (int mode = 0; ok && mode < 2; ++mode) {
    F.needs_fixup = mode == 0;
    ok = ph.time([&] { launch_flat_with(st, p, policy_for(p, kFamFlat), 1.0, trial_beta(), x, ph.y); }, &ms[mode]);
  }
  F.tuned_fixup[cls] = F.needs_fixup = !(ok && ms[1] < ms[0]);
  F.mode_tuned[cls] = ok;
  if (ok) p.flat_mode_choice[cls] = F.tuned_fixup[cls] ? 1 : 0;
  if (ok) tune_log("m %d nnz %d beta class %d flat cut rows: carries + fix-up %.2f us, finished in the tile %.2f us", p.A.m, p.A.nnz, cls, ms[0] * 1e3f, ms[1] * 1e3f);
  return ok;
}

bool autotune_flat_geometry(Plan &p, hipStream_t st, const double *x) {
  if (p.flat_geometry_tuned || tun(kT_col16) > 0 || flat_segment_sum() || t_capturing || by_rule()) return true;
  if (p.A.count() >= flat_small_nnz() || p.flat.ntiles <= 1) {
    p.flat_geometry_tuned = true;
    return true;
  }
  const bool time_npt = tun(kT_flat_npt) < 0, time_early = tun(kT_flat_early) < 0;
  if (!time_npt && !time_early) return true;
  TimingPhase ph(st, p.A.m);
  bool ok = ph.ok;
  const int pol = policy_for(p, kFamFlat);
  FlatPlan alt;
  FlatPlan *plans[2] = {&p.flat, nullptr};
  if (ok && time_npt) {
    const int other = p.flat.stride == kThreads * 4 ? kThreads * kNnzPerThread : kThreads * 4;
    ok = build_flat_plan(p.A, other, st, alt);
    if (ok) {
      alt.needs_fixup = alt.tuned_fixup[0] = alt.tuned_fixup[1] = !alt.can_finish;
      alt.mode_tuned[0] = alt.mode_tuned[1] = true;
      plans[1] = &alt;
    }
  }
  float best = 1e30f;
  int best_plan = 0;
  bool best_early = false;
  for (int k = 0; ok && k < 2; ++k) {
    if (!plans[k]) continue;
    for (int e = 0; ok && e < (time_early ? 2 : 1); ++e) {
      plans[k]->early_stream = time_early ? e != 0 : plans[k]->early_stream;
      float ms = 0.f;
      ok = ph.time([&] { launch_flat_plan(st, p.A, *plans[k], pol, 1.0, trial_beta(), x, ph.y, next_reverse(p)); }, &ms);
      if (ok) tune_log("m %d nnz %d flat geometry: %d non-zeros per tile, stream-first %d -> %.2f us", p.A.m, p.A.nnz, plans[k]->stride,
                       plans[k]->early_stream ? 1 : 0, ms * 1e3f);
      if (ok && ms < best) {
        best = ms;
        best_plan = k;
        best_early = plans[k]->early_stream;
      }
    }
  }
  if (ok) {
    if (best_plan == 1) {
      Plan::free_flat_plan(p.flat);
      p.flat = alt;
      alt = FlatPlan();
      p.flat_tiles = p.flat.ntiles;
    }
    p.flat.early_stream = p.flat_early_choice = best_early;
    p.flat_npt_choice = p.flat.stride / kThreads;
    p.flat_geometry_tuned = true;
    for (int c = 0; c < 2; ++c) p.flat_mode_choice[c] = p.flat.mode_tuned[c] ? (p.flat.tuned_fixup[c] ? 1 : 0) : -1;
  }
  Plan::free_flat_plan(alt);
  return ok;
}

bool ensure_hint(Plan &p, hipStream_t st) {
  if (p.hint_state >= 0) return true;
  const int mode = tun(kT_gather_hint);
  p.hint_state = 0;
  const CsrDev &A = p.A;
  if (mode == 0 || A.count() < 8 || A.n <= 0 || static_cast<long long>(A.n) * 8 >= (1LL << 32)) return true;
  if (mode < 0 && static_cast<long long>(A.n) * 8 < (static_cast<long long>(tun(kT_hint_min_x_mb)) << 20)) return true;
  ++t_plan_work;
  const auto census_t0 = std::chrono::steady_clock::now();
  const int nlines = (A.n + (1 << kHintLineShift) - 1) >> kHintLineShift;
  const int stride = ((A.count() + kHintSamples - 1) / kHintSamples) | 1;
  const int samples = (A.count() + stride - 1) / stride;
  unsigned *counts = nullptr, *hist_lines = nullptr;
  unsigned long long *hist_hits = nullptr;
  std::vector<unsigned> h_lines(kHintBins);
  std::vector<unsigned long long> h_hits(kHintBins);
  auto optional_alloc = [](void **ptr, size_t bytes) {
    if (hipMalloc(ptr, bytes) == hipSuccess) return true;
    (void)hipGetLastError();
    *ptr = nullptr;
    return false;
  };
  if (!optional_alloc(reinterpret_cast<void **>(&counts), sizeof(unsigned) * static_cast<size_t>(nlines)) ||
      !optional_alloc(reinterpret_cast<void **>(&hist_lines), sizeof(unsigned) * kHintBins) ||
      !optional_alloc(reinterpret_cast<void **>(&hist_hits), sizeof(unsigned long long) * kHintBins)) {
    if (counts) (void)hipFree(counts);
    if (hist_lines) (void)hipFree(hist_lines);
    if (hist_hits) (void)hipFree(hist_hits);
    return true;
  }
  bool ok = hip_ok(hipMemsetAsync(counts, 0, sizeof(unsigned) * static_cast<size_t>(nlines), st), "memset hint census") &&
// ... 264 lines not shown
```

Before: 546.0.

## Add 8-bit column offset encoding option for compressed column index streams

Extends the per-chunk column compression so it can store column offsets as 8-bit codes instead of 16-bit ones. The plan picks 8-bit when escapes stay rare. The base-analysis kernel now computes escape statistics for both widths, using block-level shared tallies to cut global atomics. The decode path in the tile stage is templated on code width, which halves index bytes streamed from HBM for matrices with tightly clustered columns. The cost is more escape-record lookups and added branching, and the selection heuristic may pick 8-bit where the extra escapes hurt.

Result: faster. 571.2 (median of 6 runs) (+4.6%).

```diff
diff --git a/include/spmv_acc.h b/include/spmv_acc.h
--- a/include/spmv_acc.h
+++ b/include/spmv_acc.h
@@ -104,6 +104,7 @@
 int spmv_acc_query_plan_slab_passes(const int *d_rowptr, int m);
 int spmv_acc_query_plan_settled(const int *d_rowptr, int m);
 int spmv_acc_query_plan_col16(const int *d_rowptr, int m);
+int spmv_acc_query_plan_col_bits(const int *d_rowptr, int m);
 enum spmv_acc_kernel {
   SPMV_ACC_KERNEL_ROWBLOCK = 0,
   SPMV_ACC_KERNEL_ROWBLOCK_PLUS = 1,
diff --git a/spmv_acc_amd/__init__.py b/spmv_acc_amd/__init__.py
--- a/spmv_acc_amd/__init__.py
+++ b/spmv_acc_amd/__init__.py
@@ -25,7 +25,7 @@
     "spmv_acc_set_stream", "spmv_acc_get_stream", "spmv_acc_last_error", "spmv_acc_last_error_string",
     "spmv_acc_clear_error", "spmv_acc_time_spmv", "spmv_acc_version", "spmv_acc_set_tunable",
     "spmv_acc_get_tunable", "spmv_acc_reset_tunables", "spmv_acc_time_spmv_total", "spmv_acc_copy_ceiling_gbs", "spmv_acc_adaptive_plus_analyze_device", "spmv_acc_prepare",
-    "spmv_acc_last_prepare_us", "spmv_acc_sharded_spmv", "spmv_acc_shard_prepare", "spmv_acc_csr_spmv_chunks", "spmv_acc_query_plan_settled", "spmv_acc_query_plan_col16", "spmv_acc_time_spmv_cold", "spmv_acc_csr_spmv_oop", "spmv_acc_check_plans",
+    "spmv_acc_last_prepare_us", "spmv_acc_sharded_spmv", "spmv_acc_shard_prepare", "spmv_acc_csr_spmv_chunks", "spmv_acc_query_plan_settled", "spmv_acc_query_plan_col16", "spmv_acc_query_plan_col_bits", "spmv_acc_time_spmv_cold", "spmv_acc_csr_spmv_oop", "spmv_acc_check_plans",
     "spmv_acc_query_plan_beta0", "spmv_acc_query_plan_slab_passes", "spmv_acc_shard_create", "spmv_acc_shard_step", "spmv_acc_shard_pipeline",
     "spmv_acc_shard_destroy", "spmv_acc_rccl_comm_init_all", "spmv_acc_rccl_comm_destroy", "spmv_acc_set_tune_cache",
     "spmv_acc_prepare_beta", "spmv_acc_time_spmv_events", "spmv_acc_refresh_values", "spmv_acc_time_spmv_region", "spmv_acc_query_plan_last_kernel", "spmv_acc_time_spmv_kernels",
@@ -104,6 +104,7 @@
     lib.spmv_acc_query_plan_slab_passes.argtypes = [vp, ci]
     lib.spmv_acc_query_plan_settled.argtypes = [vp, ci]
     lib.spmv_acc_query_plan_col16.argtypes = [vp, ci]
+    lib.spmv_acc_query_plan_col_bits.argtypes = [vp, ci]
     lib.spmv_acc_query_plan_last_kernel.argtypes = [vp, ci]
     lib.spmv_acc_shard_create.argtypes = [ctypes.POINTER(vp), vp, ci, ci, ci, ci, ci, vp, vp, vp, ci]
     lib.spmv_acc_shard_step.argtypes = [vp, cd, cd, vp, vp, vp]
@@ -450,6 +451,7 @@
     info["slab_passes"] = max(0, int(load_library().spmv_acc_query_plan_slab_passes(_ptr(rowptr), m)))
     info["settled"] = int(load_library().spmv_acc_query_plan_settled(_ptr(rowptr), m)) == 1
     info["col16"] = int(load_library().spmv_acc_query_plan_col16(_ptr(rowptr), m))
+    info["col_bits"] = int(load_library().spmv_acc_query_plan_col_bits(_ptr(rowptr), m))
     info["last_kernel"] = KERNEL_NAMES.get(int(load_library().spmv_acc_query_plan_last_kernel(_ptr(rowptr), m)), "none")
     return info
 
diff --git a/spmv_acc_amd/csrc/c_api.cpp b/spmv_acc_amd/csrc/c_api.cpp
--- a/spmv_acc_amd/csrc/c_api.cpp
+++ b/spmv_acc_amd/csrc/c_api.cpp
@@ -378,6 +378,10 @@
 int spmv_acc_query_plan_col16(const int *d_rowptr, int m) {
   PlanInfo info;
   return query_plan(d_rowptr, m, &info) ? info.col16 : -2;
+}
+int spmv_acc_query_plan_col_bits(const int *d_rowptr, int m) {
+  PlanInfo info;
+  return query_plan(d_rowptr, m, &info) ? info.col_bits : -2;
 }
 int spmv_acc_query_plan_settled(const int *d_rowptr, int m) {
   PlanInfo info;
diff --git a/spmv_acc_amd/csrc/dispatch.cpp b/spmv_acc_amd/csrc/dispatch.cpp
--- a/spmv_acc_amd/csrc/dispatch.cpp
+++ b/spmv_acc_amd/csrc/dispatch.cpp
@@ -63,6 +63,7 @@
   launch_flat_with(st, p, policy_for(p, kFamFlat), alpha, beta, x, y);
   p.last_kernel = kKernelFlatTile;
   p.last_c16 = c16 && p.flat.stride == kThreads * kNnzPerThread && p.A.cold == nullptr ? c16->rec_ints : 0;
+  p.last_col_bits = p.last_c16 > 0 ? c16->bits : 0;
   return true;
 }
 
@@ -273,6 +274,7 @@
   launch_rowblock_stream(st, p.A, vec, rpb, base_flags | (policy_for(p, kFamRowblock) << 4) | zz, alpha, beta, x, y, dg, cache_ends, c16);
   p.last_kernel = kKernelRowblock;
   p.last_c16 = c16 && p.A.cold == nullptr ? c16->rec_ints : 0;
+  p.last_col_bits = p.last_c16 > 0 ? c16->bits : 0;
   return true;
 }
 
@@ -671,13 +673,14 @@
   }
   const auto began = std::chrono::steady_clock::now();
   const int err_before = last_error_code_only();
-  int served_kernel = -1, served_c16 = 0;
+  int served_kernel = -1, served_c16 = 0, served_col_bits = 0;
   {
     ScopedSet twin(t_rule_twin, true);
     run_spmv_call(strategy, trans, alpha, beta, m, n, nnz, h_rowptr, d_rowptr, d_colindex, d_value, dx, dy, dy_in);
     if (const std::shared_ptr<Plan> tp = t_last_plan.lock()) {
       served_kernel = tp->last_kernel;
       served_c16 = tp->last_c16;
+      served_col_bits = tp->last_col_bits;
     }
   }
   if (last_error_code_only() != err_before && last_error_code_only() != kOk && last_error_code_only() != kErrUnsupportedTrans) return;
@@ -700,6 +703,7 @@
     if (!((p->settled_for[cls] >> strategy) & 1u)) {
       p->last_kernel = served_kernel;
       p->last_c16 = served_c16;
+      p->last_col_bits = served_col_bits;
     }
   }
   if (plan_settled_for(d_rowptr, d_colindex, d_value, m, n, strategy, beta != 0.0 ? 1 : 0)) drop_rule_twin(d_rowptr, d_colindex, d_value, m, n);
@@ -794,6 +798,7 @@
   } yin_scope{p->A};
   p->A.yin = beta != 0.0 ? dy_in : nullptr;
   p->last_c16 = 0;
+  p->last_col_bits = 0;
 
   if (p->A.count() == 0) {
     launch_scale_y(st, m, beta, dy, p->A.yin);
diff --git a/spmv_acc_amd/csrc/engine.hpp b/spmv_acc_amd/csrc/engine.hpp
--- a/spmv_acc_amd/csrc/engine.hpp
+++ b/spmv_acc_amd/csrc/engine.hpp
@@ -109,6 +109,7 @@
   int slab_passes = 0;
   int last_kernel = -1;
   int col16 = -1;
+  int col_bits = -1;
   int settled = 0;
 };
 bool query_plan(const int *d_rowptr, int m, PlanInfo *out);
diff --git a/spmv_acc_amd/csrc/engine_internal.hpp b/spmv_acc_amd/csrc/engine_internal.hpp
--- a/spmv_acc_amd/csrc/engine_internal.hpp
+++ b/spmv_acc_amd/csrc/engine_internal.hpp
@@ -92,6 +92,7 @@
   unsigned launches = 0;
   double trial_ms = 0.0;
   int last_c16 = -1;
+  int last_col_bits = -1;
   int last_kernel = -1;
   bool tuning_open = true;
   bool captured = false;
@@ -172,6 +173,7 @@
   bool is_stale() const { return A.stale && __atomic_load_n(A.stale, __ATOMIC_RELAXED) != 0; }
   void free_col16() {
     if (col16.d16) (void)hipFree(col16.d16);
+    if (col16.d8) (void)hipFree(col16.d8);
     if (col16.rec) (void)hipFree(col16.rec);
     if (col16.ovf) (void)hipFree(col16.ovf);
     if (col16.ci_guard) (void)hipFree(col16.ci_guard);
diff --git a/spmv_acc_amd/csrc/k_col16.hip b/spmv_acc_amd/csrc/k_col16.hip
--- a/spmv_acc_amd/csrc/k_col16.hip
+++ b/spmv_acc_amd/csrc/k_col16.hip
@@ -12,13 +12,46 @@
 
 constexpr int kChunk = kCol16Chunk;
 
-__global__ __launch_bounds__(kThreads) void col16_base_kernel(const int *__restrict__ ci, int nnz, int chunk0, int nchunks,
-                                                              int *__restrict__ base, int *__restrict__ esc_count,
-                                                              unsigned long long *__restrict__ stats) {
+template <int BITS> struct CodeWidth;
+template <> struct CodeWidth<16> {
+  typedef unsigned short T;
+  static constexpr int half = 32767;
+};
+template <> struct CodeWidth<8> {
+  typedef unsigned char T;
+  static constexpr int half = 127;
+};
+
+template <int BITS>
+__device__ __forceinline__ void chunk_base(const int (&col)[4], int median, bool none, int lane, int c, int *__restrict__ base,
+                                           int *__restrict__ esc_count, unsigned long long *__restrict__ stats) {
+  constexpr int H = CodeWidth<BITS>::half;
+  long long b = static_cast<long long>(median) - H;
+  if (none || b < 0) b = 0;
+  const int bs = static_cast<int>(b);
+  int esc = 0;
+#pragma unroll
+  for (int e = 0; e < 4; ++e) {
+    if (col[e] != INT_MAX) {
+      const long long d = static_cast<long long>(col[e]) - bs;
+      esc += (d < 0 || d > 2 * H) ? 1 : 0;
+    }
+  }
+#pragma unroll
+  for (int o = 32; o > 0; o >>= 1) esc += __shfl_xor(esc, o, kWave);
+  if (lane == 0) {
+    base[c] = bs;
+    esc_count[c] = esc;
+    if (esc > 0) atomicAdd(stats, static_cast<unsigned long long>(esc));
+    if (esc > 12) atomicAdd(stats + 1, 1ull);
+    if (esc > 28) atomicAdd(stats + 2, 1ull);
+    if (esc > 60) atomicAdd(stats + 3, 1ull);
+  }
+}
+
+__device__ __forceinline__ void chunk_stats(const int *__restrict__ ci, int nnz, int chunk0, int nchunks, int c, int *__restrict__ base,
+                                            int *__restrict__ esc_count, unsigned long long *stats) {
   const int lane = threadIdx.x & (kWave - 1);
-  const long long c_ll = static_cast<long long>(blockIdx.x) * (kThreads / kWave) + threadIdx.x / kWave;
-  if (c_ll >= nchunks) return;
-  const int c = static_cast<int>(c_ll);
   const long long j0 = (static_cast<long long>(chunk0) + c) * kChunk + 4 * lane;
   int col[4];
 #pragma unroll
@@ -38,27 +71,20 @@
   const unsigned long long holder = __ballot(rank == want);
   const int src = holder ? __ffsll(static_cast<long long>(holder)) - 1 : 0;
   const int median = __shfl(mine, src, kWave);
-  long long b = static_cast<long long>(median) - 32767;
-  if (valid == 0 || b < 0) b = 0;
-  const int bs = static_cast<int>(b);
-  int esc = 0;
-#pragma unroll
-  for (int e = 0; e < 4; ++e) {
-    if (col[e] != INT_MAX) {
-      const long long d = static_cast<long long>(col[e]) - bs;
-      esc += (d < 0 || d > 65534) ? 1 : 0;
-    }
-  }
-#pragma unroll
-  for (int o = 32; o > 0; o >>= 1) esc += __shfl_xor(esc, o, kWave);
-  if (lane == 0) {
-    base[c] = bs;
-    esc_count[c] = esc;
-    if (esc > 0) atomicAdd(stats, static_cast<unsigned long long>(esc));
-    if (esc > 12) atomicAdd(stats + 1, 1ull);
-    if (esc > 28) atomicAdd(stats + 2, 1ull);
-    if (esc > 60) atomicAdd(stats + 3, 1ull);
-  }
+  chunk_base<16>(col, median, valid == 0, lane, c, base, esc_count, stats);
+  chunk_base<8>(col, median, valid == 0, lane, c, base + nchunks + 1, esc_count + nchunks + 1, stats + 4);
+}
+
+__global__ __launch_bounds__(kThreads) void col16_base_kernel(const int *__restrict__ ci, int nnz, int chunk0, int nchunks,
+                                                              int *__restrict__ base, int *__restrict__ esc_count,
+                                                              unsigned long long *__restrict__ stats) {
+  __shared__ unsigned long long tally[8];
+  if (threadIdx.x < 8) tally[threadIdx.x] = 0;
+  __syncthreads();
+  const long long c_ll = static_cast<long long>(blockIdx.x) * (kThreads / kWave) + threadIdx.x / kWave;
+  if (c_ll < nchunks) chunk_stats(ci, nnz, chunk0, nchunks, static_cast<int>(c_ll), base, esc_count, tally);
+  __syncthreads();
+  if (threadIdx.x < 8 && tally[threadIdx.x] != 0) atomicAdd(stats + threadIdx.x, tally[threadIdx.x]);
 }
 
 __global__ __launch_bounds__(kThreads) void col16_overflow_kernel(int *__restrict__ cnt, int nchunks, int E) {
@@ -69,10 +95,13 @@
   }
 }
 
+template <int BITS>
 __global__ __launch_bounds__(kThreads) void col16_encode_kernel(const int *__restrict__ ci, int nnz, int chunk0, int nchunks,
                                                                 const int *__restrict__ base, const int *__restrict__ ovf_start,
-                                                                int R, unsigned short *__restrict__ d16, int *__restrict__ rec,
-                                                                int *__restrict__ ovf) {
+                                                                int R, typename CodeWidth<BITS>::T *__restrict__ codes,
+                                                                int *__restrict__ rec, int *__restrict__ ovf) {
+  typedef typename CodeWidth<BITS>::T Code;
+  constexpr int ESC = 2 * CodeWidth<BITS>::half + 1;
   const int lane = threadIdx.x & (kWave - 1);
   const long long c_ll = static_cast<long long>(blockIdx.x) * (kThreads / kWave) + threadIdx.x / kWave;
   if (c_ll >= nchunks) return;
@@ -87,7 +116,7 @@
   for (int e = 0; e < 4; ++e) {
     col[e] = (j0 + e < nnz) ? ci[j0 + e] : bs;
     const long long d = static_cast<long long>(col[e]) - bs;
-    is_esc[e] = d < 0 || d > 65534;
+    is_esc[e] = d < 0 || d >= ESC;
     mine += is_esc[e] ? 1 : 0;
   }
   int incl = mine;
@@ -100,19 +129,19 @@
   int pos = incl - mine;
   int *r = rec + static_cast<size_t>(c) * R;
   const int o0 = ovf_start[c];
-  unsigned short out[4];
+  Code out[4];
 #pragma unroll
   for (int e = 0; e < 4; ++e) {
-    out[e] = 0xFFFF;
+    out[e] = static_cast<Code>(ESC);
     if (is_esc[e]) {
       if (pos < E) r[4 + pos] = col[e];
       else ovf[o0 + pos - E] = col[e];
       ++pos;
     } else {
-      out[e] = static_cast<unsigned short>(col[e] - bs);
+      out[e] = static_cast<Code>(col[e] - bs);
     }
   }
-  unsigned short *dst = d16 + static_cast<size_t>(c) * kChunk + 4 * lane;
+  Code *dst = codes + static_cast<size_t>(c) * kChunk + 4 * lane;
 #pragma unroll
   for (int e = 0; e < 4; ++e) dst[e] = out[e];
   if (lane == 0) {
@@ -154,11 +183,16 @@
 }
 
 void launch_col16_encode(hipStream_t stream, const int *ci, int nnz, int chunk0, int nchunks, const int *base, const int *ovf_start,
-                         int R, unsigned short *d16, int *rec, int *ovf) {
+                         int R, int bits, void *codes, int *rec, int *ovf) {
   if (nchunks <= 0) return;
   const int waves_per_block = kThreads / kWave;
-  SPMV_ACC_LAUNCH(col16_encode_kernel, dim3((nchunks + waves_per_block - 1) / waves_per_block), dim3(kThreads), 0, stream, ci, nnz,
-                     chunk0, nchunks, base, ovf_start, R, d16, rec, ovf);
+  const dim3 grid((nchunks + waves_per_block - 1) / waves_per_block);
+  if (bits == 8)
+    SPMV_ACC_LAUNCH(col16_encode_kernel<8>, grid, dim3(kThreads), 0, stream, ci, nnz, chunk0, nchunks, base, ovf_start, R,
+                       static_cast<unsigned char *>(codes), rec, ovf);
+  else
+    SPMV_ACC_LAUNCH(col16_encode_kernel<16>, grid, dim3(kThreads), 0, stream, ci, nnz, chunk0, nchunks, base, ovf_start, R,
+                       static_cast<unsigned short *>(codes), rec, ovf);
 }
 
 void launch_col16_guard(hipStream_t stream, const int *ci, int lo, int span, int *out) {
diff --git a/spmv_acc_amd/csrc/kernels.hpp b/spmv_acc_amd/csrc/kernels.hpp
--- a/spmv_acc_amd/csrc/kernels.hpp
+++ b/spmv_acc_amd/csrc/kernels.hpp
@@ -108,7 +108,9 @@
   int chunk0 = 0;
   int nchunks = 0;
   int rec_ints = 0;
+  int bits = 0;
   unsigned short *d16 = nullptr;
+  unsigned char *d8 = nullptr;
   int *rec = nullptr;
   int *ovf = nullptr;
   int *ci_guard = nullptr;
@@ -118,6 +120,7 @@
 };
 struct Col16Dev {
   const unsigned short *d16;
+  const unsigned char *d8;
   const int *rec;
   const int *ovf;
   const int *ci_guard;
@@ -126,7 +129,8 @@
 };
 inline Col16Dev col16_dev(const Col16 &C, const CsrDev &A) {
   Col16Dev d;
-  d.d16 = C.d16 - static_cast<long long>(C.chunk0) * kCol16Chunk;
+  d.d16 = C.d16 ? C.d16 - static_cast<long long>(C.chunk0) * kCol16Chunk : nullptr;
+  d.d8 = C.d8 ? C.d8 - static_cast<long long>(C.chunk0) * kCol16Chunk : nullptr;
   d.rec = C.rec - static_cast<long long>(C.chunk0) * C.rec_ints;
   d.ovf = C.ovf;
   d.ci_guard = C.ci_guard;
@@ -147,7 +151,7 @@
 void launch_col16_overflow(hipStream_t stream, int *cnt, int nchunks, int E);
 bool launch_col16_scan(hipStream_t stream, int nchunks, const int *esc_count, int *esc_start, void *tmp, size_t tmp_bytes);
 void launch_col16_encode(hipStream_t stream, const int *ci, int nnz, int chunk0, int nchunks, const int *base, const int *ovf_start, int R,
-                         unsigned short *d16, int *rec, int *ovf);
+                         int bits, void *codes, int *rec, int *ovf);
 void launch_col16_guard(hipStream_t stream, const int *ci, int lo, int span, int *out);
 
 struct FlatPlan {
diff --git a/spmv_acc_amd/csrc/plan.cpp b/spmv_acc_amd/csrc/plan.cpp
--- a/spmv_acc_amd/csrc/plan.cpp
+++ b/spmv_acc_amd/csrc/plan.cpp
@@ -503,6 +503,7 @@
       out->settled = p.calls > 0 && !p.tuning_open ? 1 : 0;
       out->last_kernel = p.last_kernel;
       out->col16 = p.last_c16;
+      out->col_bits = p.last_col_bits;
       out->slab_passes = p.seg_state == 1 && (tun(kT_slab_segments) >= 1 || (tun(kT_slab_segments) < 0 && p.seg_choice == 1)) ? p.seg_slabs - (p.seg_rest_below > 0 ? 1 : 0) : 0;
       return true;
     }
diff --git a/spmv_acc_amd/csrc/tile_stage.hpp b/spmv_acc_amd/csrc/tile_stage.hpp
--- a/spmv_acc_amd/csrc/tile_stage.hpp
+++ b/spmv_acc_amd/csrc/tile_stage.hpp
@@ -185,16 +185,47 @@
 typedef unsigned int uint2v __attribute__((ext_vector_type(2)));
 typedef uint2v uint2v_a2 __attribute__((aligned(2)));
 
-__device__ __forceinline__ void c16_decode(int (&c)[4], const uint2v d, int rv, int R, int lane, const int *__restrict__ ovf) {
+template <int BITS> struct Codes4;
+template <> struct Codes4<16> {
+  static constexpr int escape = 0xFFFF;
+  uint2v d;
+  template <bool NT> __device__ __forceinline__ void load(const Col16Dev &C, int j) {
+    const uint2v_a2 *p = reinterpret_cast<const uint2v_a2 *>(C.d16 + j);
+    d = NT ? __builtin_nontemporal_load(p) : *p;
+  }
+  __device__ __forceinline__ void split(int (&dq)[4]) const {
+    dq[0] = static_cast<int>(d.x & 0xFFFFu);
+    dq[1] = static_cast<int>(d.x >> 16);
+    dq[2] = static_cast<int>(d.y & 0xFFFFu);
+    dq[3] = static_cast<int>(d.y >> 16);
+  }
+};
+template <> struct Codes4<8> {
+  static constexpr int escape = 0xFF;
+  unsigned d;
+  template <bool NT> __device__ __forceinline__ void load(const Col16Dev &C, int j) {
+    const unsigned *p = reinterpret_cast<const unsigned *>(C.d8 + j);
+    d = NT ? __builtin_nontemporal_load(p) : *p;
+  }
+  __device__ __forceinline__ void split(int (&dq)[4]) const {
+#pragma unroll
+    for (int q = 0; q < 4; ++q) dq[q] = static_cast<int>((d >> (8 * q)) & 0xFFu);
+  }
+};
+
+template <int BITS>
+__device__ __forceinline__ void c16_decode(int (&c)[4], const Codes4<BITS> &d, int rv, int R, int lane, const int *__restrict__ ovf) {
+  constexpr int ESC = Codes4<BITS>::escape;
   const int bs = __builtin_amdgcn_readlane(rv, 0);
   const int nesc = __builtin_amdgcn_readlane(rv, 1);
-  const int dq[4] = {static_cast<int>(d.x & 0xFFFFu), static_cast<int>(d.x >> 16), static_cast<int>(d.y & 0xFFFFu), static_cast<int>(d.y >> 16)};
+  int dq[4];
+  d.split(dq);
 #pragma unroll
   for (int q = 0; q < 4; ++q) c[q] = bs + dq[q];
   if (nesc > 0) {
     const int E = R - 4;
     const unsigned long long lt = (1ull << lane) - 1ull;
-    const bool e[4] = {dq[0] == 0xFFFF, dq[1] == 0xFFFF, dq[2] == 0xFFFF, dq[3] == 0xFFFF};
+    const bool e[4] = {dq[0] == ESC, dq[1] == ESC, dq[2] == ESC, dq[3] == ESC};
     const unsigned long long slot[4] = {__ballot(e[0]), __ballot(e[1]), __ballot(e[2]), __ballot(e[3])};
     int r = __popcll(slot[0] & lt) + __popcll(slot[1] & lt) + __popcll(slot[2] & lt) + __popcll(slot[3] & lt);
 #pragma unroll
@@ -208,11 +239,11 @@
   }
 }
 
-template <int THREADS, int NPT, bool NTC, bool NTV>
+template <int THREADS, int NPT, bool NTC, bool NTV, int BITS>
 __device__ __forceinline__ void stage_products_c16_all(double *__restrict__ lds, int a0, int lo4, int hi, const Col16Dev &C,
                                                        const double *__restrict__ v, const double *__restrict__ x) {
   constexpr int K = NPT / 4;
-  uint2v d[K];
+  Codes4<BITS> d[K];
   double2v va[K], vb[K];
   int rv[K];
   const int lane = threadIdx.x & (kWave - 1);
@@ -224,11 +255,7 @@
     rv[k] = C.rec[static_cast<long long>(wave_j >> 8) * R + rl];
   }
 #pragma unroll
-  for (int k = 0; k < K; ++k) {
-    const int j = a0 + 4 * (threadIdx.x + k * THREADS);
-    const uint2v_a2 *p = reinterpret_cast<const uint2v_a2 *>(C.d16 + j);
-    d[k] = NTC ? __builtin_nontemporal_load(p) : *p;
-  }
+  for (int k = 0; k < K; ++k) d[k].template load<NTC>(C, a0 + 4 * (threadIdx.x + k * THREADS));
 #pragma unroll
   for (int k = 0; k < K; ++k) {
     const int j = a0 + 4 * (threadIdx.x + k * THREADS);
@@ -261,7 +288,7 @@
   }
 }
 
-template <int THREADS, int NPT, bool NTC, bool NTV>
+template <int THREADS, int NPT, bool NTC, bool NTV, int BITS>
 __device__ __forceinline__ void stage_products_c16_tail(double *__restrict__ lds, int a0, int lo4, int hi, const Col16Dev &C,
                                                         const double *__restrict__ v, const double *__restrict__ x) {
   const int lane = threadIdx.x & (kWave - 1);
@@ -274,8 +301,8 @@
     const int g = threadIdx.x + k * THREADS;
     const int j = a0 + 4 * g;
     const int rv = C.rec[static_cast<long long>(wave_j >> 8) * R + rl];
-    const uint2v_a2 *p = reinterpret_cast<const uint2v_a2 *>(C.d16 + j);
-    const uint2v d = NTC ? __builtin_nontemporal_load(p) : *p;
+    Codes4<BITS> d;
+    d.template load<NTC>(C, j);
     const int jv = (j >= lo4 && j < hi) ? j : lo4;
     const double2v va = load_stream_d2<NTV>(v + jv), vb = load_stream_d2<NTV>(v + jv + 2);
     int c[4];
@@ -300,8 +327,13 @@
 __device__ __forceinline__ void stage_products_c16(double *__restrict__ lds, int a0, int lo4, int hi, const Col16Dev &C,
                                                    const double *__restrict__ v, const double *__restrict__ x) {
   const int last_j = __builtin_amdgcn_readfirstlane(a0 + 4 * ((threadIdx.x & ~(kWave - 1)) + (NPT / 4 - 1) * THREADS));
-  if (last_j < hi) stage_products_c16_all<THREADS, NPT, NTC, NTV>(lds, a0, lo4, hi, C, v, x);
-  else stage_products_c16_tail<THREADS, NPT, NTC, NTV>(lds, a0, lo4, hi, C, v, x);
+  if (C.d8 != nullptr) {
+    if (last_j < hi) stage_products_c16_all<THREADS, NPT, NTC, NTV, 8>(lds, a0, lo4, hi, C, v, x);
+    else stage_products_c16_tail<THREADS, NPT, NTC, NTV, 8>(lds, a0, lo4, hi, C, v, x);
+  } else {
+    if (last_j < hi) stage_products_c16_all<THREADS, NPT, NTC, NTV, 16>(lds, a0, lo4, hi, C, v, x);
+    else stage_products_c16_tail<THREADS, NPT, NTC, NTV, 16>(lds, a0, lo4, hi, C, v, x);
+  }
 }
 
 __device__ __forceinline__ void check_ci_guard(const int *__restrict__ ci, const Col16Dev &C, int *__restrict__ stale) {
diff --git a/spmv_acc_amd/csrc/tuner.cpp b/spmv_acc_amd/csrc/tuner.cpp
--- a/spmv_acc_amd/csrc/tuner.cpp
+++ b/spmv_acc_amd/csrc/tuner.cpp
@@ -281,15 +281,16 @@
   void *tmp = nullptr;
   const size_t tmp_bytes = col16_scan_bytes(nchunks);
   const size_t n1 = static_cast<size_t>(nchunks) + 1;
-  bool ok = hip_ok(hipMalloc(reinterpret_cast<void **>(&base), sizeof(int) * n1), "hipMalloc col16 bases") &&
-            hip_ok(hipMalloc(reinterpret_cast<void **>(&cnt), sizeof(int) * n1), "hipMalloc col16 escape counts") &&
+  bool ok = hip_ok(hipMalloc(reinterpret_cast<void **>(&base), sizeof(int) * 2 * n1), "hipMalloc col16 bases") &&
+            hip_ok(hipMalloc(reinterpret_cast<void **>(&cnt), sizeof(int) * 2 * n1), "hipMalloc col16 escape counts") &&
             hip_ok(hipMalloc(reinterpret_cast<void **>(&ovf_start), sizeof(int) * n1), "hipMalloc col16 overflow offsets") &&
-            hip_ok(hipMalloc(reinterpret_cast<void **>(&stats), sizeof(unsigned long long) * 4), "hipMalloc col16 statistics") &&
+            hip_ok(hipMalloc(reinterpret_cast<void **>(&stats), sizeof(unsigned long long) * 8), "hipMalloc col16 statistics") &&
             hip_ok(hipMalloc(&tmp, tmp_bytes > 0 ? tmp_bytes : 16), "hipMalloc col16 scan workspace") &&
             hip_ok(hipMemsetAsync(cnt + nchunks, 0, sizeof(int), st), "memset col16") &&
-            hip_ok(hipMemsetAsync(stats, 0, sizeof(unsigned long long) * 4, st), "memset col16 statistics");
-  unsigned long long h_stats[4] = {0, 0, 0, 0};
-  int R = 0, total = 0;
+            hip_ok(hipMemsetAsync(cnt + n1 + nchunks, 0, sizeof(int), st), "memset col16") &&
+            hip_ok(hipMemsetAsync(stats, 0, sizeof(unsigned long long) * 8, st), "memset col16 statistics");
+  unsigned long long h_stats[8] = {0, 0, 0, 0, 0, 0, 0, 0};
+  int R = 0, total = 0, bits = 16;
   if (ok) {
     launch_col16_base(st, A.ci, A.nnz, chunk0, nchunks, base, cnt, stats);
     ok = hip_ok(hipMemcpyAsync(h_stats, stats, sizeof(h_stats), hipMemcpyDeviceToHost, st), "read col16 statistics") &&
@@ -298,30 +299,41 @@
   if (ok) {
     const unsigned long long limit = static_cast<unsigned long long>(nchunks) / 100;
     R = h_stats[1] <= limit ? 16 : (h_stats[2] <= limit ? 32 : (h_stats[3] <= limit ? 64 : 0));
+    const int R8 = h_stats[5] <= limit ? 16 : (h_stats[6] <= limit ? 32 : (h_stats[7] <= limit ? 64 : 0));
+    const long long extra8 = static_cast<long long>(h_stats[4]) - static_cast<long long>(h_stats[0]);
+    const int mode = tun(kT_col16);
+    bits = mode == 8 || (mode != 2 && R > 0 && R8 > 0 && R8 <= R && 200 * extra8 <= static_cast<long long>(A.count())) ? 8 : 16;
+    if (bits == 8) R = R8;
     const int forced = tun(kT_col16) > 1 ? tun(kT_col16) : 0;
     if (forced == 16 || forced == 32 || forced == 64) R = forced;
     tune_log("m %d nnz %d 16-bit columns: %llu escapes in %d chunks, %llu / %llu / %llu chunks above 12 / 28 / 60 -> %s", A.m, A.nnz, h_stats[0], nchunks,
              h_stats[1], h_stats[2], h_stats[3], R ? (R == 16 ? "16-int records" : (R == 32 ? "32-int records" : "64-int records")) : "not encoded");
+    tune_log("m %d nnz %d 8-bit columns: %llu escapes (%+lld), %llu / %llu / %llu chunks above 12 / 28 / 60 -> %d-bit codes", A.m, A.nnz, h_stats[4], extra8,
+             h_stats[5], h_stats[6], h_stats[7], bits);
   }
   if (ok && R > 0) {
-    launch_col16_overflow(st, cnt, nchunks, R - 4);
-    ok = launch_col16_scan(st, nchunks, cnt, ovf_start, tmp, tmp_bytes) &&
+    const size_t cofs = bits == 8 ? n1 : 0;
+    launch_col16_overflow(st, cnt + cofs, nchunks, R - 4);
+    ok = launch_col16_scan(st, nchunks, cnt + cofs, ovf_start, tmp, tmp_bytes) &&
          hip_ok(hipMemcpyAsync(&total, ovf_start + nchunks, sizeof(int), hipMemcpyDeviceToHost, st), "read col16 overflow total") &&
          hip_ok(hipStreamSynchronize(st), "sync col16");
-    const size_t d16_bytes = sizeof(unsigned short) * static_cast<size_t>(nchunks) * kCol16Chunk;
+    const size_t code_bytes = static_cast<size_t>(bits / 8) * static_cast<size_t>(nchunks) * kCol16Chunk;
     const size_t rec_bytes = sizeof(int) * static_cast<size_t>(nchunks) * R;
     const size_t ovf_bytes = sizeof(int) * (static_cast<size_t>(total) + 64);
-    ok = ok && hip_ok(hipMalloc(reinterpret_cast<void **>(&C.d16), d16_bytes), "hipMalloc col16 offsets") &&
+    void *codes = nullptr;
+    ok = ok && hip_ok(hipMalloc(&codes, code_bytes), "hipMalloc col16 offsets") &&
          hip_ok(hipMalloc(reinterpret_cast<void **>(&C.rec), rec_bytes), "hipMalloc col16 records") &&
          hip_ok(hipMalloc(reinterpret_cast<void **>(&C.ovf), ovf_bytes), "hipMalloc col16 overflow list") &&
          hip_ok(hipMalloc(reinterpret_cast<void **>(&C.ci_guard), sizeof(int) * kGuardSamples), "hipMalloc col16 guard") &&
          hip_ok(hipMemsetAsync(C.rec, 0, rec_bytes, st), "memset col16 records") && hip_ok(hipMemsetAsync(C.ovf, 0, ovf_bytes, st), "memset col16 overflow");
+    if (bits == 8) C.d8 = static_cast<unsigned char *>(codes);
+    else C.d16 = static_cast<unsigned short *>(codes);
     if (ok) {
-      launch_col16_encode(st, A.ci, A.nnz, chunk0, nchunks, base, ovf_start, R, C.d16, C.rec, C.ovf);
+      launch_col16_encode(st, A.ci, A.nnz, chunk0, nchunks, base + cofs, ovf_start, R, bits, codes, C.rec, C.ovf);
       launch_col16_guard(st, A.ci, A.nnz0, A.count() > 0 ? A.count() - 1 : 0, C.ci_guard);
       ok = hip_ok(hipStreamSynchronize(st), "sync col16 encode");
     }
-    C.bytes = d16_bytes + rec_bytes + ovf_bytes;
+    C.bytes = code_bytes + rec_bytes + ovf_bytes;
   }
   for (void *q : {static_cast<void *>(base), static_cast<void *>(cnt), static_cast<void *>(ovf_start), static_cast<void *>(stats), tmp})
     if (q) (void)hipFree(q);
@@ -338,7 +350,8 @@
   C.chunk0 = chunk0;
   C.nchunks = nchunks;
   C.rec_ints = R;
-  C.escapes = static_cast<long long>(h_stats[0]);
+  C.bits = bits;
+  C.escapes = static_cast<long long>(h_stats[bits == 8 ? 4 : 0]);
   C.overflow = total;
   return true;
 }
```
